# csiro-robotics/HOTFormerLoc

Hardware: AMD Instinct MI355X
Metric: point-clouds/sec (4096 pts, Wild-Places cfg) (higher is better)
Workload: dtype f32 storage and accumulation; Linear products as 3-term bf16 (hi, lo) split (16 significant bits per operand); window-attention QK^T / PV on fp16 (hi, lo) pairs (22 significant bits), softmax in f32; matched_precision leg = fp32-grade Linear products (3 bf16 planes per operand, 6 plane products) + f; 1 GPU; wild-places cfg, batch=32 clouds/GPU x 4096 pts, octree depth 7, forward-only, octree+neighbours resident, window plan + tap tables rebuilt inside every step (reference boundary); global_batch=32, parallelism=dp1, gemm=x3, collective=none

## Files before the change

### hotformerloc_amd/_native.py

```python

import ctypes
import os
from ctypes import c_char_p, c_double, c_float, c_int, c_int32, c_int64, c_uint32, c_uint64, c_void_p

_HERE = os.path.dirname(os.path.abspath(__file__))
LIB_PATH = os.path.join(_HERE, 'lib', 'libhotformerloc_hip.so')

HFL_OCTREE_MAX_POINTS = 1 << 20
HFL_OCTREE_MAX_DEPTH = 10


class NativeLibraryError(RuntimeError):
    pass


class WindowAttnDesc(ctypes.Structure):
    _fields_ = [('n_tokens', c_int64), ('rt_row0', c_int64), ('n_windows', c_int32),
                ('patch_size', c_int32), ('dilation', c_int32), ('n_relay', c_int32),
                ('n_heads', c_int32), ('pos_bnd', c_int32), ('batch_size', c_int32),
                ('scale', c_float), ('depth', c_int32), ('rpe_expanded', c_void_p)]


class BlockWeights(ctypes.Structure):
    _fields_ = [('channels', c_int64), ('eps', c_float), ('q_scale', c_float),
# ... 28 lines not shown
PHASE_REST = 2
PHASE_RELAY_QKV = 3
PHASE_TAIL = 4
FUSE_ATTN_NO_RELAY = 1
FUSE_ATTN_WS = 2


class BlockIO(ctypes.Structure):
    _fields_ = [('x_in', c_void_p), ('relay', c_void_p), ('out', c_void_p), ('arena', c_void_p),
                ('neigh', c_void_p), ('tok_meta', c_void_p), ('n_rows', c_int64), ('n_tokens', c_int64),
                ('phase', c_int32)]


class AdamChunk(ctypes.Structure):
    _fields_ = [('param', c_void_p), ('grad', c_void_p), ('exp_avg', c_void_p), ('exp_avg_sq', c_void_p), ('ema', c_void_p),
                ('count', c_int32), ('slot', c_int32)]


class AdamSlot(ctypes.Structure):
    _fields_ = [('step_size', c_float), ('bias_correction2_sqrt', c_float), ('one_minus_beta1', c_float), ('beta2', c_float),
                ('one_minus_beta2', c_float), ('eps', c_float), ('decay', c_float), ('decoupled', c_int32)]


class AugmentCloud(ctypes.Structure):
    _fields_ = [('remove_k', c_int32), ('block', c_int32), ('rot_cos', c_float), ('rot_sin', c_float), ('trans', c_float * 3),
                ('block_u', c_float * 4), ('reserved', c_float)]


class AugmentConfig(ctypes.Structure):
    _fields_ = [('normalize', c_int32), ('cylindrical_mask', c_int32), ('cylindrical_transform', c_int32),
                ('augment', c_int32), ('rotate', c_int32), ('set_rotate', c_int32), ('flip_axis', c_int32),
                ('set_cos', c_float), ('set_sin', c_float), ('jitter_sigma', c_float), ('jitter_clip', c_float)]


SIGNATURES = {
    'hfl_version': (c_int, []),
    'hfl_arch': (c_char_p, []),
    'hfl_dwconv_forward_backward': (c_int, [c_void_p, c_void_p, c_void_p, c_void_p, c_int, c_int64,
                                            c_int64, c_int, c_void_p]),
    'hfl_dwconv_weight_backward_workspace': (c_int64, [c_int64, c_int64, c_int]),
    'hfl_dwconv_weight_backward': (c_int, [c_void_p, c_void_p, c_void_p, c_void_p, c_int, c_int64,
                                           c_int64, c_int, c_void_p, c_void_p]),
    'hfl_inverse_neigh': (c_int, [c_void_p, c_void_p, c_int, c_int64, c_int, c_void_p]),
    'hfl_cpe_forward': (c_int, [c_void_p, c_void_p, c_void_p, c_void_p, c_void_p, c_void_p, c_int64,
                                c_int64, c_int, c_float, c_int, c_void_p]),
    'hfl_cpe_forward_save': (c_int, [c_void_p, c_void_p, c_void_p, c_void_p, c_void_p, c_void_p, c_void_p, c_int64,
                                c_int64, c_int, c_float, c_int, c_void_p]),
    'hfl_dwconv_add': (c_int, [c_void_p, c_void_p, c_void_p, c_void_p, c_void_p, c_int64, c_int64, c_int, c_void_p]),
    'hfl_octree_scratch_bytes': (c_int64, [c_int64, c_int, c_int, c_int]),
    'hfl_octree_build_clouds': (c_int, [c_void_p, c_void_p, c_int, c_int64, c_int, c_int, c_int,
                                        c_void_p, c_void_p, c_void_p, c_void_p]),
    'hfl_octree_merge': (c_int, [c_void_p, c_void_p, c_void_p, c_int, c_int, c_int, c_int64,
                                 c_void_p, c_void_p, c_void_p, c_void_p, c_void_p, c_void_p,
                                 c_void_p]),
    'hfl_octree_neigh': (c_int, [c_void_p, c_void_p, c_void_p, c_void_p, c_void_p, c_int64, c_int,
                                 c_int, c_void_p]),
    'hfl_token_meta': (c_int, [c_void_p, c_void_p, c_int64, c_int, c_void_p]),
    'hfl_octree_gather': (c_int, [c_void_p, c_void_p, c_void_p, c_int64, c_int, c_int64, c_void_p]),
    'hfl_prepare_clouds': (c_int, [c_void_p, c_void_p, c_void_p, c_void_p, c_int, c_int, c_int, c_int, c_void_p]),
    'hfl_augment_clouds': (c_int, [c_void_p, c_void_p, c_void_p, c_void_p, c_void_p, c_void_p, c_int, c_void_p, c_void_p,
                                   ctypes.POINTER(AugmentConfig), c_uint64, c_int64, c_void_p, c_void_p]),
    'hfl_voxel_keys': (c_int, [c_void_p, c_void_p, c_void_p, c_void_p, c_void_p, c_int, c_int64, c_double, c_void_p]),
    'hfl_voxel_reduce_workspace': (c_int64, [c_int64]),
    'hfl_voxel_reduce': (c_int, [c_void_p, c_void_p, c_void_p, c_void_p, c_void_p, c_void_p, c_void_p, c_int64, c_int, c_void_p,
                                 c_int64, c_void_p]),
    'hfl_submap_normalise': (c_int, [c_void_p, c_void_p, c_void_p, c_void_p, c_void_p, c_int, c_void_p]),
    'hfl_submap_normalise_rows': (c_int, [c_void_p] * 8 + [c_int, c_void_p]),
    'hfl_voxel_gather_rows': (c_int, [c_void_p, c_void_p, c_int64, c_void_p, c_int64, c_void_p]),
    'hfl_voxel_bounds': (c_int, [c_void_p, c_void_p, c_void_p, c_int, c_int64, c_void_p]),
    'hfl_voxel_occupancy_workspace': (c_int64, [c_int, c_int64]),
    'hfl_voxel_occupancy': (c_int, [c_void_p, c_void_p, c_int, c_int64, c_void_p, c_void_p, c_void_p, c_int, c_int64, c_int64,
                                    c_void_p, c_int64, c_void_p]),
    'hfl_cloth_raster': (c_int, [c_void_p, c_void_p, c_void_p, c_void_p, c_int, c_int64, c_void_p, c_void_p, c_int64, c_float,
                                 c_void_p]),
    'hfl_cloth_simulate': (c_int, [c_void_p, c_void_p, c_void_p, c_void_p, c_void_p, c_void_p, c_int, c_int64, c_float, c_float,
                                   c_float, c_float, c_int, c_int, c_void_p]),
    'hfl_cloth_classify': (c_int, [c_void_p, c_void_p, c_void_p, c_void_p, c_int, c_int64, c_void_p, c_void_p, c_int64, c_float,
                                   c_float, c_void_p]),
    'hfl_cloud_nonfinite': (c_int, [c_void_p, c_void_p, c_void_p, c_int, c_int64, c_void_p]),
    'hfl_knn_cell_keys': (c_int, [c_void_p, c_void_p, c_void_p, c_int, c_int64, c_void_p, c_void_p, c_int64, c_void_p]),
    'hfl_knn_mean_dist': (c_int, [c_void_p] * 9 + [c_int, c_int64, c_void_p, c_int64, c_int, c_void_p]),
    'hfl_outlier_threshold': (c_int, [c_void_p, c_void_p, c_void_p, c_int, c_int64, c_double, c_void_p]),
    'hfl_outlier_mask': (c_int, [c_void_p, c_void_p, c_void_p, c_void_p, c_int, c_int64, c_void_p]),
    'hfl_radius_mask': (c_int, [c_void_p, c_void_p, c_int64, c_double, c_void_p]),
    'hfl_tap_lists_workspace': (c_int64, [c_int64, c_int]),
    'hfl_tap_lists': (c_int, [c_void_p, c_void_p, c_void_p, c_void_p, c_int64, c_int, c_void_p, c_void_p]),
    'hfl_tap_lists_multi': (c_int, [c_int, c_void_p, c_void_p, c_void_p, c_void_p, c_void_p, c_void_p, c_void_p, c_void_p]),
    'hfl_tap_tiles': (c_int, [c_void_p, c_void_p, c_int, c_int, c_int, c_void_p]),
    'hfl_pad_index': (c_int, [c_void_p, c_void_p, c_int, c_int64, c_void_p]),
    'hfl_pad_rows': (c_int, [c_void_p, c_void_p, c_void_p, c_int, c_int64, c_int64, c_void_p]),
    'hfl_mixer_tail': (c_int, [c_void_p] * 6 + [c_int] * 5 + [c_void_p]),
    'hfl_attn_pool_ok': (c_int, [c_int]),
    'hfl_attn_pool_workspace': (c_int64, [c_int, c_int, c_int, c_int64]),
    'hfl_attn_pool': (c_int, [c_void_p, c_int64, c_void_p, c_void_p, c_void_p, c_int, c_int, c_int, c_int64, c_float, c_void_p,
                              c_int64, c_void_p]),
    'hfl_window_attention_fwd': (c_int, [c_void_p, c_void_p, c_void_p, c_void_p,
                                         ctypes.POINTER(WindowAttnDesc), c_void_p]),
    'hfl_window_attention_fwd_ex': (c_int, [c_void_p, c_void_p, c_void_p, c_void_p, c_void_p,
                                            ctypes.POINTER(WindowAttnDesc), c_int, c_void_p]),
    'hfl_window_attention_fwd_multi': (c_int, [c_int, c_void_p, c_void_p, c_void_p, c_void_p, c_void_p, c_int, c_void_p]),
    'hfl_layer_norm_split3': (c_int, [c_void_p, c_void_p, c_void_p, c_void_p, c_int64, c_int64,
                                      c_float, c_void_p]),
    'hfl_add_layer_norm_split3': (c_int, [c_void_p, c_void_p, c_void_p, c_void_p, c_void_p, c_void_p,
                                          c_void_p, c_int64, c_int64, c_float, c_void_p]),
    'hfl_add_bias': (c_int, [c_void_p, c_void_p, c_void_p, c_void_p, c_int64, c_int64, c_void_p]),
    'hfl_bias_gelu_split3': (c_int, [c_void_p, c_void_p, c_void_p, c_int64, c_int64, c_void_p]),
    'hfl_split3': (c_int, [c_void_p, c_void_p, c_int64, c_int64, c_void_p]),
    'hfl_window_attention_bwd': (c_int, [c_void_p, c_void_p, c_void_p, c_void_p, c_void_p, c_void_p,
                                         ctypes.POINTER(WindowAttnDesc), c_void_p]),
    'hfl_window_attention_bwd_workspace': (c_int64, [ctypes.POINTER(WindowAttnDesc)]),
    'hfl_window_attention_bwd_det': (c_int, [c_void_p, c_void_p, c_void_p, c_void_p, c_void_p, c_void_p,
                                             ctypes.POINTER(WindowAttnDesc), c_void_p, c_void_p]),
    'hfl_window_attention_bwd_split2': (c_int, [c_void_p, c_void_p, c_void_p, c_void_p, c_void_p, c_void_p,
                                                ctypes.POINTER(WindowAttnDesc), c_void_p, c_void_p]),
    'hfl_relay_attention_bwd': (c_int, [c_void_p, c_void_p, c_void_p, c_void_p, c_void_p, c_int, c_int,
                                        c_float, c_int, c_void_p]),
    'hfl_inverse_table': (c_int, [c_void_p, c_int64, c_void_p, c_int64, c_int, c_void_p]),
    'hfl_octree_gather_bwd': (c_int, [c_void_p, c_void_p, c_void_p, c_int64, c_int, c_int64, c_void_p]),
    'hfl_relay_token_init_bwd': (c_int, [c_void_p, c_void_p, c_void_p, c_int64, c_int32, c_int32,
                                         c_int64, c_void_p]),
    'hfl_linear_x3': (c_int, [c_void_p, c_void_p, c_void_p, c_void_p, c_void_p, c_int64, c_int, c_int, c_int, c_void_p]),
    'hfl_linear_x6_grouped_gather': (c_int, [c_void_p, c_void_p, c_void_p, c_void_p, c_int64, c_void_p, c_int64, c_int64, c_int, c_int,
                                     c_void_p]),
    'hfl_linear_x6_padded_k': (c_int64, [c_int64]),
    'hfl_linear_x6_pack': (c_int, [c_void_p, c_void_p, c_int64, c_int64, c_void_p]),
    'hfl_linear_x6': (c_int, [c_void_p, c_void_p, c_void_p, c_void_p, c_void_p, c_void_p, c_int64, c_int, c_int, c_int, c_void_p]),
    'hfl_linear_x6_gelu_fwd': (c_int, [c_void_p, c_void_p, c_void_p, c_void_p, c_void_p, c_int64, c_int, c_int, c_void_p]),
    'hfl_linear_x6_gelu_bwd': (c_int, [c_void_p, c_void_p, c_void_p, c_void_p, c_int64, c_int, c_int, c_void_p]),
    'hfl_layer_norm_split2': (c_int, [c_void_p, c_void_p, c_void_p, c_void_p, c_int64, c_int64,
                                      c_float, c_void_p]),
    'hfl_layer_norm_relu': (c_int, [c_void_p, c_void_p, c_void_p, c_void_p, c_void_p, c_int64, c_int64, c_float, c_void_p]),
    'hfl_linear_x3_qkv': (c_int, [c_void_p, c_void_p, c_void_p, c_void_p, c_int64, c_int, c_int, c_float, c_void_p]),
    'hfl_window_attention_f16_ok': (c_int, [ctypes.POINTER(WindowAttnDesc), c_int64]),
    'hfl_split2': (c_int, [c_void_p, c_void_p, c_int64, c_int64, c_void_p]),
    'hfl_block_forward_x3_arena': (c_int64, [c_int64, c_int64]),
    'hfl_block_forward_x3': (c_int, [c_void_p, c_void_p, c_void_p, c_void_p]),
    'hfl_block_attention_x3_multi': (c_int, [c_int, c_void_p, c_void_p, c_void_p, c_void_p]),
    'hfl_relay_block_forward_x3_arena': (c_int64, [c_int64, c_int64]),
    'hfl_relay_block_forward_x3': (c_int, [c_void_p, c_void_p, c_void_p]),
    'hfl_relay_block_fused_ok': (c_int, [c_void_p, c_void_p]),
    'hfl_relay_block_fused_x3': (c_int, [c_void_p, c_void_p, c_void_p]),
    'hfl_relay_block_pack_bytes': (c_int64, [c_int]),
    'hfl_relay_block_pack': (c_int, [c_void_p, c_void_p, c_void_p, c_void_p, c_void_p, c_int, c_void_p]),
    'hfl_linear_x3_grouped': (c_int, [c_void_p, c_void_p, c_void_p, c_void_p, c_int64, c_int64, c_int, c_int, c_void_p]),
    'hfl_linear_x3_grouped_gather': (c_int, [c_void_p, c_void_p, c_void_p, c_int64, c_void_p, c_void_p, c_int64, c_int64, c_int,
                                     c_int, c_void_p]),
    'hfl_split2_rows': (c_int, [c_void_p, c_void_p, c_void_p, c_int64, c_int64, c_void_p]),
    'hfl_linear_x3_rows': (c_int, [c_void_p, c_void_p, c_void_p, c_void_p, c_void_p, c_void_p, c_int64, c_int, c_int, c_void_p]),
    'hfl_linear_x3_gelu_fwd': (c_int, [c_void_p, c_void_p, c_void_p, c_void_p, c_void_p, c_int64, c_int, c_int, c_void_p]),
    'hfl_linear_x3_gelu_bwd': (c_int, [c_void_p, c_void_p, c_void_p, c_void_p, c_int64, c_int, c_int, c_void_p]),
    'hfl_tap_wgrad': (c_int, [c_void_p, c_void_p, c_void_p, c_void_p, c_int, c_void_p, c_int, c_int, c_int, c_void_p,
                             c_void_p]),
    'hfl_slot_sum': (c_int, [c_void_p, c_void_p, c_void_p, c_void_p, c_int64, c_int64, c_int, c_void_p]),
    'hfl_tap_wgrad_gather': (c_int, [c_void_p, c_void_p, c_void_p, c_void_p, c_void_p, c_void_p, c_int, c_void_p, c_int, c_int,
                                    c_int, c_void_p, c_void_p]),
    'hfl_wgrad_x3_workspace': (c_int64, [c_int64, c_int64, c_int64]),
    'hfl_wgrad_x3': (c_int, [c_void_p, c_void_p, c_void_p, c_void_p, c_int64, c_int64, c_int64, c_void_p, c_void_p]),
    'hfl_wgrad_f32_workspace': (c_int64, [c_int64, c_int64, c_int64]),
    'hfl_wgrad_f32': (c_int, [c_void_p, c_void_p, c_void_p, c_void_p, c_int64, c_int64, c_int64, c_void_p, c_void_p]),
    'hfl_layer_norm_bwd_blocks': (c_int, [c_int64, c_int64]),
    'hfl_layer_norm_bwd_add': (c_int, [c_void_p, c_void_p, c_void_p, c_void_p, c_void_p, c_void_p, c_void_p, c_int64, c_int64,
                                       c_float, c_void_p]),
    'hfl_layer_norm_bwd_finalize': (c_int, [c_void_p, c_void_p, c_void_p, c_void_p, c_int, c_int64, c_void_p]),
    'hfl_layer_norm_bwd': (c_int, [c_void_p, c_void_p, c_void_p, c_void_p, c_void_p, c_void_p, c_int64, c_int64,
                                   c_float, c_void_p]),
    'hfl_set_variant': (c_int, [c_char_p, c_int]),
    'hfl_smoothap_rows': (c_int, [c_void_p, c_void_p, c_void_p, c_void_p, c_void_p, c_void_p, c_int, c_int,
                                  c_float, c_void_p]),
    'hfl_pairwise_dist': (c_int, [c_void_p, c_void_p, c_int, c_int, c_void_p]),
    'hfl_pairwise_dist_bwd': (c_int, [c_void_p, c_void_p, c_void_p, c_void_p, c_int, c_int, c_void_p]),
    'hfl_batch_masks': (c_int, [c_void_p, c_void_p, c_void_p, c_void_p, c_int, c_void_p, c_void_p, c_void_p, c_void_p, c_int,
                                c_void_p]),
    'hfl_radius_lists': (c_int, [c_void_p, c_void_p, c_void_p, c_void_p, c_void_p, c_void_p, c_int64, c_void_p, c_int64, c_double,
                                 c_double, c_int, c_void_p]),
    'hfl_transform_points': (c_int, [c_void_p, c_void_p, c_void_p, c_void_p, c_int64, c_int64, c_void_p]),
    'hfl_nn_dist': (c_int, [c_void_p, c_void_p, c_void_p, c_void_p, c_int64, c_void_p, c_void_p, c_int64, c_void_p, c_int64,
                            c_int64, c_void_p]),
    'hfl_pair_stats': (c_int, [c_void_p, c_void_p, c_void_p, c_void_p, c_int64, c_int64, ctypes.POINTER(c_float), c_int,
                               c_void_p]),
    'hfl_ema_update': (c_int, [c_void_p, c_int, c_float, c_void_p]),
    'hfl_adam_step': (c_int, [c_void_p, c_int, c_void_p, c_int, c_float, c_void_p]),
    'hfl_kd_rows': (c_int, [c_void_p, c_void_p, c_void_p, c_void_p, c_int, c_int, c_float, c_void_p]),
    'hfl_gemm_bf16_tn': (c_int, [c_void_p, c_void_p, c_void_p, c_int64, c_int, c_int, c_void_p]),
    'hfl_gemm_bf16': (c_int, [c_void_p, c_void_p, c_void_p, c_void_p, c_void_p, c_int64, c_int, c_int, c_void_p]),
    'hfl_window_rpe_expand_size': (c_int64, [c_int, c_int, c_int, c_int]),
    'hfl_window_rpe_expand': (c_int, [c_void_p, c_void_p, c_int, c_int, c_int, c_int, c_void_p]),
    'hfl_relay_attention_fwd': (c_int, [c_void_p, c_void_p, c_void_p, c_void_p, c_int, c_int,
                                        c_float, c_int, c_void_p]),
    'hfl_relay_attention_f16_fwd': (c_int, [c_void_p, c_void_p, c_void_p, c_void_p, c_int, c_int, c_int, c_void_p, c_int, c_void_p]),
    'hfl_relay_token_init': (c_int, [c_void_p, c_void_p, c_void_p, c_int64, c_int32, c_int32,
                                     c_int64, c_void_p]),
    'hfl_window_stats': (c_int, [c_void_p, c_void_p, c_int64, c_int32, c_int32, c_int, c_void_p]),
    'hfl_layer_norm': (c_int, [c_void_p, c_void_p, c_void_p, c_void_p, c_int64, c_int64, c_float,
                               c_void_p]),
    'hfl_add_layer_norm': (c_int, [c_void_p, c_void_p, c_void_p, c_void_p, c_void_p, c_void_p,
                                   c_void_p, c_int64, c_int64, c_float, c_void_p]),
    'hfl_mlp_fused_pack_bytes': (c_int64, [c_int]),
    'hfl_mlp_fused_pack': (c_int, [c_void_p, c_void_p, c_void_p, c_int, c_void_p]),
    'hfl_ln_mlp_fused': (c_int, [c_void_p, c_void_p, c_void_p, c_void_p, c_float, c_void_p, c_void_p, c_void_p, c_int64, c_int,
                         c_void_p]),
    'hfl_ln_mlp_fused_workspace': (c_int64, [c_int64, c_int]),
    'hfl_mlp_fused_pack_bytes_h': (c_int64, [c_int, c_int]),
    'hfl_mlp_fused_pack_h': (c_int, [c_void_p, c_void_p, c_void_p, c_int, c_int, c_void_p]),
    'hfl_ln_mlp_fused_workspace_h': (c_int64, [c_int64, c_int, c_int]),
    'hfl_ln_mlp_fused_h': (c_int, [c_void_p, c_void_p, c_void_p, c_void_p, c_float, c_void_p, c_void_p, c_void_p, c_int64, c_int,
                                   c_int, c_void_p, c_int64, c_void_p]),
    'hfl_ln_mlp_fused_ws': (c_int, [c_void_p, c_void_p, c_void_p, c_void_p, c_float, c_void_p, c_void_p, c_void_p, c_int64, c_int,
                            c_void_p, c_int64, c_void_p]),
    'hfl_attn_fused_ok': (c_int, [c_void_p, c_int, c_int]),
    'hfl_attn_fused_fwd': (c_int, [c_void_p, c_void_p, c_void_p, c_void_p, c_float, c_void_p, c_void_p, c_float, c_void_p, c_void_p,
                           c_void_p, c_void_p]),
    'hfl_attn_ws_ok': (c_int, [c_void_p, c_int]),
    'hfl_attn_ws_fwd': (c_int, [c_void_p, c_void_p, c_void_p, c_void_p, c_float, c_void_p, c_void_p, c_float, c_void_p,
                        c_void_p, c_void_p, c_void_p, c_void_p]),
    'hfl_qkv_fused_pack_bytes': (c_int64, [c_int]),
    'hfl_qkv_fused_pack': (c_int, [c_void_p, c_void_p, c_int, c_void_p]),
    'hfl_ln_qkv_fused_seg': (c_int, [c_void_p, c_void_p, c_void_p, c_void_p, c_float, c_void_p, c_void_p, c_float, c_int64, c_int,
                                     c_void_p]),
    'hfl_linear_x3_seg': (c_int, [c_void_p, c_void_p, c_void_p, c_void_p, c_void_p, c_int64, c_int, c_int, c_void_p]),
    'hfl_ln_qkv_fused': (c_int, [c_void_p, c_void_p, c_void_p, c_void_p, c_float, c_void_p, c_void_p, c_float, c_int64, c_int,
                         c_void_p]),
    'hfl_segment_softmax': (c_int, [c_void_p, c_void_p, c_int, c_int, c_float, c_void_p]),
    'hfl_row_sq_norms': (c_int, [c_void_p, c_void_p, c_int64, c_int, c_void_p]),
    'hfl_flat_l2_topk_workspace': (c_int64, [c_int64, c_int64, c_int64, c_int]),
    'hfl_flat_l2_topk': (c_int, [c_void_p, c_void_p, c_void_p, c_void_p, c_void_p, c_int64, c_int64, c_int, c_int, c_void_p,
                                 c_int64, c_void_p]),
}

_lib = None


def load():
    global _lib
    if _lib is not None:
        return _lib
    if not os.path.exists(LIB_PATH):
        raise NativeLibraryError(
            'libhotformerloc_hip.so not found at %s -- the HIP extension is required '
            '(no CPU fallback); run `python -m hotformerloc_amd.build`' % LIB_PATH)
    lib = ctypes.CDLL(LIB_PATH)
    for name, (res, args) in SIGNATURES.items():
        try:
            fn = getattr(lib, name)
        except AttributeError as e:
            raise NativeLibraryError('symbol %s missing from %s' % (name, LIB_PATH)) from e
        fn.restype = res
        fn.argtypes = args
    _lib = lib
    return lib


def check(rc: int, what: str):
    if rc != 0:
        kind = {-1: 'HFL_EINVAL (unsupported shape/argument)',
                -2: 'HFL_ECAPACITY (input exceeds a kernel limit)'}.get(
                    rc, 'hipBLASLt status %d' % (-100 - rc) if rc <= -100 else 'hipError %d' % rc)
        raise NativeLibraryError('%s failed: %s' % (what, kind))


def ptr_array(ptrs):
    arr = (c_void_p * len(ptrs))()
    for i, p in enumerate(ptrs):
        arr[i] = p
    return arr
```

### hotformerloc_amd/build.py

```python

import os
import shutil
import subprocess
import sys
from concurrent.futures import ThreadPoolExecutor

HERE = os.path.dirname(os.path.abspath(__file__))
CSRC = os.path.join(HERE, 'csrc')
LIBDIR = os.path.join(HERE, 'lib')
LIBNAME = 'libhotformerloc_hip.so'
ARCH = 'gfx950'
SOURCES = ['capi.hip', 'dwconv.hip', 'octree.hip', 'preprocess.hip', 'augment.hip', 'voxel.hip', 'ground.hip', 'outliers.hip', 'window_misc.hip', 'attention.hip', 'gemm_x3.hip', 'gemm_x6.hip', 'mlp_fused.hip', 'qkv_fused.hip', 'attn_fused.hip', 'attn_ws.hip', 'relay_block.hip', 'attn_pool.hip', 'wgrad_x3.hip', 'wgrad_f32.hip', 'tapconv.hip', 'gemm_lt.hip', 'loss.hip', 'pairwise.hip', 'batch_masks.hip', 'radius.hip', 'overlap.hip', 'ema.hip', 'optim.hip', 'retrieval.hip']
FLAGS = ['--offload-arch=' + ARCH, '-O3', '-std=c++17', '-fPIC', '-fno-gpu-rdc',
         '-Wall', '-Wno-unused-function']
ROCM = os.environ.get('ROCM_PATH', '/opt/rocm')
LINK_FLAGS = ['-L' + os.path.join(ROCM, 'lib'), '-lhipblaslt', '-Wl,-rpath,' + os.path.join(ROCM, 'lib')]
EXTRA_FLAGS = {'attention.hip': ['-mllvm', '-amdgpu-mfma-vgpr-form=1'],
               'mlp_fused.hip': ['-fno-slp-vectorize'],
               'qkv_fused.hip': ['-fno-slp-vectorize'],
               'attn_fused.hip': ['-fno-slp-vectorize', '-mllvm', '-amdgpu-mfma-vgpr-form=1'],
               'attn_ws.hip': ['-fno-slp-vectorize', '-mllvm', '-amdgpu-mfma-vgpr-form=1'],
               'relay_block.hip': ['-fno-slp-vectorize', '-mllvm', '-amdgpu-mfma-vgpr-form=1'],
               'radius.hip': ['-ffp-contract=off'],
               'ground.hip': ['-ffp-contract=off'],
               'outliers.hip': ['-ffp-contract=off']}


def _hipcc() -> str:
    for cand in (os.environ.get('HIPCC'), shutil.which('hipcc'), '/opt/rocm/bin/hipcc'):
        if cand and os.path.exists(cand):
            return cand
    raise RuntimeError('hipcc not found (need ROCm >= 7.0 for gfx950)')


def _newer(target: str, deps) -> bool:
    if not os.path.exists(target):
        return False
    t = os.path.getmtime(target)
    return all(os.path.getmtime(d) <= t for d in deps)


def build_library(force: bool = False, verbose: bool = True) -> str:
    os.makedirs(LIBDIR, exist_ok=True)
    objdir = os.path.join(LIBDIR, 'obj')
    os.makedirs(objdir, exist_ok=True)
    hipcc = _hipcc()
    headers = [os.path.join(CSRC, 'hfl_common.h'), os.path.join(CSRC, 'x3_math.h'), os.path.join(CSRC, 'stage_stream.h'),
               os.path.join(CSRC, 'prep_common.h'),
               os.path.join(HERE, '..', 'include', 'hotformerloc_hip.h')]
    jobs = []
    for src in SOURCES:
        s = os.path.join(CSRC, src)
        o = os.path.join(objdir, src.replace('.hip', '.o'))
        if force or not _newer(o, [s] + headers):
            jobs.append((s, o))

    def compile_one(job):
        s, o = job
        cmd = [hipcc] + FLAGS + EXTRA_FLAGS.get(os.path.basename(s), []) + os.environ.get('HFL_EXTRA_HIPCC_FLAGS', '').split() + \
            ['-c', s, '-o', o]
        r = subprocess.run(cmd, capture_output=True, text=True)
        if r.returncode != 0:
            raise RuntimeError('hipcc failed for %s:\n%s' % (s, r.stderr))
        if verbose and r.stderr.strip():
            print(r.stderr, file=sys.stderr)
        return o

    if jobs:
        with ThreadPoolExecutor(max_workers=min(4, len(jobs))) as ex:
            list(ex.map(compile_one, jobs))
    objs = [os.path.join(objdir, s.replace('.hip', '.o')) for s in SOURCES]
    for stale in set(os.listdir(objdir)) - {os.path.basename(o) for o in objs}:
        os.remove(os.path.join(objdir, stale))
    lib = os.path.join(LIBDIR, LIBNAME)
    if force or jobs or not os.path.exists(lib):
        cmd = [hipcc, '--offload-arch=' + ARCH, '-shared', '-fPIC', '-o', lib] + objs + LINK_FLAGS
        r = subprocess.run(cmd, capture_output=True, text=True)
        if r.returncode != 0:
            raise RuntimeError('link failed:\n' + r.stderr)
    if verbose:
        print('built', lib)
    return lib


if __name__ == '__main__':
    build_library(force='--force' in sys.argv)
```

### hotformerloc_amd/csrc/dwconv.hip

```cpp
#include "hfl_common.h"

namespace {

constexpr int kMaxTaps = 27;
constexpr int kMaxRowsPerBlock = 16;

struct RowGeom {
  int tpr;
  int rpb;
};

static RowGeom row_geom(int64_t channels) {
  RowGeom g;
  g.tpr = (int)(channels / 4);
  g.rpb = 256 / g.tpr;
  if (g.rpb < 1) g.rpb = 1;
  if (g.rpb > kMaxRowsPerBlock) g.rpb = kMaxRowsPerBlock;
  return g;
}

static int persistent_per_cu(const void* kernel, int threads, size_t lds, int want, int* cache_nb, size_t* cache_lds) {
  if (*cache_lds != lds + 1) {
    int nb = 0;
    if (hipOccupancyMaxActiveBlocksPerMultiprocessor(&nb, kernel, threads, lds) != hipSuccess || nb < 1) nb = 0;
    *cache_nb = nb;
    *cache_lds = lds + 1;
  }
  const int nb = *cache_nb;
  if (nb < 1) return want;
  if (nb >= want) return want;
  return (want / nb) * nb >= nb ? ((want / nb) * nb) : nb;
}

template <typename IdxT, int KFIX>
__global__ void __launch_bounds__(256) dwconv_fwd_vec4(float* __restrict__ out, const float* __restrict__ data,
                                const float* __restrict__ weight, const IdxT* __restrict__ neigh,
                                int64_t n_out, int C, int kngh, int tpr, int rpb) {
  extern __shared__ __attribute__((aligned(16))) unsigned char smem[];
  const int K = KFIX > 0 ? KFIX : kngh;
  float4* s_w = reinterpret_cast<float4*>(smem);
  IdxT* s_idx = reinterpret_cast<IdxT*>(smem + (size_t)K * C * sizeof(float));
  const int tx = threadIdx.x % tpr, ty = threadIdx.x / tpr;
  const int c4n = C / 4;
  for (int i = threadIdx.x; i < K * c4n; i += blockDim.x)
    s_w[i] = reinterpret_cast<const float4*>(weight)[i];

  for (int64_t base = (int64_t)blockIdx.x * rpb; base < n_out; base += (int64_t)gridDim.x * rpb) {
    const int64_t h = base + ty;
    const bool live = h < n_out;
    __syncthreads();
    if (live)
      for (int k = tx; k < K; k += tpr) s_idx[ty * K + k] = neigh[h * K + k];
    __syncthreads();
    if (!live) continue;
    float4 acc = make_float4(0.f, 0.f, 0.f, 0.f);
    constexpr int B = 9;
#pragma unroll 1
    for (int k0 = 0; k0 < K; k0 += B) {
      float4 v[B];
      bool ok[B];
#pragma unroll
      for (int j = 0; j < B; ++j) {
        const int k = k0 + j;
        int64_t ni = (k < K) ? (int64_t)s_idx[ty * K + k] : -1;
        ok[j] = ni >= 0;
        if (!ok[j]) ni = 0;
        v[j] = reinterpret_cast<const float4*>(data + ni * C)[tx];
      }
#pragma unroll
      for (int j = 0; j < B; ++j) {
        const int k = k0 + j;
        if (k < K && ok[j]) acc = hfl_fma4(s_w[k * c4n + tx], v[j], acc);
      }
    }
    reinterpret_cast<float4*>(out + h * C)[tx] = acc;
  }
}

template <int B>
__global__ void __launch_bounds__(256) slot_sum_kernel(float* __restrict__ out, const float* __restrict__ part,
                                                        const int32_t* __restrict__ slot, const float* __restrict__ bias,
                                                        int64_t n_out, int C, int K, int tpr, int rpb) {
  extern __shared__ __attribute__((aligned(16))) unsigned char smem[];
  int32_t* s_idx = reinterpret_cast<int32_t*>(smem);
  const int tx = threadIdx.x % tpr, ty = threadIdx.x / tpr;
  const float4 bv = bias != nullptr ? reinterpret_cast<const float4*>(bias)[tx] : make_float4(0.f, 0.f, 0.f, 0.f);
  for (int64_t base = (int64_t)blockIdx.x * rpb; base < n_out; base += (int64_t)gridDim.x * rpb) {
    const int64_t h = base + ty;
    const bool live = h < n_out;
    __syncthreads();
    if (live)
      for (int k = tx; k < K; k += tpr) s_idx[ty * K + k] = slot[h * K + k];
    __syncthreads();
    if (!live) continue;
    float4 acc = make_float4(0.f, 0.f, 0.f, 0.f);
#pragma unroll 1
    for (int k0 = 0; k0 < K; k0 += B) {
      float4 v[B];
      bool ok[B];
#pragma unroll
      for (int j = 0; j < B; ++j) {
        const int k = k0 + j;
        int64_t ni = (k < K) ? (int64_t)s_idx[ty * K + k] : -1;
        ok[j] = ni >= 0;
        if (!ok[j]) ni = 0;
        v[j] = reinterpret_cast<const float4*>(part + ni * C)[tx];
      }
#pragma unroll
      for (int j = 0; j < B; ++j)
        if (ok[j]) { acc.x += v[j].x; acc.y += v[j].y; acc.z += v[j].z; acc.w += v[j].w; }
    }
    if (bias != nullptr) { acc.x += bv.x; acc.y += bv.y; acc.z += bv.z; acc.w += bv.w; }
    reinterpret_cast<float4*>(out + h * C)[tx] = acc;
  }
}

template <typename IdxT>
__global__ void dwconv_fwd_scalar(float* __restrict__ out, const float* __restrict__ data,
                                  const float* __restrict__ weight, const IdxT* __restrict__ neigh,
                                  int64_t n_out, int64_t C, int K) {
  const int64_t total = n_out * C;
  for (int64_t i = (int64_t)blockIdx.x * blockDim.x + threadIdx.x; i < total;
       i += (int64_t)gridDim.x * blockDim.x) {
    const int64_t h = i / C, c = i % C;
    float acc = 0.f;
    for (int k = 0; k < K; ++k) {
      const int64_t ni = (int64_t)neigh[h * K + k];
      if (ni >= 0) acc = fmaf(weight[k * C + c], data[ni * C + c], acc);
    }
    out[i] = acc;
  }
}

template <typename IdxT>
static int launch_fwd(float* out, const float* data, const float* weight, const IdxT* neigh,
                      int64_t n_out, int64_t C, int K, hipStream_t s) {
  if (n_out == 0) return HFL_OK;
  if (C % 4 == 0 && C <= 1024 && K <= kMaxTaps) {
    RowGeom g = row_geom(C);
    const size_t lds = (size_t)K * C * sizeof(float) + (size_t)g.rpb * K * sizeof(IdxT);
    const int64_t need = hfl_cdiv(n_out, g.rpb);
    static int nb27 = 0, nb0 = 0;
    static size_t l27 = 0, l0 = 0;
    const int per_cu = K == 27 ? persistent_per_cu(reinterpret_cast<const void*>(dwconv_fwd_vec4<IdxT, 27>), g.tpr * g.rpb, lds, 8,
                                                   &nb27, &l27)
                               : persistent_per_cu(reinterpret_cast<const void*>(dwconv_fwd_vec4<IdxT, 0>), g.tpr * g.rpb, lds, 8,
                                                   &nb0, &l0);
    const int64_t cap = (int64_t)hfl_stream_cus(s) * per_cu;
    const int blocks = (int)(need < cap ? need : cap);
    if (K == 27)
      dwconv_fwd_vec4<IdxT, 27><<<blocks, g.tpr * g.rpb, lds, s>>>(out, data, weight, neigh, n_out,
                                                                   (int)C, K, g.tpr, g.rpb);
    else
      dwconv_fwd_vec4<IdxT, 0><<<blocks, g.tpr * g.rpb, lds, s>>>(out, data, weight, neigh, n_out,
                                                                  (int)C, K, g.tpr, g.rpb);
  } else {
    const int64_t total = n_out * C;
    const int64_t need = hfl_cdiv(total, 256);
    const int blocks = (int)(need < 2048 ? need : 2048);
    dwconv_fwd_scalar<IdxT><<<blocks, 256, 0, s>>>(out, data, weight, neigh, n_out, C, K);
  }
  HFL_RETURN_LAST_ERROR();
}

template <typename IdxT, int B, int K0>
__device__ __forceinline__ void wgrad_taps(float4 (&acc)[kMaxTaps], const float4 g, const float* __restrict__ data,
                                           const IdxT* idx, int K, int C, int tx) {
  constexpr int NB = K0 + B <= kMaxTaps ? B : kMaxTaps - K0;
  float4 d[NB];
  bool ok[NB];
#pragma unroll
  for (int j = 0; j < NB; ++j) {
    const int64_t ni = K0 + j < K ? (int64_t)idx[K0 + j] : (int64_t)-1;
    ok[j] = ni >= 0;
    d[j] = reinterpret_cast<const float4*>(data + (ok[j] ? ni : (int64_t)0) * C)[tx];
  }
#pragma unroll
  for (int j = 0; j < NB; ++j) {
    const float4 a = hfl_fma4(d[j], g, acc[K0 + j]);
    acc[K0 + j].x = ok[j] ? a.x : acc[K0 + j].x;
    acc[K0 + j].y = ok[j] ? a.y : acc[K0 + j].y;
    acc[K0 + j].z = ok[j] ? a.z : acc[K0 + j].z;
    acc[K0 + j].w = ok[j] ? a.w : acc[K0 + j].w;
  }
}

template <typename IdxT, int B, int K0 = 0>
__device__ __forceinline__ void wgrad_row(float4 (&acc)[kMaxTaps], const float4 g, const float* __restrict__ data,
                                          const IdxT* idx, int K, int C, int tx) {
  if constexpr (K0 < kMaxTaps) {
    if (K0 < K) wgrad_taps<IdxT, B, K0>(acc, g, data, idx, K, C, tx);
    wgrad_row<IdxT, B, K0 + B>(acc, g, data, idx, K, C, tx);
  }
}

template <typename IdxT, int B>
__global__ void __launch_bounds__(256) dwconv_wgrad_partial(float* __restrict__ partial, const float* __restrict__ grad,
                                     const float* __restrict__ data, const IdxT* __restrict__ neigh,
                                     int64_t n_rows, int C, int K, int tpr, int rpb) {
  extern __shared__ __attribute__((aligned(16))) unsigned char smem[];
  IdxT* s_idx = reinterpret_cast<IdxT*>(smem);
  const int tx = threadIdx.x % tpr, ty = threadIdx.x / tpr;
  float4 acc[kMaxTaps];
#pragma unroll
  for (int k = 0; k < kMaxTaps; ++k) acc[k] = make_float4(0.f, 0.f, 0.f, 0.f);
  const int64_t groups = (n_rows + rpb - 1) / rpb;
  const int64_t per_xcd = (groups + 7) >> 3;
  const int xcd = blockIdx.x & 7;
  const int64_t xg0 = (int64_t)xcd * per_xcd;
  const int64_t xg1 = xg0 + per_xcd < groups ? xg0 + per_xcd : groups;
  const int nb = ((int)gridDim.x - xcd + 7) >> 3;
  for (int64_t grp = xg0 + (blockIdx.x >> 3); grp < xg1; grp += nb) {
    const int64_t h = grp * rpb + ty;
    const bool live = h < n_rows;
    __syncthreads();
    if (live)
      for (int k = tx; k < K; k += tpr) s_idx[ty * K + k] = neigh[h * K + k];
    __syncthreads();
    if (!live) continue;
    const float4 g = reinterpret_cast<const float4*>(grad + h * C)[tx];
    wgrad_row<IdxT, B>(acc, g, data, s_idx + ty * K, K, C, tx);
  }
  float4* s_red = reinterpret_cast<float4*>(smem + (((size_t)rpb * K * sizeof(IdxT) + 15) & ~(size_t)15));
#pragma unroll
  for (int k0 = 0; k0 < kMaxTaps; k0 += 9) {
    if (k0 < K && rpb > 1) {
      __syncthreads();
      if (ty > 0) {
#pragma unroll
        for (int j = 0; j < 9; ++j)
          if (k0 + j < K) s_red[((ty - 1) * 9 + j) * tpr + tx] = acc[k0 + j];
      }
      __syncthreads();
      if (ty == 0) {
        for (int t = 1; t < rpb; ++t) {
#pragma unroll
          for (int j = 0; j < 9; ++j)
            if (k0 + j < K) {
              const float4 v = s_red[((t - 1) * 9 + j) * tpr + tx];
              acc[k0 + j].x += v.x; acc[k0 + j].y += v.y; acc[k0 + j].z += v.z; acc[k0 + j].w += v.w;
            }
        }
      }
    }
  }
  if (ty == 0) {
    float4* dst = reinterpret_cast<float4*>(partial + (int64_t)blockIdx.x * K * C);
#pragma unroll
    for (int k = 0; k < kMaxTaps; ++k)
      if (k < K) dst[k * (C / 4) + tx] = acc[k];
  }
}

__global__ void __launch_bounds__(1024) dwconv_wgrad_reduce(float* __restrict__ out, const float* __restrict__ partial,
                                                            int n_partial, int64_t kc) {
  __shared__ float s[16][64];
  const int lane = threadIdx.x & 63, grp = threadIdx.x >> 6;
  const int64_t i = (int64_t)blockIdx.x * 64 + lane;
  float acc = 0.f;
  if (i < kc)
    for (int p = grp; p < n_partial; p += 16) acc += partial[(int64_t)p * kc + i];
  s[grp][lane] = acc;
  __syncthreads();
  if (grp == 0 && i < kc) {
    float v = 0.f;
#pragma unroll
// ... 29 lines not shown
template <typename IdxT>
static int launch_wgrad(float* out, const float* grad, const float* data, const IdxT* neigh,
                        int64_t n_rows, int64_t C, int K, void* workspace, hipStream_t s) {
  if (C % 4 == 0 && C <= 1024 && K <= kMaxTaps) {
    RowGeom g = row_geom(C);
    const int blocks = wgrad_blocks(n_rows, g.rpb);
    const size_t lds = (((size_t)g.rpb * K * sizeof(IdxT) + 15) & ~(size_t)15) +
                       (size_t)(g.rpb - 1) * 9 * C * sizeof(float);
    float* partial = static_cast<float*>(workspace);
    dwconv_wgrad_partial<IdxT, 9><<<blocks, g.tpr * g.rpb, lds, s>>>(partial, grad, data, neigh, n_rows, (int)C, K, g.tpr, g.rpb);
    const int64_t kc = (int64_t)K * C;
    dwconv_wgrad_reduce<<<(int)hfl_cdiv(kc, 64), 1024, 0, s>>>(out, partial, blocks, kc);
  } else {
    const int64_t kc = (int64_t)K * C;
    dwconv_wgrad_scalar<IdxT><<<(int)hfl_cdiv(kc, 256), 256, 0, s>>>(out, grad, data, neigh, n_rows, C, K);
  }
  HFL_RETURN_LAST_ERROR();
}

template <typename IdxT>
__global__ void inverse_neigh_kernel(IdxT* __restrict__ ineigh, const IdxT* __restrict__ neigh,
                                     int64_t n_rows, int K) {
  const int64_t total = n_rows * K;
  for (int64_t i = (int64_t)blockIdx.x * blockDim.x + threadIdx.x; i < total;
       i += (int64_t)gridDim.x * blockDim.x) {
    const int64_t h = i / K;
    const int k = (int)(i % K);
    const int64_t j = (int64_t)neigh[i];
    if (j >= 0) ineigh[j * K + k] = (IdxT)h;
  }
}

template <int TPR, bool NORM>
__global__ void __launch_bounds__(256) cpe_fwd_kernel(float* __restrict__ out, float* __restrict__ conv_out,
                               const float* __restrict__ x, const float* __restrict__ add,
                               const float* __restrict__ weight, const float* __restrict__ gamma,
                               const float* __restrict__ beta, const int32_t* __restrict__ neigh,
                               int64_t n_rows, int K, float eps, int residual) {
  constexpr int C = TPR * 4;
  constexpr int RPB = 256 / TPR;
  extern __shared__ __attribute__((aligned(16))) unsigned char smem[];
  float4* s_w = reinterpret_cast<float4*>(smem);
  int32_t* s_idx = reinterpret_cast<int32_t*>(smem + (size_t)K * C * sizeof(float));
  unsigned char* s_tap = reinterpret_cast<unsigned char*>(s_idx + (256 / TPR) * K);
  const int tx = threadIdx.x % TPR, ty = threadIdx.x / TPR;
  for (int i = threadIdx.x; i < K * TPR; i += blockDim.x)
    s_w[i] = reinterpret_cast<const float4*>(weight)[i];
  const float4 gm = NORM ? reinterpret_cast<const float4*>(gamma)[tx] : make_float4(1.f, 1.f, 1.f, 1.f);
  const float4 bt = NORM ? reinterpret_cast<const float4*>(beta)[tx] : make_float4(0.f, 0.f, 0.f, 0.f);

  const int64_t groups = (n_rows + RPB - 1) / RPB;
  const int64_t per_xcd = (groups + 7) >> 3;
  const int64_t xg0 = (int64_t)(blockIdx.x & 7) * per_xcd;
  const int64_t xg1 = xg0 + per_xcd < groups ? xg0 + per_xcd : groups;
  for (int64_t grp = xg0 + (blockIdx.x >> 3); grp < xg1; grp += gridDim.x >> 3) {
    const int64_t base = grp * RPB;
    const int64_t h = base + ty;
    const bool live = h < n_rows;
    __syncthreads();
    int n_live = 0;
    if (TPR >= kMaxTaps) {
      const int ni = (live && tx < K) ? neigh[h * K + tx] : -1;
      const unsigned long long bal = __ballot(ni >= 0);
      const int shift = (threadIdx.x & 63) - tx;
      const unsigned mask = (unsigned)((bal >> shift) & ((1ull << kMaxTaps) - 1ull));
      n_live = __popc(mask);
      if (ni >= 0) {
        const int rank = __popc(mask & ((1u << tx) - 1u));
        s_idx[ty * K + rank] = ni;
        s_tap[ty * K + rank] = (unsigned char)tx;
      }
    } else if (live) {
      for (int k = tx; k < K; k += TPR) s_idx[ty * K + k] = neigh[h * K + k];
    }
    __syncthreads();
    float4 acc = make_float4(0.f, 0.f, 0.f, 0.f);
    constexpr int B = 9;
    if (TPR >= kMaxTaps) {
#pragma unroll 1
      for (int k0 = 0; k0 < n_live; k0 += B) {
        float4 v[B];
        int e[B];
#pragma unroll
        for (int j = 0; j < B; ++j) {
          e[j] = ty * K + min(k0 + j, n_live - 1);
          v[j] = reinterpret_cast<const float4*>(x + (int64_t)s_idx[e[j]] * C)[tx];
        }
#pragma unroll
        for (int j = 0; j < B; ++j) {
          float4 w = s_w[(int)s_tap[e[j]] * TPR + tx];
          if (k0 + j >= n_live) w = make_float4(0.f, 0.f, 0.f, 0.f);
          acc = hfl_fma4(w, v[j], acc);
        }
      }
    } else {
#pragma unroll 1
      for (int k0 = 0; k0 < K; k0 += B) {
        float4 v[B];
        bool ok[B];
#pragma unroll
        for (int j = 0; j < B; ++j) {
          const int k = k0 + j;
          int64_t ni = (live && k < K) ? (int64_t)s_idx[ty * K + k] : -1;
          ok[j] = ni >= 0;
          if (!ok[j]) ni = 0;
          v[j] = reinterpret_cast<const float4*>(x + ni * C)[tx];
        }
#pragma unroll
        for (int j = 0; j < B; ++j) {
          const int k = k0 + j;
          if (k < K && ok[j]) acc = hfl_fma4(s_w[k * TPR + tx], v[j], acc);
        }
      }
    }
    float4 y = acc;
    if (NORM) {
      const float inv_c = 1.0f / (float)C;
      const float mean = hfl_group_sum<TPR>((acc.x + acc.y) + (acc.z + acc.w)) * inv_c;
      const float4 d = make_float4(acc.x - mean, acc.y - mean, acc.z - mean, acc.w - mean);
      const float var = hfl_group_sum<TPR>((d.x * d.x + d.y * d.y) + (d.z * d.z + d.w * d.w)) * inv_c;
      const float rstd = 1.0f / sqrtf(var + eps);
      y = make_float4(fmaf(d.x * rstd, gm.x, bt.x), fmaf(d.y * rstd, gm.y, bt.y),
                      fmaf(d.z * rstd, gm.z, bt.z), fmaf(d.w * rstd, gm.w, bt.w));
    }
    if (live) {
      if (NORM && conv_out != nullptr) reinterpret_cast<float4*>(conv_out + h * C)[tx] = acc;
      if (residual) {
        const float4 xv = reinterpret_cast<const float4*>(add + h * C)[tx];
        y.x += xv.x; y.y += xv.y; y.z += xv.z; y.w += xv.w;
      }
      reinterpret_cast<float4*>(out + h * C)[tx] = y;
    }
  }
}


template <int TPR, bool NORM>
static int launch_cpe(float* out, float* conv_out, const float* x, const float* add, const float* w, const float* gamma,
                      const float* beta, const int32_t* neigh, int64_t n, int K, float eps,
                      int residual, hipStream_t s) {
  constexpr int RPB = 256 / TPR;
  const size_t lds = (size_t)K * TPR * 16 + (size_t)RPB * K * (sizeof(int32_t) + 1) + 16;
  const int64_t need = hfl_cdiv(n, RPB);
  static int nb = 0;
  static size_t nb_lds = 0;
  const int per_cu = persistent_per_cu(reinterpret_cast<const void*>(cpe_fwd_kernel<TPR, NORM>), 256, lds, 8, &nb, &nb_lds);
  const int64_t cap = (int64_t)hfl_stream_cus(s) * per_cu;
  int blocks = (int)(need < cap ? need : cap);
  blocks = (blocks + 7) & ~7;
  cpe_fwd_kernel<TPR, NORM><<<blocks, 256, lds, s>>>(out, conv_out, x, add, w, gamma, beta, neigh, n, K, eps, residual);
  HFL_RETURN_LAST_ERROR();
}

}

extern "C" {

int hfl_dwconv_forward_backward(float* out, const float* data, const float* weight,
                                const void* neigh, int idx64, int64_t n_out, int64_t channels,
                                int kngh, hfl_stream_t stream) {
  if (n_out < 0 || channels <= 0 || kngh <= 0) return HFL_EINVAL;
  hipStream_t s = static_cast<hipStream_t>(stream);
  if (idx64)
    return launch_fwd<int64_t>(out, data, weight, static_cast<const int64_t*>(neigh), n_out,
                               channels, kngh, s);
  return launch_fwd<int32_t>(out, data, weight, static_cast<const int32_t*>(neigh), n_out,
                             channels, kngh, s);
}

int64_t hfl_dwconv_weight_backward_workspace(int64_t n_rows, int64_t channels, int kngh) {
  if (channels % 4 != 0 || channels > 1024 || kngh > kMaxTaps) return 16;
  RowGeom g = row_geom(channels);
  return (int64_t)wgrad_blocks(n_rows, g.rpb) * kngh * channels * (int64_t)sizeof(float);
}

int hfl_dwconv_weight_backward(float* out, const float* grad, const float* data,
                               const void* neigh, int idx64, int64_t n_rows, int64_t channels,
                               int kngh, void* workspace, hfl_stream_t stream) {
  if (n_rows < 0 || channels <= 0 || kngh <= 0) return HFL_EINVAL;
  hipStream_t s = static_cast<hipStream_t>(stream);
  if (idx64)
    return launch_wgrad<int64_t>(out, grad, data, static_cast<const int64_t*>(neigh), n_rows,
                                 channels, kngh, workspace, s);
  return launch_wgrad<int32_t>(out, grad, data, static_cast<const int32_t*>(neigh), n_rows,
                               channels, kngh, workspace, s);
}

int hfl_inverse_neigh(void* ineigh, const void* neigh, int idx64, int64_t n_rows, int kngh,
                      hfl_stream_t stream) {
  if (n_rows < 0 || kngh <= 0) return HFL_EINVAL;
  hipStream_t s = static_cast<hipStream_t>(stream);
  const size_t esz = idx64 ? 8 : 4;
  hipError_t e = hipMemsetAsync(ineigh, 0xFF, (size_t)n_rows * kngh * esz, s);
  if (e != hipSuccess) return (int)e;
  if (n_rows == 0) return HFL_OK;
  const int64_t need = hfl_cdiv(n_rows * kngh, 256);
  const int blocks = (int)(need < 4096 ? need : 4096);
  if (idx64)
    inverse_neigh_kernel<int64_t><<<blocks, 256, 0, s>>>(static_cast<int64_t*>(ineigh),
                                                         static_cast<const int64_t*>(neigh), n_rows, kngh);
  else
    inverse_neigh_kernel<int32_t><<<blocks, 256, 0, s>>>(static_cast<int32_t*>(ineigh),
                                                         static_cast<const int32_t*>(neigh), n_rows, kngh);
  HFL_RETURN_LAST_ERROR();
}

int hfl_cpe_forward_save(float* out, float* conv_out, const float* x, const float* weight, const float* gamma,
                         const float* beta, const int32_t* neigh, int64_t n_rows, int64_t channels,
                         int kngh, float eps, int residual, hfl_stream_t stream) {
  if (n_rows < 0 || kngh <= 0 || kngh > kMaxTaps) return HFL_EINVAL;
  if (n_rows == 0) return HFL_OK;
  hipStream_t s = static_cast<hipStream_t>(stream);
  switch (channels) {
    case 256: return launch_cpe<64, true>(out, conv_out, x, x, weight, gamma, beta, neigh, n_rows, kngh, eps, residual, s);
    case 128: return launch_cpe<32, true>(out, conv_out, x, x, weight, gamma, beta, neigh, n_rows, kngh, eps, residual, s);
    case 64:  return launch_cpe<16, true>(out, conv_out, x, x, weight, gamma, beta, neigh, n_rows, kngh, eps, residual, s);
    case 32:  return launch_cpe<8, true>(out, conv_out, x, x, weight, gamma, beta, neigh, n_rows, kngh, eps, residual, s);
    default:  return HFL_EINVAL;
  }
}

int hfl_dwconv_add(float* out, const float* data, const float* weight, const int32_t* neigh, const float* add,
                   int64_t n_out, int64_t channels, int kngh, hfl_stream_t stream) {
  if (n_out < 0 || kngh <= 0 || kngh > kMaxTaps || out == data || out == nullptr) return HFL_EINVAL;
  if (n_out == 0) return HFL_OK;
  hipStream_t s = static_cast<hipStream_t>(stream);
  const int res = add != nullptr ? 1 : 0;
  switch (channels) {
    case 256: return launch_cpe<64, false>(out, nullptr, data, add, weight, nullptr, nullptr, neigh, n_out, kngh, 0.f, res, s);
    case 128: return launch_cpe<32, false>(out, nullptr, data, add, weight, nullptr, nullptr, neigh, n_out, kngh, 0.f, res, s);
    case 64:  return launch_cpe<16, false>(out, nullptr, data, add, weight, nullptr, nullptr, neigh, n_out, kngh, 0.f, res, s);
    case 32:  return launch_cpe<8, false>(out, nullptr, data, add, weight, nullptr, nullptr, neigh, n_out, kngh, 0.f, res, s);
    default:  return HFL_EINVAL;
  }
}

int hfl_cpe_forward(float* out, const float* x, const float* weight, const float* gamma,
                    const float* beta, const int32_t* neigh, int64_t n_rows, int64_t channels,
                    int kngh, float eps, int residual, hfl_stream_t stream) {
  return hfl_cpe_forward_save(out, nullptr, x, weight, gamma, beta, neigh, n_rows, channels, kngh, eps, residual, stream);
}

int hfl_inverse_table(int32_t* inverse, int64_t n_src_rows, const int32_t* table, int64_t n_dst_rows,
                      int kngh, hfl_stream_t stream) {
  if (n_src_rows < 0 || n_dst_rows < 0 || kngh <= 0) return HFL_EINVAL;
  hipStream_t s = static_cast<hipStream_t>(stream);
  hipError_t e = hipMemsetAsync(inverse, 0xFF, (size_t)n_src_rows * kngh * sizeof(int32_t), s);
  if (e != hipSuccess) return (int)e;
  if (n_dst_rows == 0) return HFL_OK;
  const int64_t need = hfl_cdiv(n_dst_rows * kngh, 256);
  const int blocks = (int)(need < 4096 ? need : 4096);
  inverse_neigh_kernel<int32_t><<<blocks, 256, 0, s>>>(inverse, table, n_dst_rows, kngh);
  HFL_RETURN_LAST_ERROR();
}

int hfl_slot_sum(float* out, const float* part, const int32_t* slot, const float* bias, int64_t n_out, int64_t channels, int kngh,
                 hfl_stream_t stream) {
  if (n_out < 0 || channels <= 0 || channels % 4 != 0 || channels > 1024 || kngh <= 0 || kngh > kMaxTaps) return HFL_EINVAL;
  if (n_out == 0) return HFL_OK;
  if (out == nullptr || part == nullptr || slot == nullptr) return HFL_EINVAL;
  hipStream_t s = static_cast<hipStream_t>(stream);
  const RowGeom g = row_geom(channels);
  const size_t lds = (size_t)g.rpb * kngh * sizeof(int32_t);
  static int nb = 0;
  static size_t nb_lds = 0;
  const int per_cu = persistent_per_cu(reinterpret_cast<const void*>(slot_sum_kernel<9>), g.tpr * g.rpb, lds, 8, &nb, &nb_lds);
  const int64_t need = hfl_cdiv(n_out, g.rpb), cap = (int64_t)hfl_stream_cus(s) * per_cu;
  slot_sum_kernel<9><<<(int)(need < cap ? need : cap), g.tpr * g.rpb, lds, s>>>(out, part, slot, bias, n_out, (int)channels, kngh,
                                                                               g.tpr, g.rpb);
  HFL_RETURN_LAST_ERROR();
}
}
```

### hotformerloc_amd/csrc/octree.hip

```cpp
#include "hfl_common.h"

namespace {

constexpr int kBuildThreads = 1024;
constexpr int kLdsChunk = 16384;
constexpr int kMaxDepthSlots = HFL_OCTREE_MAX_DEPTH + 1;

__device__ __forceinline__ uint32_t shuffle_key(uint32_t x, uint32_t y, uint32_t z, int depth) {
  uint32_t key = 0;
  for (int i = 0; i < depth; ++i)
    key |= (((x >> i) & 1u) << (3 * i + 2)) | (((y >> i) & 1u) << (3 * i + 1)) |
           (((z >> i) & 1u) << (3 * i));
  return key;
}

__device__ __forceinline__ void unshuffle_key(uint32_t key, int depth, int& x, int& y, int& z) {
  x = y = z = 0;
  for (int i = 0; i < depth; ++i) {
    x |= ((key >> (3 * i + 2)) & 1u) << i;
    y |= ((key >> (3 * i + 1)) & 1u) << i;
    z |= ((key >> (3 * i)) & 1u) << i;
  }
}

// ... 170 lines not shown
      o[2] = sz / c;
      ++rank;
    }
  }
  int cur = total;
  if (tid == 0) counts[depth * batch + b] = cur;
  __syncthreads();

  for (int d = depth; d > full_depth; --d) {
    const uint32_t* kd = sv.key_at(d) + base;
    uint32_t* kp = sv.key_at(d - 1) + base;
    uint32_t* sl = sv.slot_at(d) + base;
    const int perd = (cur + kBuildThreads - 1) / kBuildThreads;
    const int a0 = min(tid * perd, cur), a1 = min(a0 + perd, cur);
    int h = 0;
    for (int i = a0; i < a1; ++i) h += (i == 0 || (kd[i - 1] >> 3) != (kd[i] >> 3)) ? 1 : 0;
    int tot = 0;
    int r = block_excl_scan(h, s_wave, &tot);
    for (int i = a0; i < a1; ++i) {
      const uint32_t ki = kd[i];
      if (i == 0 || (kd[i - 1] >> 3) != (ki >> 3)) {
        kp[r] = ki >> 3;
        ++r;
      }
      sl[i] = (uint32_t)(r - 1) * 8u + (ki & 7u);
    }
    cur = tot;
    if (tid == 0) counts[(d - 1) * batch + b] = cur;
    __syncthreads();
  }
  if (tid < full_depth) counts[tid * batch + b] = 1 << (3 * tid);
}

struct MergeArgs {
  int64_t* keys[kMaxDepthSlots];
  int32_t* children[kMaxDepthSlots];
  int64_t* nkeys[kMaxDepthSlots];
  int32_t* nidx[kMaxDepthSlots];
};

__device__ __forceinline__ int find_cloud(const int64_t* __restrict__ off, int batch, int64_t t) {
  int lo = 0, hi = batch;
  while (hi - lo > 1) {
    const int mid = (lo + hi) >> 1;
    if (off[mid] <= t) lo = mid; else hi = mid;
  }
  return lo;
}

__global__ void merge_sparse_kernel(ScratchView sv, const int64_t* __restrict__ cloud_off,
                                    const int32_t* __restrict__ cum_nne, int batch, int depth,
                                    int full_depth, MergeArgs a,
                                    const float* __restrict__ leaf_points,
                                    float* __restrict__ points_out) {
  const int d = full_depth + blockIdx.y;
  const int64_t t = (int64_t)blockIdx.x * blockDim.x + threadIdx.x;
  if (t >= sv.P) return;
  const int b = find_cloud(cloud_off, batch, t);
  const int64_t i = t - cloud_off[b];
  const int32_t* cum_d = cum_nne + (int64_t)d * (batch + 1);
  const int64_t cnt = cum_d[b + 1] - cum_d[b];
  if (i >= cnt) return;
  const int64_t g = cum_d[b] + i;
  const uint32_t key = sv.key_at(d)[t];
  const int64_t bbits = (int64_t)b << 48;
  a.nkeys[d][g] = bbits | (int64_t)key;
  int64_t pos;
  if (d == full_depth) {
    pos = ((int64_t)b << (3 * d)) + key;
  } else {
    const int32_t* cum_p = cum_nne + (int64_t)(d - 1) * (batch + 1);
    pos = 8 * (int64_t)cum_p[b] + sv.slot_at(d)[t];
  }
  a.nidx[d][g] = (int32_t)pos;
  a.children[d][pos] = (int32_t)g;
  if (d < depth && a.keys[d + 1] != nullptr) {
    int64_t* kc = a.keys[d + 1] + 8 * g;
#pragma unroll
    for (int j = 0; j < 8; ++j) kc[j] = bbits | (int64_t)(key * 8u + j);
  }
  if (d == depth) {
    const float* src = leaf_points + t * 3;
    float* dst = points_out + g * 3;
    dst[0] = src[0];
    dst[1] = src[1];
    dst[2] = src[2];
  }
}

__global__ void merge_full_kernel(int batch, int full_depth, MergeArgs a) {
  const int d = blockIdx.y;
  const int64_t per = (int64_t)1 << (3 * d);
  const int64_t t = (int64_t)blockIdx.x * blockDim.x + threadIdx.x;
  if (t >= per * batch) return;
  const int64_t b = t / per, m = t % per;
  if (a.keys[d] != nullptr) a.keys[d][t] = (b << 48) | m;
  if (d < full_depth) {
    a.children[d][t] = (int32_t)t;
    a.nkeys[d][t] = (b << 48) | m;
    a.nidx[d][t] = (int32_t)t;
  }
}

__global__ void neigh_full_kernel(int32_t* __restrict__ out, const int32_t* __restrict__ children,
                                  const int64_t* __restrict__ nkeys, int64_t nne, int depth) {
  const int64_t t = (int64_t)blockIdx.x * blockDim.x + threadIdx.x;
  if (t >= nne * 27) return;
  const int64_t g = t / 27;
  const int o = (int)(t % 27);
  const int64_t key = nkeys[g];
  const int64_t b = key >> 48;
  int x, y, z;
  unshuffle_key((uint32_t)(key & 0xFFFFFFFFll), depth, x, y, z);
  x += o / 9 - 1;
  y += (o / 3) % 3 - 1;
  z += o % 3 - 1;
  const int bound = 1 << depth;
  int32_t res = -1;
  if (x >= 0 && y >= 0 && z >= 0 && x < bound && y < bound && z < bound)
    res = children[(b << (3 * depth)) + shuffle_key((uint32_t)x, (uint32_t)y, (uint32_t)z, depth)];
  out[t] = res;
}

__global__ void neigh_walk_kernel(int32_t* __restrict__ out, const int32_t* __restrict__ neigh_parent,
                                  const int32_t* __restrict__ nidx,
                                  const int32_t* __restrict__ children, int64_t nne) {
  const int64_t t = (int64_t)blockIdx.x * blockDim.x + threadIdx.x;
  if (t >= nne * 27) return;
  const int64_t g = t / 27;
  const int o = (int)(t % 27);
  const int32_t pos = nidx[g];
  const int64_t parent = pos >> 3;
  const int oct = pos & 7;
  const int tx = ((oct >> 2) & 1) + o / 9 - 1;
  const int ty = ((oct >> 1) & 1) + (o / 3) % 3 - 1;
  const int tz = (oct & 1) + o % 3 - 1;
  const int po = ((tx >> 1) + 1) * 9 + ((ty >> 1) + 1) * 3 + ((tz >> 1) + 1);
  const int co = ((tx & 1) << 2) | ((ty & 1) << 1) | (tz & 1);
  const int32_t q = neigh_parent[parent * 27 + po];
  out[t] = q < 0 ? -1 : children[(int64_t)q * 8 + co];
}

__global__ void token_meta_kernel(uint32_t* __restrict__ meta, const int64_t* __restrict__ nkeys,
                                  int64_t n, int depth) {
  const int64_t t = (int64_t)blockIdx.x * blockDim.x + threadIdx.x;
  if (t >= n) return;
  const int64_t key = nkeys[t];
  int x, y, z;
  unshuffle_key((uint32_t)(key & 0xFFFFFFFFll), depth, x, y, z);
  meta[2 * t] = (uint32_t)x | ((uint32_t)y << 10) | ((uint32_t)z << 20);
  meta[2 * t + 1] = (uint32_t)(key >> 48);
}

constexpr int kTapRows = 1024;
constexpr int kTapMax = 32;
constexpr int kTapTables = 16;

struct TapTable {
  const int32_t* table;
  int32_t* src;
  int32_t* slot;
  int32_t* edges;
  int32_t* block_counts;
  int64_t rows;
  int taps;
  int first_block;
};
struct TapMulti {
  TapTable t[kTapTables];
  int n;
  int total_blocks;
};

__device__ __forceinline__ const TapTable& tap_find(const TapMulti& m, int block, int& local) {
  int i = 0;
  while (i + 1 < m.n && block >= m.t[i + 1].first_block) ++i;
  local = block - m.t[i].first_block;
  return m.t[i];
}

template <int TAPS>
__device__ __forceinline__ void tap_load_rows(const int32_t* __restrict__ table, int64_t rows, int64_t row0, int32_t* lds_wave,
                                              int lane, int32_t (&v)[kTapMax], int taps_rt) {
  if constexpr (TAPS == 8) {
    const int64_t r = row0 + lane;
    int4 a = make_int4(-1, -1, -1, -1), b = a;
    if (r < rows) {
      a = reinterpret_cast<const int4*>(table)[r * 2];
      b = reinterpret_cast<const int4*>(table)[r * 2 + 1];
    }
    v[0] = a.x; v[1] = a.y; v[2] = a.z; v[3] = a.w; v[4] = b.x; v[5] = b.y; v[6] = b.z; v[7] = b.w;
  } else if constexpr (TAPS > 0) {
    const int64_t w0 = row0 * TAPS, wend = rows * TAPS;
#pragma unroll
    for (int j = 0; j < TAPS; ++j) {
      const int64_t w = w0 + j * 64 + lane;
      lds_wave[j * 64 + lane] = w < wend ? table[w] : -1;
    }
    __builtin_amdgcn_fence(__ATOMIC_RELEASE, "wavefront");
    __builtin_amdgcn_wave_barrier();
#pragma unroll
    for (int k = 0; k < TAPS; ++k) v[k] = lds_wave[lane * TAPS + k];
    __builtin_amdgcn_wave_barrier();
  } else {
    const int64_t r = row0 + lane;
#pragma unroll
    for (int k = 0; k < kTapMax; ++k)
      if (k < taps_rt) v[k] = r < rows ? table[r * taps_rt + k] : -1;
  }
}

template <int TAPS>
__device__ __forceinline__ void tap_count_body(const TapTable& t, int block, int32_t* lds) {
  __shared__ int32_t wave_cnt[4][kTapMax];
  const int lane = threadIdx.x & 63, wave = threadIdx.x >> 6;
  const int taps = TAPS > 0 ? TAPS : t.taps;
  int32_t acc[kTapMax];
#pragma unroll
  for (int k = 0; k < kTapMax; ++k) acc[k] = 0;
  const int64_t row0 = (int64_t)block * kTapRows;
  int32_t* lds_wave = lds + wave * (64 * (TAPS > 0 ? TAPS : 1));
  for (int it = 0; it < kTapRows / 256; ++it) {
    int32_t v[kTapMax];
    tap_load_rows<TAPS>(t.table, t.rows, row0 + it * 256 + wave * 64, lds_wave, lane, v, taps);
#pragma unroll
    for (int k = 0; k < kTapMax; ++k)
      if (k < taps) acc[k] += __popcll(__ballot(v[k] >= 0));
  }
  if (lane == 0)
    for (int k = 0; k < taps; ++k) wave_cnt[wave][k] = acc[k];
  __syncthreads();
  if ((int)threadIdx.x < taps)
    t.block_counts[(int64_t)block * taps + threadIdx.x] =
        wave_cnt[0][threadIdx.x] + wave_cnt[1][threadIdx.x] + wave_cnt[2][threadIdx.x] + wave_cnt[3][threadIdx.x];
}

__global__ void __launch_bounds__(256)
tap_count_kernel(const TapMulti m) {
  __shared__ int32_t lds[4 * 64 * 27];
  int block;
  const TapTable& t = tap_find(m, blockIdx.x, block);
  if (t.taps == 27) tap_count_body<27>(t, block, lds);
  else if (t.taps == 8) tap_count_body<8>(t, block, lds);
  else tap_count_body<0>(t, block, lds);
}

__global__ void __launch_bounds__(1024)
tap_scan_kernel(const TapMulti m) {
  __shared__ int32_t total[kTapMax];
  const TapTable& t = m.t[blockIdx.x];
  const int taps = t.taps;
  const int nblocks = (blockIdx.x + 1 < (unsigned)m.n ? m.t[blockIdx.x + 1].first_block : m.total_blocks) - t.first_block;
  int32_t* block_counts = t.block_counts;
  const int lane = threadIdx.x & 63;
  for (int k = threadIdx.x >> 6; k < taps; k += 16) {
    int32_t run = 0;
    for (int b0 = 0; b0 < nblocks; b0 += 64) {
      const int b = b0 + lane;
      const int32_t v = b < nblocks ? block_counts[(int64_t)b * taps + k] : 0;
      int32_t inc = v;
#pragma unroll
      for (int o = 1; o < 64; o <<= 1) {
        const int32_t u = __shfl_up(inc, o, 64);
        if (lane >= o) inc += u;
      }
      if (b < nblocks) block_counts[(int64_t)b * taps + k] = run + inc - v;
      run += __shfl(inc, 63, 64);
    }
    if (lane == 0) total[k] = run;
  }
  __syncthreads();
  if (threadIdx.x == 0) {
    int32_t e = 0;
    for (int k = 0; k < taps; ++k) {
      t.edges[k] = e;
      e += total[k];
    }
    t.edges[taps] = e;
  }
}

template <int TAPS>
__device__ __forceinline__ void tap_fill_body(const TapTable& t, int block, int32_t* lds) {
  __shared__ int32_t wave_cnt[4][kTapMax];
  __shared__ int32_t base[kTapMax];
  const int lane = threadIdx.x & 63, wave = threadIdx.x >> 6;
  const int taps = TAPS > 0 ? TAPS : t.taps;
  if ((int)threadIdx.x < taps) base[threadIdx.x] = t.edges[threadIdx.x] + t.block_counts[(int64_t)block * taps + threadIdx.x];
  const int64_t row0 = (int64_t)block * kTapRows;
  const unsigned long long lt = lane == 0 ? 0ull : (~0ull >> (64 - lane));
  int32_t* lds_wave = lds + wave * (64 * (TAPS > 0 ? TAPS : 1));
  for (int it = 0; it < kTapRows / 256; ++it) {
    const int64_t rw = row0 + it * 256 + wave * 64;
    const int64_t r = rw + lane;
    const bool in = r < t.rows;
    int32_t v[kTapMax];
    unsigned long long mk[kTapMax];
    tap_load_rows<TAPS>(t.table, t.rows, rw, lds_wave, lane, v, taps);
#pragma unroll
    for (int k = 0; k < kTapMax; ++k)
      if (k < taps) mk[k] = __ballot(v[k] >= 0);
    __syncthreads();
    if (lane == 0)
      for (int k = 0; k < taps; ++k) wave_cnt[wave][k] = __popcll(mk[k]);
    __syncthreads();
    int32_t pos[kTapMax];
#pragma unroll
    for (int k = 0; k < kTapMax; ++k) {
      if (k < taps) {
        int32_t off = base[k];
        for (int w = 0; w < wave; ++w) off += wave_cnt[w][k];
        pos[k] = v[k] >= 0 ? off + __popcll(mk[k] & lt) : -1;
        if (in && v[k] >= 0) t.src[pos[k]] = v[k];
      }
    }
    if constexpr (TAPS == 8) {
      if (in) {
        reinterpret_cast<int4*>(t.slot)[r * 2] = make_int4(pos[0], pos[1], pos[2], pos[3]);
        reinterpret_cast<int4*>(t.slot)[r * 2 + 1] = make_int4(pos[4], pos[5], pos[6], pos[7]);
      }
    } else if constexpr (TAPS > 0) {
#pragma unroll
      for (int k = 0; k < TAPS; ++k) lds_wave[lane * TAPS + k] = pos[k];
      __builtin_amdgcn_fence(__ATOMIC_RELEASE, "wavefront");
      __builtin_amdgcn_wave_barrier();
      const int64_t w0 = rw * TAPS, wend = t.rows * TAPS;
#pragma unroll
      for (int j = 0; j < TAPS; ++j) {
        const int64_t w = w0 + j * 64 + lane;
        if (w < wend) t.slot[w] = lds_wave[j * 64 + lane];
      }
      __builtin_amdgcn_wave_barrier();
    } else {
#pragma unroll
      for (int k = 0; k < kTapMax; ++k)
        if (k < taps && in) t.slot[r * taps + k] = pos[k];
    }
    __syncthreads();
    if ((int)threadIdx.x < taps)
      base[threadIdx.x] += wave_cnt[0][threadIdx.x] + wave_cnt[1][threadIdx.x] + wave_cnt[2][threadIdx.x] +
                           wave_cnt[3][threadIdx.x];
  }
}

__global__ void __launch_bounds__(256)
tap_fill_kernel(const TapMulti m) {
  __shared__ int32_t lds[4 * 64 * 27];
  int block;
  const TapTable& t = tap_find(m, blockIdx.x, block);
  if (t.taps == 27) tap_fill_body<27>(t, block, lds);
  else if (t.taps == 8) tap_fill_body<8>(t, block, lds);
  else tap_fill_body<0>(t, block, lds);
}

}

extern "C" {

int64_t hfl_octree_scratch_bytes(int64_t total_points, int batch, int max_points, int depth) {
  return level_words(total_points, depth) * (int64_t)sizeof(uint32_t) +
         (int64_t)batch * next_pow2(max_points) * (int64_t)sizeof(unsigned long long) + 64;
}

int hfl_octree_build_clouds(const float* points, const int64_t* cloud_offsets, int batch,
                              int64_t total_points, int max_points, int depth, int full_depth,
                              void* scratch, float* leaf_points, int32_t* counts,
                              hfl_stream_t stream) {
  if (batch <= 0 || depth < 1 || depth > HFL_OCTREE_MAX_DEPTH || full_depth < 0 || full_depth > depth)
    return HFL_EINVAL;
  if (max_points > HFL_OCTREE_MAX_POINTS) return HFL_ECAPACITY;
  if (max_points < 1) return HFL_EINVAL;
  int ch_cap = next_pow2(max_points);
  if (ch_cap > kLdsChunk) ch_cap = kLdsChunk;
  hipStream_t s = static_cast<hipStream_t>(stream);
  ScratchView sv = make_view(scratch, total_points, max_points, depth, full_depth);
  const size_t lds = (size_t)ch_cap * 8 + 32 * sizeof(int);
  hipError_t e = hipFuncSetAttribute(reinterpret_cast<const void*>(build_cloud_kernel),
                                     hipFuncAttributeMaxDynamicSharedMemorySize, (int)lds);
  if (e != hipSuccess) return (int)e;
  build_cloud_kernel<<<batch, kBuildThreads, lds, s>>>(points, cloud_offsets, batch, depth, full_depth,
                                                       sv, leaf_points, counts, ch_cap);
  HFL_RETURN_LAST_ERROR();
}

int hfl_octree_merge(const void* scratch, const int64_t* cloud_offsets, const int32_t* cum_nne,
                     int batch, int depth, int full_depth, int64_t total_points,
                     int64_t* const* keys, int32_t* const* children, int64_t* const* nkeys,
                     int32_t* const* nidx, const float* leaf_points, float* points_out,
                     hfl_stream_t stream) {
  if (batch <= 0 || depth < 1 || depth > HFL_OCTREE_MAX_DEPTH || full_depth < 0 || full_depth > depth)
    return HFL_EINVAL;
  hipStream_t s = static_cast<hipStream_t>(stream);
  MergeArgs a;
  for (int d = 0; d < kMaxDepthSlots; ++d) {
    const bool in = d <= depth;
    a.keys[d] = (in && keys != nullptr) ? keys[d] : nullptr;
    a.children[d] = in ? children[d] : nullptr;
    a.nkeys[d] = in ? nkeys[d] : nullptr;
    a.nidx[d] = in ? nidx[d] : nullptr;
  }
  ScratchView sv = make_view(const_cast<void*>(scratch), total_points, 2, depth, full_depth);
  {
    const int64_t per = ((int64_t)1 << (3 * full_depth)) * batch;
    dim3 grid((unsigned)hfl_cdiv(per, 256), (unsigned)(full_depth + 1));
    merge_full_kernel<<<grid, 256, 0, s>>>(batch, full_depth, a);
  }
  if (total_points > 0) {
    dim3 grid((unsigned)hfl_cdiv(total_points, 256), (unsigned)(depth - full_depth + 1));
    merge_sparse_kernel<<<grid, 256, 0, s>>>(sv, cloud_offsets, cum_nne, batch, depth, full_depth, a,
                                             leaf_points, points_out);
  }
  HFL_RETURN_LAST_ERROR();
}

int hfl_octree_neigh(int32_t* neigh_out, const int32_t* neigh_parent, const int32_t* nidx,
                     const int32_t* children, const int64_t* nkeys, int64_t nne, int depth,
                     int full_depth, hfl_stream_t stream) {
  if (nne < 0 || depth < 0) return HFL_EINVAL;
  if (nne == 0) return HFL_OK;
  hipStream_t s = static_cast<hipStream_t>(stream);
  const unsigned blocks = (unsigned)hfl_cdiv(nne * 27, 256);
  if (depth <= full_depth)
    neigh_full_kernel<<<blocks, 256, 0, s>>>(neigh_out, children, nkeys, nne, depth);
  else
    neigh_walk_kernel<<<blocks, 256, 0, s>>>(neigh_out, neigh_parent, nidx, children, nne);
  HFL_RETURN_LAST_ERROR();
}

int hfl_token_meta(uint32_t* tok_meta, const int64_t* nkeys, int64_t n, int depth,
                   hfl_stream_t stream) {
  if (n < 0 || depth < 0 || depth > HFL_OCTREE_MAX_DEPTH) return HFL_EINVAL;
  if (n == 0) return HFL_OK;
  token_meta_kernel<<<(unsigned)hfl_cdiv(n, 256), 256, 0, static_cast<hipStream_t>(stream)>>>(
      tok_meta, nkeys, n, depth);
  HFL_RETURN_LAST_ERROR();
}

int64_t hfl_tap_lists_workspace(int64_t rows, int taps) {
  return hfl_cdiv(rows > 0 ? rows : 1, kTapRows) * (int64_t)taps * (int64_t)sizeof(int32_t);
}

int hfl_tap_lists_multi(int n, int32_t* const* src, int32_t* const* slot, int32_t* const* edges, const int32_t* const* table,
                        const int64_t* rows, const int32_t* taps, void* const* workspace, hfl_stream_t stream) {
  if (n < 1 || n > kTapTables || src == nullptr || slot == nullptr || edges == nullptr || table == nullptr || rows == nullptr ||
      taps == nullptr || workspace == nullptr)
    return HFL_EINVAL;
  TapMulti m;
  m.n = n;
  int first = 0;
  for (int i = 0; i < n; ++i) {
    if (rows[i] < 0 || taps[i] < 1 || taps[i] > kTapMax) return HFL_EINVAL;
    if (rows[i] * taps[i] > 0x7fffffffLL) return HFL_ECAPACITY;
    m.t[i].table = table[i]; m.t[i].src = src[i]; m.t[i].slot = slot[i]; m.t[i].edges = edges[i];
    m.t[i].block_counts = static_cast<int32_t*>(workspace[i]);
    m.t[i].rows = rows[i]; m.t[i].taps = taps[i]; m.t[i].first_block = first;
    first += (int)hfl_cdiv(rows[i] > 0 ? rows[i] : 1, kTapRows);
  }
  for (int i = n; i < kTapTables; ++i) m.t[i] = m.t[0];
  m.total_blocks = first;
  hipStream_t s = static_cast<hipStream_t>(stream);
  tap_count_kernel<<<first, 256, 0, s>>>(m);
  tap_scan_kernel<<<n, 1024, 0, s>>>(m);
  tap_fill_kernel<<<first, 256, 0, s>>>(m);
  HFL_RETURN_LAST_ERROR();
}

int hfl_tap_lists(int32_t* src, int32_t* slot, int32_t* edges, const int32_t* table, int64_t rows, int taps,
                  void* workspace, hfl_stream_t stream) {
  const int32_t t = taps;
  return hfl_tap_lists_multi(1, &src, &slot, &edges, &table, &rows, &t, &workspace, stream);
}

__global__ void __launch_bounds__(64) tap_tiles_kernel(int32_t* __restrict__ tiles, const int32_t* __restrict__ edges, int taps,
                                                       int tile_rows, int w_rows) {
  __shared__ int first[kTapMax + 1];
  if (threadIdx.x == 0) {
    int acc = 0;
    for (int k = 0; k < taps; ++k) {
      first[k] = acc;
      acc += (edges[k + 1] - edges[k] + tile_rows - 1) / tile_rows;
    }
    first[taps] = acc;
  }
  __syncthreads();
  for (int k = 0; k < taps; ++k) {
    const int a = edges[k], b = edges[k + 1];
    for (int t = threadIdx.x; t < first[k + 1] - first[k]; t += blockDim.x) {
      const int r0 = a + t * tile_rows;
      int32_t* o = tiles + 3 * (int64_t)(first[k] + t);
      o[0] = r0;
      o[1] = b - r0 < tile_rows ? b - r0 : tile_rows;
      o[2] = k * w_rows;
    }
  }
// ... 57 lines not shown
```

### hotformerloc_amd/csrc/window_misc.hip

```cpp
#include "hfl_common.h"

namespace {

template <int VEC>
__global__ void gather_kernel(float* __restrict__ out, const float* __restrict__ data,
                              const int32_t* __restrict__ neigh, int64_t n_out, int K, int C) {
  const int cv = C / VEC;
  const int64_t total = n_out * K * cv;
  for (int64_t i = (int64_t)blockIdx.x * blockDim.x + threadIdx.x; i < total;
       i += (int64_t)gridDim.x * blockDim.x) {
    const int64_t mk = i / cv;
    const int c = (int)(i % cv);
    const int32_t ni = neigh[mk];
    if (VEC == 4) {
      float4 v = make_float4(0.f, 0.f, 0.f, 0.f);
      if (ni >= 0) v = reinterpret_cast<const float4*>(data + (int64_t)ni * C)[c];
      reinterpret_cast<float4*>(out + mk * C)[c] = v;
    } else {
      out[mk * C + c] = ni >= 0 ? data[(int64_t)ni * C + c] : 0.f;
    }
  }
}


__global__ void gather_bwd_kernel(float* __restrict__ ddata, const float* __restrict__ dcol,
                                  const int32_t* __restrict__ ineigh, int64_t n_rows, int K, int C) {
  const int cv = C / 4;
  const int64_t total = n_rows * cv;
  for (int64_t i = (int64_t)blockIdx.x * blockDim.x + threadIdx.x; i < total;
       i += (int64_t)gridDim.x * blockDim.x) {
    const int64_t n = i / cv;
    const int c = (int)(i % cv);
    float4 acc = make_float4(0.f, 0.f, 0.f, 0.f);
    for (int k = 0; k < K; ++k) {
      const int32_t m = ineigh[n * K + k];
      if (m >= 0) {
        const float4 v = reinterpret_cast<const float4*>(dcol + ((int64_t)m * K + k) * C)[c];
        acc.x += v.x; acc.y += v.y; acc.z += v.z; acc.w += v.w;
      }
    }
    reinterpret_cast<float4*>(ddata + n * C)[c] = acc;
  }
}

__global__ void gather_bwd_scalar_kernel(float* __restrict__ ddata, const float* __restrict__ dcol,
                                         const int32_t* __restrict__ ineigh, int64_t n_rows, int K, int C) {
  const int64_t total = n_rows * C;
  for (int64_t i = (int64_t)blockIdx.x * blockDim.x + threadIdx.x; i < total;
       i += (int64_t)gridDim.x * blockDim.x) {
    const int64_t n = i / C;
    const int c = (int)(i % C);
    float acc = 0.f;
    for (int k = 0; k < K; ++k) {
      const int32_t m = ineigh[n * K + k];
      if (m >= 0) acc += dcol[((int64_t)m * K + k) * C + c];
    }
    ddata[i] = acc;
  }
}

__global__ void relay_init_bwd_kernel(float* __restrict__ dx, const float* __restrict__ drt,
                                      const uint32_t* __restrict__ meta, int64_t n_tokens,
                                      int32_t n_windows, int K, int C) {
  const int cv = C / 4;
  const int c = threadIdx.x;
  for (int w = blockIdx.x; w < n_windows; w += gridDim.x) {
    const int64_t t0 = (int64_t)w * K;
    if (t0 >= n_tokens) continue;
    const uint32_t owner = meta[2 * t0 + 1];
    int cnt = 0;
    for (int k = 0; k < K; ++k) {
      const int64_t t = t0 + k;
      if (t >= n_tokens || meta[2 * t + 1] != owner) break;
      ++cnt;
    }
    float4 gsc = make_float4(0.f, 0.f, 0.f, 0.f);
    if (c < cv) {
      const float4 gr = reinterpret_cast<const float4*>(drt + (int64_t)w * C)[c];
      const float n = (float)cnt;
      gsc = make_float4(gr.x / n, gr.y / n, gr.z / n, gr.w / n);
    }
    for (int k = 0; k < K; ++k) {
      const int64_t t = t0 + k;
      if (t >= n_tokens) break;
      if (c < cv)
        reinterpret_cast<float4*>(dx + t * C)[c] = k < cnt ? gsc : make_float4(0.f, 0.f, 0.f, 0.f);
    }
  }
}

__global__ void relay_init_kernel(float* __restrict__ rt, const float* __restrict__ x,
                                  const uint32_t* __restrict__ meta, int64_t n_tokens,
                                  int32_t n_windows, int K, int C) {
  const int cv = C / 4;
  const int c = threadIdx.x;
  const int lane = threadIdx.x & 63;
  for (int w = blockIdx.x; w < n_windows; w += gridDim.x) {
    const int64_t t0 = (int64_t)w * K;
    float4 acc = make_float4(0.f, 0.f, 0.f, 0.f);
    int cnt = 0;
    if (t0 < n_tokens) {
      const uint32_t owner = meta[2 * t0 + 1];
      for (int k0 = 0; k0 < K; k0 += 64) {
        const int k = k0 + lane;
        const int64_t t = t0 + k;
        const bool mine = k < K && t < n_tokens && meta[2 * (t < n_tokens ? t : t0) + 1] == owner;
        const unsigned long long lead = ~__ballot(mine);
        const int run = lead == 0ull ? 64 : __builtin_ctzll(lead);
        cnt += run;
        if (run < 64) break;
      }
      if (c < cv) {
        for (int k0 = 0; k0 < cnt; k0 += 8) {
          float4 v[8];
#pragma unroll
          for (int j = 0; j < 8; ++j) v[j] = reinterpret_cast<const float4*>(x + (t0 + (k0 + j < cnt ? k0 + j : 0)) * C)[c];
#pragma unroll
          for (int j = 0; j < 8; ++j)
            if (k0 + j < cnt) { acc.x += v[j].x; acc.y += v[j].y; acc.z += v[j].z; acc.w += v[j].w; }
        }
      }
    }
    if (c < cv) {
      float4 o = make_float4(0.f, 0.f, 0.f, 0.f);
      if (cnt > 0) {
        const float n = (float)cnt;
        o = make_float4(acc.x / n, acc.y / n, acc.z / n, acc.w / n);
      }
      reinterpret_cast<float4*>(rt + (int64_t)w * C)[c] = o;
    }
  }
}

__global__ void window_stats_kernel(float* __restrict__ stats, const uint32_t* __restrict__ meta,
                                    int64_t n_tokens, int32_t n_windows, int K, float scale) {
  const int w = blockIdx.x * blockDim.x + threadIdx.x;
  if (w >= n_windows) return;
  float* o = stats + (int64_t)w * 9;
  const int64_t t0 = (int64_t)w * K;
  float out[9] = {0.f, 0.f, 0.f, 0.f, 0.f, 0.f, 0.f, 0.f, 0.f};
  if (t0 < n_tokens) {
    const uint32_t owner = meta[2 * t0 + 1];
    int cnt = 0;
    float sx = 0.f, sy = 0.f, sz = 0.f;
    for (int k = 0; k < K; ++k) {
      const int64_t t = t0 + k;
      if (t >= n_tokens || meta[2 * t + 1] != owner) break;
      const uint32_t p = meta[2 * t];
      sx += (float)(p & 1023u) * scale - 1.0f;
      sy += (float)((p >> 10) & 1023u) * scale - 1.0f;
      sz += (float)((p >> 20) & 1023u) * scale - 1.0f;
      ++cnt;
    }
    const float c = (float)cnt;
    const float cs = c < 1.f ? 1.f : c;
    const float mx = sx / cs, my = sy / cs, mz = sz / cs;
    out[0] = mx; out[1] = my; out[2] = mz;
    if (cnt >= 2) {
      float cxx = 0.f, cxy = 0.f, cxz = 0.f, cyy = 0.f, cyz = 0.f, czz = 0.f;
      for (int k = 0; k < cnt; ++k) {
        const uint32_t p = meta[2 * (t0 + k)];
        const float dx = ((float)(p & 1023u) * scale - 1.0f) - mx;
        const float dy = ((float)((p >> 10) & 1023u) * scale - 1.0f) - my;
        const float dz = ((float)((p >> 20) & 1023u) * scale - 1.0f) - mz;
        cxx += dx * dx; cxy += dx * dy; cxz += dx * dz;
        cyy += dy * dy; cyz += dy * dz; czz += dz * dz;
      }
      const float den = c - 1.0f;
      out[3] = cxx / den; out[4] = cxy / den; out[5] = cxz / den;
      out[6] = cyy / den; out[7] = cyz / den; out[8] = czz / den;
    }
  }
#pragma unroll
  for (int i = 0; i < 9; ++i) o[i] = out[i];
}

__global__ void __launch_bounds__(1024)
segment_softmax_kernel(float* __restrict__ scores, const int64_t* __restrict__ row_off,
                       int n_queries, float scale) {
  __shared__ float s_m[16][64];
  __shared__ float s_l[16][64];
  const int b = blockIdx.x;
  const int q = blockIdx.y * 64 + (threadIdx.x & 63);
  const int grp = threadIdx.x >> 6;
  const int64_t r0 = row_off[b], r1 = row_off[b + 1];
  const bool live = q < n_queries;
  float m = -INFINITY, l = 0.f;
  if (live) {
    for (int64_t r = r0 + grp; r < r1; r += 16) {
      const float s = scores[r * n_queries + q] * scale;
      const float mn = fmaxf(m, s);
      l = l * __expf(m - mn) + __expf(s - mn);
      m = mn;
    }
  }
  s_m[grp][threadIdx.x & 63] = m;
  s_l[grp][threadIdx.x & 63] = l;
  __syncthreads();
  float M = -INFINITY;
#pragma unroll
  for (int g = 0; g < 16; ++g) M = fmaxf(M, s_m[g][threadIdx.x & 63]);
  float L = 0.f;
#pragma unroll
  for (int g = 0; g < 16; ++g) {
    const float mg = s_m[g][threadIdx.x & 63];
    if (mg > -INFINITY) L += s_l[g][threadIdx.x & 63] * __expf(mg - M);
  }
  if (live && L > 0.f) {
    const float inv = 1.0f / L;
    for (int64_t r = r0 + grp; r < r1; r += 16) {
      const int64_t idx = r * n_queries + q;
      scores[idx] = __expf(scores[idx] * scale - M) * inv;
    }
  }
}


__device__ __forceinline__ uint16_t hfl_bf16_rne(float v) {
  uint32_t u = __float_as_uint(v);
  u += 0x7FFFu + ((u >> 16) & 1u);
  return (uint16_t)(u >> 16);
}
__device__ __forceinline__ void hfl_split4(const float4 v, uint2& hi, uint2& lo) {
  const uint16_t h0 = hfl_bf16_rne(v.x), h1 = hfl_bf16_rne(v.y), h2 = hfl_bf16_rne(v.z), h3 = hfl_bf16_rne(v.w);
  const uint16_t l0 = hfl_bf16_rne(v.x - __uint_as_float((uint32_t)h0 << 16));
  const uint16_t l1 = hfl_bf16_rne(v.y - __uint_as_float((uint32_t)h1 << 16));
  const uint16_t l2 = hfl_bf16_rne(v.z - __uint_as_float((uint32_t)h2 << 16));
  const uint16_t l3 = hfl_bf16_rne(v.w - __uint_as_float((uint32_t)h3 << 16));
  hi = make_uint2((uint32_t)h0 | ((uint32_t)h1 << 16), (uint32_t)h2 | ((uint32_t)h3 << 16));
  lo = make_uint2((uint32_t)l0 | ((uint32_t)l1 << 16), (uint32_t)l2 | ((uint32_t)l3 << 16));
}
__device__ __forceinline__ void hfl_store_split3(uint16_t* row, int C, int c4, const float4 v) {
  uint2 hi, lo;
  hfl_split4(v, hi, lo);
  reinterpret_cast<uint2*>(row)[c4] = hi;
  reinterpret_cast<uint2*>(row + C)[c4] = hi;
  reinterpret_cast<uint2*>(row + 2 * C)[c4] = lo;
}

__device__ __forceinline__ void hfl_store_split2(uint16_t* row, int c4, const float4 v) {
  uint2 hi, lo;
  hfl_split4(v, hi, lo);
  uint16_t* o = row + (c4 >> 3) * 64 + (c4 & 7) * 4;
  *reinterpret_cast<uint2*>(o) = hi;
  *reinterpret_cast<uint2*>(o + 32) = lo;
}

template <int TPR, int VPL, bool ADD, int SPLIT>
__global__ void __launch_bounds__(256)
layer_norm_kernel(float* __restrict__ h_out, float* x_out, const float* x, const float* __restrict__ y,
                  const float* __restrict__ bias, const float* __restrict__ gamma,
                  const float* __restrict__ beta, int64_t n_rows, float eps, int relu) {
  constexpr int C = TPR * VPL * 4;
  constexpr int RPB = 256 / TPR;
  const int tx = threadIdx.x % TPR, ty = threadIdx.x / TPR;
  float4 gm[VPL], bt[VPL], bs[VPL];
#pragma unroll
  for (int v = 0; v < VPL; ++v) {
    gm[v] = reinterpret_cast<const float4*>(gamma)[v * TPR + tx];
    bt[v] = reinterpret_cast<const float4*>(beta)[v * TPR + tx];
    bs[v] = make_float4(0.f, 0.f, 0.f, 0.f);
    if (ADD && bias != nullptr) bs[v] = reinterpret_cast<const float4*>(bias)[v * TPR + tx];
  }
  const float inv_c = 1.0f / (float)C;
  for (int64_t base = (int64_t)blockIdx.x * RPB; base < n_rows; base += (int64_t)gridDim.x * RPB) {
    const int64_t r = base + ty;
    const bool live = r < n_rows;
    float4 a[VPL];
    float sum = 0.f;
#pragma unroll
    for (int v = 0; v < VPL; ++v) {
      a[v] = make_float4(0.f, 0.f, 0.f, 0.f);
      if (live) {
        a[v] = reinterpret_cast<const float4*>(x + r * C)[v * TPR + tx];
        if (ADD) {
          const float4 b = reinterpret_cast<const float4*>(y + r * C)[v * TPR + tx];
          a[v].x += b.x + bs[v].x; a[v].y += b.y + bs[v].y;
          a[v].z += b.z + bs[v].z; a[v].w += b.w + bs[v].w;
          reinterpret_cast<float4*>(x_out + r * C)[v * TPR + tx] = a[v];
        }
      }
      sum += (a[v].x + a[v].y) + (a[v].z + a[v].w);
    }
    const float mean = hfl_group_sum<TPR>(sum) * inv_c;
    float sq = 0.f;
#pragma unroll
    for (int v = 0; v < VPL; ++v) {
      a[v].x -= mean; a[v].y -= mean; a[v].z -= mean; a[v].w -= mean;
      sq += (a[v].x * a[v].x + a[v].y * a[v].y) + (a[v].z * a[v].z + a[v].w * a[v].w);
    }
    const float rstd = 1.0f / sqrtf(hfl_group_sum<TPR>(sq) * inv_c + eps);
    if (live) {
#pragma unroll
      for (int v = 0; v < VPL; ++v) {
        float4 o;
        o.x = fmaf(a[v].x * rstd, gm[v].x, bt[v].x);
        o.y = fmaf(a[v].y * rstd, gm[v].y, bt[v].y);
        o.z = fmaf(a[v].z * rstd, gm[v].z, bt[v].z);
        o.w = fmaf(a[v].w * rstd, gm[v].w, bt[v].w);
        if (relu) {
          o.x = fmaxf(o.x, 0.f); o.y = fmaxf(o.y, 0.f); o.z = fmaxf(o.z, 0.f); o.w = fmaxf(o.w, 0.f);
        }
        if (SPLIT == 1)
          hfl_store_split3(reinterpret_cast<uint16_t*>(h_out) + r * 3 * C, C, v * TPR + tx, o);
        else if (SPLIT == 2)
          hfl_store_split2(reinterpret_cast<uint16_t*>(h_out) + r * 2 * C, v * TPR + tx, o);
        else
          reinterpret_cast<float4*>(h_out + r * C)[v * TPR + tx] = o;
      }
    }
  }
}

template <int TPR, int VPL>
static int launch_ln(float* h_out, float* x_out, const float* x, const float* y, const float* bias,
                     const float* gamma, const float* beta, int64_t n, float eps, int split_flags,
                     hipStream_t s) {
  const int split = split_flags & 0xF, relu = (split_flags >> 4) & 1;
  constexpr int RPB = 256 / TPR;
  const int64_t need = hfl_cdiv(n, RPB);
  const int64_t cap = (int64_t)hfl_stream_cus(s) * 16;
  const int blocks = (int)(need < cap ? need : cap);
  if (y != nullptr) {
    if (split == 2)
      layer_norm_kernel<TPR, VPL, true, 2><<<blocks, 256, 0, s>>>(h_out, x_out, x, y, bias, gamma, beta, n, eps, relu);
    else if (split)
      layer_norm_kernel<TPR, VPL, true, 1><<<blocks, 256, 0, s>>>(h_out, x_out, x, y, bias, gamma, beta, n, eps, relu);
    else
      layer_norm_kernel<TPR, VPL, true, 0><<<blocks, 256, 0, s>>>(h_out, x_out, x, y, bias, gamma, beta, n, eps, relu);
  } else {
    if (split == 2)
      layer_norm_kernel<TPR, VPL, false, 2><<<blocks, 256, 0, s>>>(h_out, x_out, x, y, bias, gamma, beta, n, eps, relu);
    else if (split)
      layer_norm_kernel<TPR, VPL, false, 1><<<blocks, 256, 0, s>>>(h_out, x_out, x, y, bias, gamma, beta, n, eps, relu);
    else
      layer_norm_kernel<TPR, VPL, false, 0><<<blocks, 256, 0, s>>>(h_out, x_out, x, y, bias, gamma, beta, n, eps, relu);
  }
  HFL_RETURN_LAST_ERROR();
}

static int dispatch_ln(float* h_out, float* x_out, const float* x, const float* y, const float* bias,
                       const float* gamma, const float* beta, int64_t n, int64_t C, float eps,
                       int split, hipStream_t s) {
  if (n == 0) return HFL_OK;
  switch (C) {
    case 16:   return launch_ln<4, 1>(h_out, x_out, x, y, bias, gamma, beta, n, eps, split, s);
    case 32:   return launch_ln<8, 1>(h_out, x_out, x, y, bias, gamma, beta, n, eps, split, s);
    case 64:   return launch_ln<16, 1>(h_out, x_out, x, y, bias, gamma, beta, n, eps, split, s);
    case 128:  return launch_ln<32, 1>(h_out, x_out, x, y, bias, gamma, beta, n, eps, split, s);
    case 256:  return launch_ln<64, 1>(h_out, x_out, x, y, bias, gamma, beta, n, eps, split, s);
    case 512:  return launch_ln<64, 2>(h_out, x_out, x, y, bias, gamma, beta, n, eps, split, s);
    case 1024: return launch_ln<64, 4>(h_out, x_out, x, y, bias, gamma, beta, n, eps, split, s);
    default:   return HFL_EINVAL;
  }
}

template <int TPR, int VPL>
__global__ void __launch_bounds__(256)
layer_norm_bwd_kernel(float* __restrict__ dx, float* __restrict__ dg_part, float* __restrict__ db_part,
                      const float* __restrict__ dy, const float* __restrict__ x, const float* __restrict__ gamma,
                      const float* dres, int64_t n_rows, float eps) {
  constexpr int C = TPR * VPL * 4;
  constexpr int RPB = 256 / TPR;
  __shared__ float4 s_red[256];
  const int tx = threadIdx.x % TPR, ty = threadIdx.x / TPR;
  float4 gm[VPL], ag[VPL], ab[VPL];
#pragma unroll
  for (int v = 0; v < VPL; ++v) {
    gm[v] = reinterpret_cast<const float4*>(gamma)[v * TPR + tx];
    ag[v] = make_float4(0.f, 0.f, 0.f, 0.f);
    ab[v] = ag[v];
  }
  const float inv_c = 1.0f / (float)C;
  for (int64_t base = (int64_t)blockIdx.x * RPB; base < n_rows; base += (int64_t)gridDim.x * RPB) {
    const int64_t r = base + ty;
    const bool live = r < n_rows;
    float4 a[VPL], d[VPL];
    float sum = 0.f;
#pragma unroll
    for (int v = 0; v < VPL; ++v) {
      a[v] = make_float4(0.f, 0.f, 0.f, 0.f);
      d[v] = a[v];
      if (live) {
        a[v] = reinterpret_cast<const float4*>(x + r * C)[v * TPR + tx];
        d[v] = reinterpret_cast<const float4*>(dy + r * C)[v * TPR + tx];
      }
      sum += (a[v].x + a[v].y) + (a[v].z + a[v].w);
    }
    const float mean = hfl_group_sum<TPR>(sum) * inv_c;
    float sq = 0.f;
#pragma unroll
    for (int v = 0; v < VPL; ++v) {
      a[v].x -= mean; a[v].y -= mean; a[v].z -= mean; a[v].w -= mean;
      sq += (a[v].x * a[v].x + a[v].y * a[v].y) + (a[v].z * a[v].z + a[v].w * a[v].w);
    }
    const float rstd = 1.0f / sqrtf(hfl_group_sum<TPR>(sq) * inv_c + eps);
    float s1 = 0.f, s2 = 0.f;
#pragma unroll
    for (int v = 0; v < VPL; ++v) {
      a[v].x *= rstd; a[v].y *= rstd; a[v].z *= rstd; a[v].w *= rstd;
      ab[v].x += d[v].x; ab[v].y += d[v].y; ab[v].z += d[v].z; ab[v].w += d[v].w;
      ag[v].x = fmaf(d[v].x, a[v].x, ag[v].x); ag[v].y = fmaf(d[v].y, a[v].y, ag[v].y);
      ag[v].z = fmaf(d[v].z, a[v].z, ag[v].z); ag[v].w = fmaf(d[v].w, a[v].w, ag[v].w);
      d[v].x *= gm[v].x; d[v].y *= gm[v].y; d[v].z *= gm[v].z; d[v].w *= gm[v].w;
      s1 += (d[v].x + d[v].y) + (d[v].z + d[v].w);
      s2 += (d[v].x * a[v].x + d[v].y * a[v].y) + (d[v].z * a[v].z + d[v].w * a[v].w);
    }
    s1 = hfl_group_sum<TPR>(s1) * inv_c;
    s2 = hfl_group_sum<TPR>(s2) * inv_c;
    if (live) {
#pragma unroll
      for (int v = 0; v < VPL; ++v) {
        float4 o;
        o.x = rstd * (d[v].x - s1 - a[v].x * s2);
        o.y = rstd * (d[v].y - s1 - a[v].y * s2);
        o.z = rstd * (d[v].z - s1 - a[v].z * s2);
        o.w = rstd * (d[v].w - s1 - a[v].w * s2);
        if (dres != nullptr) {
          const float4 rs = reinterpret_cast<const float4*>(dres + r * C)[v * TPR + tx];
          o.x += rs.x; o.y += rs.y; o.z += rs.z; o.w += rs.w;
        }
        reinterpret_cast<float4*>(dx + r * C)[v * TPR + tx] = o;
      }
    }
  }
#pragma unroll
  for (int v = 0; v < VPL; ++v) {
#pragma unroll
    for (int which = 0; which < 2; ++which) {
      __syncthreads();
      s_red[threadIdx.x] = which == 0 ? ag[v] : ab[v];
      __syncthreads();
      if (ty == 0) {
        float4 t = s_red[tx];
        for (int j = 1; j < RPB; ++j) {
          const float4 u = s_red[j * TPR + tx];
          t.x += u.x; t.y += u.y; t.z += u.z; t.w += u.w;
        }
        float* dst = (which == 0 ? dg_part : db_part) + (int64_t)blockIdx.x * C;
        reinterpret_cast<float4*>(dst)[v * TPR + tx] = t;
      }
    }
  }
}

static int ln_bwd_blocks(int64_t n, int rpb) {
  const int64_t need = hfl_cdiv(n, rpb);
  const int64_t cap = (int64_t)hfl_num_cus() * 8;
  return (int)(need < cap ? (need < 1 ? 1 : need) : cap);
}

template <int TPR, int VPL>
static int launch_ln_bwd(float* dx, float* dgp, float* dbp, const float* dy, const float* x, const float* gamma,
                         const float* dres, int64_t n, float eps, hipStream_t s) {
  layer_norm_bwd_kernel<TPR, VPL><<<ln_bwd_blocks(n, 256 / TPR), 256, 0, s>>>(dx, dgp, dbp, dy, x, gamma, dres, n, eps);
  HFL_RETURN_LAST_ERROR();
}

template <int MODE>
__global__ void __launch_bounds__(256)
eltwise_kernel(void* __restrict__ out, const float* a, const float* b,
               const float* __restrict__ bias, int64_t n_rows, int C) {
  const int cv = C / 4;
// ... 259 lines not shown
```

### hotformerloc_amd/model.py

```python

import contextlib
import functools
import os
from typing import Dict, List, Optional

import torch
import torch.nn as nn
import torch.nn.functional as F
from torch.utils.checkpoint import checkpoint

from . import autograd as ag
from . import dwconv as hdw
from . import ops
from ._native import (BlockWeights, RelayBlockWeights, WindowAttnDesc, FUSE_ATTN_NO_RELAY, FUSE_ATTN_WS, PHASE_WHOLE,
                      PHASE_TOKENS, PHASE_REST, PHASE_RELAY_QKV, PHASE_TAIL)
from .plan import WindowPlan
from .weight_cache import _STORE as _W3_CACHE, derived


_FORCE_TRAIN_PATH = False


def _grad_path(x=None) -> bool:
    return torch.is_grad_enabled() or _FORCE_TRAIN_PATH


@contextlib.contextmanager
def training_numerics():
    global _FORCE_TRAIN_PATH
    old, _FORCE_TRAIN_PATH = _FORCE_TRAIN_PATH, True
    try:
        yield
    finally:
        _FORCE_TRAIN_PATH = old


def _ln(x, m: nn.LayerNorm):
    if x.is_cuda and not _grad_path(x) and x.shape[-1] in ops._LN_CHANNELS:
        return ops.layer_norm(x, m.weight, m.bias, m.eps)
    if x.is_cuda and x.numel() > 0 and x.shape[-1] in ops._LN_CHANNELS and x.dtype == torch.float32:
        return ag.layer_norm(x, m.weight, m.bias, m.eps)
    return F.layer_norm(x, m.normalized_shape, m.weight, m.bias, m.eps)


def _add_ln(x, y, m: nn.LayerNorm):
    if x.is_cuda and not _grad_path(x) and x.shape[-1] in ops._LN_CHANNELS:
        return ops.add_layer_norm(x, y, m.weight, m.bias, m.eps)
    x = x + y
    return x, _ln(x, m)


_GEMM_MODE = os.environ.get('HFL_GEMM', 'x3')
_SIDE_STREAM_MAX_ROWS = 32768

_PYRAMID_STREAMS = True
_SERIAL_STREAMS = False
_TRAIN_SPLIT = False
_TRAIN_X3 = True
_TRAIN_X6 = True
_TRAIN_MLP = True
_SPARSE_CONV = True
_EARLY_PHASE = True
_ATTN_WS = True
_ATTN_WS_MIN_ROWS = 40000
_ATTN_WS_EARLY = False
_MERGED_ATTN = True
_NATIVE_BLOCK = True
_RELAY_FUSED = True
_Q_PRESCALE = 16 ** -0.5 * 1.4426950408889634


def set_train_split(enabled: bool):
    global _TRAIN_SPLIT
    _TRAIN_SPLIT = bool(enabled)


def set_train_x3(enabled: bool):
    global _TRAIN_X3
    _TRAIN_X3 = bool(enabled)


def set_train_x6(enabled: bool):
    global _TRAIN_X6
    _TRAIN_X6 = bool(enabled)


def set_pyramid_streams(enabled):
    global _PYRAMID_STREAMS, _SERIAL_STREAMS
    _SERIAL_STREAMS = enabled == 'serial'
    _PYRAMID_STREAMS = bool(enabled)


def set_gemm_mode(mode: str):
    global _GEMM_MODE
    assert mode in ('fp32', 'bf16x3', 'x3', 'x6')
    _GEMM_MODE = mode


def get_gemm_mode() -> str:
    return _GEMM_MODE


def _split_path(x) -> bool:
    return _GEMM_MODE in ('bf16x3', 'x3') and x.is_cuda and not _grad_path() and x.shape[-1] % 128 == 0


def _w2(lin: nn.Linear):
    return ag._weight_image('x3', ops.split2_weight, lin.weight, False)


def _w6(lin: nn.Linear):
    return ag._w6_cached(lin.weight, False)


def _x6_lin_ok(lin: nn.Linear) -> bool:
    return ops.linear_x6_ok(lin.in_features, lin.out_features)


def _x6_path(x, *linears) -> bool:
    return (_GEMM_MODE == 'x6' and x.is_cuda and not _grad_path() and x.dtype == torch.float32 and x.numel() > 0
            and all(_x6_lin_ok(l) for l in linears))


def _x3_train(x, *linears) -> bool:
    return (_GEMM_MODE == 'x3' and _TRAIN_X3 and x.is_cuda and x.dtype == torch.float32 and x.numel() > 0
            and all(ag.linear_x3_ok(l.in_features, l.out_features) for l in linears))


def _x6_train(x, *linears) -> bool:
    return (_GEMM_MODE == 'x6' and _TRAIN_X6 and x.is_cuda and _grad_path() and x.dtype == torch.float32 and x.numel() > 0
            and all(ag.linear_x6_ok(l.in_features, l.out_features) for l in linears))


def _block_tail_x6(x, attn_out, proj: nn.Linear, norm2: nn.LayerNorm, mlp: 'MLP'):
    x = ops.linear_x6(attn_out, _w6(proj), bias=proj.bias, residual=x)
    h = ops.layer_norm(x, norm2.weight, norm2.bias, norm2.eps)
    g = ops.linear_x6(h, _w6(mlp.fc1), bias=mlp.fc1.bias, gelu=True)
    return ops.linear_x6(g, _w6(mlp.fc2), bias=mlp.fc2.bias, residual=x)


_MLP_FUSED_MIN_ROWS = 1000


def _mlp_pack(mlp: 'MLP', rows: int):
    f1, f2 = mlp.fc1, mlp.fc2
    c = f1.in_features
    if not (rows >= _MLP_FUSED_MIN_ROWS and c in (128, 256) and f1.out_features == 4 * c
            and f2.in_features == 4 * c and f2.out_features == c and f1.bias is not None and f2.bias is not None):
        return None
    w1, w2 = f1.weight, f2.weight
    return derived('mlp', (w1, w2), lambda: ops.mlp_fused_pack(w1, w2))


_QKV_FUSED_MIN_ROWS = 1000


def _qkv_pack(att: 'OctreeAttention', rows: int):
    lin = att.qkv
    c = lin.in_features
    if not (rows >= _QKV_FUSED_MIN_ROWS and c in (128, 256) and lin.out_features == 3 * c and lin.bias is not None):
        return None
    w = lin.weight
    return derived('qkvpack', (w,), lambda: ops.qkv_fused_pack(w))


def _relay_pack(att: 'RTAttention', mlp: 'MLP'):
    lins = (att.qkv, att.proj, mlp.fc1, mlp.fc2)
    c = att.dim
    if not (c == 256 and att.num_heads == 16 and mlp.fc1.out_features == 4 * c and all(l.bias is not None for l in lins)):
        return None
    ws = tuple(l.weight for l in lins)
    return derived('relaypack', ws, lambda: ops.relay_block_pack(*ws))


def _block_tail_x3(x, attn_out2, attn: 'OctreeAttention', norm2: nn.LayerNorm, mlp: 'MLP', fused_any_rows: bool = False):
    x = ops.linear_x3(attn_out2, _w2(attn.proj), bias=attn.proj.bias, residual=x)
    pack = _mlp_pack(mlp, _MLP_FUSED_MIN_ROWS if fused_any_rows else x.shape[0])
    if pack is not None:
        return ops.ln_mlp_fused(x, norm2.weight, norm2.bias, norm2.eps, pack, mlp.fc1.bias, mlp.fc2.bias)
    h2 = ops.layer_norm_split2(x, norm2.weight, norm2.bias, norm2.eps)
    g2 = ops.linear_x3(h2, _w2(mlp.fc1), bias=mlp.fc1.bias, gelu_split_out=True)
    return ops.linear_x3(g2, _w2(mlp.fc2), bias=mlp.fc2.bias, residual=x)


def _w3(lin: nn.Linear):
    return ag._w3_cached(lin.weight, False)


class SplitLinear(nn.Linear):

    def forward(self, x):
        if _grad_path() and _x3_train(x, self):
            return ag.linear_x3(x, self.weight, self.bias)
        if (_GEMM_MODE == 'bf16x3' and _TRAIN_SPLIT and x.is_cuda and _grad_path()
                and self.in_features % 8 == 0 and self.out_features % 8 == 0 and x.numel() > 0):
            return ag.linear_split(x, self.weight, self.bias)
        if _x6_train(x, self):
            return ag.linear_x6(x, self.weight, self.bias)
        if _x6_path(x, self):
            y = ops.linear_x6(x.reshape(-1, self.in_features), _w6(self), bias=self.bias)
            return y.view(*x.shape[:-1], self.out_features)
        return F.linear(x, self.weight, self.bias)


def _block_tail_split(x, attn_out3, attn: 'OctreeAttention', norm2: nn.LayerNorm, mlp: 'MLP'):
    if _GEMM_MODE == 'x3':
        return _block_tail_x3(x, attn_out3, attn, norm2, mlp)
    x = ops.gemm_bf16(attn_out3, _w3(attn.proj), bias=attn.proj.bias, residual=x)
    h3 = ops.layer_norm_split3(x, norm2.weight, norm2.bias, norm2.eps)
    g3 = ops.bias_gelu_split3(ops.split_mm(h3, _w3(mlp.fc1)), mlp.fc1.bias)
    return ops.gemm_bf16(g3, _w3(mlp.fc2), bias=mlp.fc2.bias, residual=x)


_CHECKPOINT_POLICY = os.environ.get('HFL_CHECKPOINT', 'auto')
_CHECKPOINT_FREE_FRACTION = float(os.environ.get('HFL_CHECKPOINT_FREE_FRACTION', '0.5'))
_BLOCK_BYTES_PER_ROW_CHANNEL = 80


def set_checkpoint_policy(policy: str):
    global _CHECKPOINT_POLICY
    assert policy in ('always', 'never', 'auto')
    prev, _CHECKPOINT_POLICY = _CHECKPOINT_POLICY, policy
    return prev


def _free_memory(device) -> int:
    free, _ = torch.cuda.mem_get_info(device)
    return free + torch.cuda.memory_reserved(device) - torch.cuda.memory_allocated(device)


def _use_checkpoint(stage, row_channels: int = 0, n_blocks: int = 1, device=None) -> bool:
    if not (bool(stage.grad_checkpoint) and stage.training and torch.is_grad_enabled()):
        return False
    if _CHECKPOINT_POLICY == 'always':
        return True
    if _CHECKPOINT_POLICY == 'never':
        return False
    if device is None or device.type != 'cuda' or row_channels <= 0:
        return True
    need = row_channels * n_blocks * _BLOCK_BYTES_PER_ROW_CHANNEL
    return need > _CHECKPOINT_FREE_FRACTION * _free_memory(device)


def _checkpoint_block(blk, *args):
    mods = blk.__dict__.get('_drop_path_mods')
    if mods is None:
        mods = blk.__dict__['_drop_path_mods'] = [m for m in blk.modules() if isinstance(m, OctreeDropPath)]
    snap = [(m, m._factors) for m in mods]

    def run(*a):
        prev = [(m, m._factors, m._calls) for m, _ in snap]
        for m, f in snap:
            m._factors, m._calls = f, 0
        try:
            return blk(*a)
        finally:
            for m, f, c in prev:
                m._factors, m._calls = f, c
    return checkpoint(run, *args, use_reentrant=False)


def disarm_drop_paths(model: nn.Module):
    cache = model.__dict__.get('_drop_path_cache')
    if cache is not None:
        for m in cache['mods']:
            m._factors = None


def _require_layernorm(conv_norm: str):
    if conv_norm.lower() != 'layernorm':
        raise NotImplementedError("conv_norm=%r: every shipped config uses 'layernorm'" % conv_norm)


def arm_drop_paths(model: nn.Module, batch_size: int, device, dtype=torch.float32):
    cache = model.__dict__.get('_drop_path_cache')
    if cache is None:
        cache = model.__dict__['_drop_path_cache'] = {'mods': [m for m in model.modules() if isinstance(m, OctreeDropPath)]}
    mods = [m for m in cache['mods'] if m.drop_prob > 0.0]
    sig = (tuple((m.drop_prob, m.scale_by_keep) for m in mods), str(device), dtype)
    if cache.get('sig') != sig:
        keep = [1.0 - m.drop_prob for m in mods for _ in range(2)]
        div = [(1.0 - m.drop_prob) if (m.scale_by_keep and m.drop_prob < 1.0) else 1.0 for m in mods for _ in range(2)]
        cache['sig'] = sig
        cache['keep'] = torch.tensor(keep, dtype=dtype).reshape(-1, 1).to(device)
        cache['div'] = torch.tensor(div, dtype=dtype).reshape(-1, 1).to(device)
    if not mods:
        return
    f = torch.floor(torch.rand(2 * len(mods), batch_size, dtype=dtype, device=device) + cache['keep']) / cache['div']
    for i, m in enumerate(mods):
        m._factors = f[2 * i:2 * i + 2]
        m._calls = 0


class OctreeDropPath(nn.Module):

    def __init__(self, drop_prob: float = 0.0, scale_by_keep: bool = True):
        super().__init__()
        self.drop_prob = float(drop_prob)
        self.scale_by_keep = scale_by_keep

    _factors = None
    _calls = 0

    def _draw(self, batch_size: int, dtype, device):
        f = self._factors
        if f is not None:
            if f.dim() != 2 or f.shape[1] != batch_size or f.device != device or f.dtype != dtype:
                raise RuntimeError('OctreeDropPath: armed factors %s %s on %s do not match a call with batch %d, %s on %s'
                                   % (tuple(f.shape), f.dtype, f.device, batch_size, dtype, device))
            r = f[self._calls % f.shape[0]]
            self._calls += 1
            return r
        keep = 1.0 - self.drop_prob
        rnd = torch.floor(torch.rand(batch_size, dtype=dtype, device=device) + keep)
        if keep > 0.0 and self.scale_by_keep:
            rnd = rnd / keep
        return rnd

    def forward(self, data, bid, batch_size: int):
        if self.drop_prob <= 0.0 or not self.training:
            return data
        return data * self._draw(batch_size, data.dtype, data.device)[bid].unsqueeze(1)

    def row_scale(self, bid, batch_size: int, like):
        if self.drop_prob <= 0.0 or not self.training:
            return None
        return self._draw(batch_size, like.dtype, like.device)[bid].reshape(-1).contiguous()

    def extra_repr(self):
        return 'drop_prob={:.4f}'.format(self.drop_prob)


class OctreeConv(nn.Module):

    def __init__(self, in_channels: int, out_channels: int, kernel_size: List[int] = [3],
                 stride: int = 1, nempty: bool = True, use_bias: bool = False):
        super().__init__()
        if not nempty:
            raise NotImplementedError('nempty=False octree conv is off the HOTFormerLoc path')
        ks = list(kernel_size) * 3 if len(kernel_size) == 1 else list(kernel_size)
        self.kernel = ''.join(str(k) for k in ks)
        self.kdim = ks[0] * ks[1] * ks[2]
        self.in_channels, self.out_channels, self.stride = in_channels, out_channels, stride
        self.weights = nn.Parameter(torch.empty(self.kdim, in_channels, out_channels))
        self.bias = nn.Parameter(torch.zeros(out_channels)) if use_bias else None
        nn.init.xavier_uniform_(self.weights)

    def takes_split2(self) -> bool:
        return (_SPARSE_CONV and (self.kernel, self.stride) in (('333', 1), ('222', 2)) and self.in_channels >= 32
                and _GEMM_MODE == 'x3' and self.in_channels % 32 == 0
                and (self.out_channels % 128 == 0 or self.out_channels == 64) and not _grad_path())

    def forward(self, data: torch.Tensor, octree, depth: int):
        if data.dtype == torch.bfloat16:
            assert self.takes_split2() and data.shape[1] == 2 * self.in_channels
            return self._forward_live_taps(data, octree, depth)
        if (_SPARSE_CONV and (self.kernel, self.stride) in (('333', 1), ('222', 2)) and self.in_channels >= 32
                and data.is_cuda):
            if not _grad_path(data):
                return self._forward_live_taps(data, octree, depth)
            if self.in_channels % 64 == 0 and self.out_channels % 64 == 0:
                out = ag.live_tap_conv(data, self.weights, octree, depth, self.kernel, self.stride)
                return out if self.bias is None else out + self.bias
        neigh = octree.get_neigh(depth, self.kernel, self.stride, nempty=True)
        col = ag.octree_gather(data, neigh) if _grad_path(data) else ops.octree_gather(data, neigh)
        w = self.weights.reshape(self.kdim * self.in_channels, self.out_channels)
        if torch.is_grad_enabled() and (col.requires_grad or self.weights.requires_grad):
            return ag.tall_mm(col, w, self.bias)
        if self.bias is not None:
            return torch.addmm(self.bias, col, w)
        return torch.mm(col, w)


    def _forward_live_taps(self, data, octree, depth):
        src, slot, edges = octree.sparse_taps(depth, self.kernel, self.stride)
        if (_GEMM_MODE == 'x3' and self.in_channels % 32 == 0
                and (self.out_channels % 128 == 0 or self.out_channels == 64) and edges[-1] > 0):
            npad = max(self.out_channels, 128)
            d2 = data if data.dtype == torch.bfloat16 else ops.split2(data)
            if d2.shape[0] * self.in_channels * 4 < (1 << 32):
                part = ops.linear_x3_grouped_gather(d2, src, ag._tap_blocks(self.weights, True, npad, ops.split2, 'taps2'),
                                                    octree.tap_tiles(depth, self.kernel, self.stride, npad), self.out_channels)
            else:
                gs = ops.octree_gather(d2.view(torch.float32), src).view(torch.bfloat16)
                part = ops.linear_x3_grouped(gs, ag._tap_blocks(self.weights, True, npad, ops.split2, 'taps2'),
                                             octree.tap_tiles(depth, self.kernel, self.stride, npad), self.out_channels)
            return self._slot_sum(part, slot)
        if (_GEMM_MODE == 'x6' and not _grad_path() and data.dtype == torch.float32 and edges[-1] > 0
                and self.in_channels % 32 == 0 and (self.out_channels % 128 == 0 or self.out_channels == 64)):
            npad = max(self.out_channels, 128)
            part = ops.linear_x6_grouped_gather(data, src, ag._tap_blocks(self.weights, True, npad),
                                                octree.tap_tiles(depth, self.kernel, self.stride, npad), self.out_channels)
            return self._slot_sum(part, slot)
        g = ops.octree_gather(data, src)
        part = torch.empty((g.shape[0], self.out_channels), dtype=torch.float32, device=data.device)
        w = self.weights
        for k in range(self.kdim):
            if edges[k + 1] > edges[k]:
                torch.mm(g[edges[k]:edges[k + 1]], w[k], out=part[edges[k]:edges[k + 1]])
        return self._slot_sum(part, slot)

    def _slot_sum(self, part, slot):
        if part.shape[1] % 4 == 0 and part.shape[1] <= 1024 and slot.shape[1] <= 27 and slot.dtype == torch.int32:
            return ops.slot_sum(part, slot, self.bias)
        out = ops.dwconv_forward_backward(part, self._unit(part.device), slot)
        return out if self.bias is None else out + self.bias

    def _unit(self, device):
        ones = self.__dict__.get('_unit_taps')
        if ones is None or ones.device != device:
            ones = torch.ones((self.kdim, 1, self.out_channels), dtype=torch.float32, device=device)
            self.__dict__['_unit_taps'] = ones
        return ones


class OctreeDWConvParams(nn.Module):

    def __init__(self, channels: int):
        super().__init__()
        self.weights = nn.Parameter(torch.empty(27, 1, channels))
        nn.init.xavier_uniform_(self.weights)


class OctreeConvNormRelu(nn.Module):

    def __init__(self, in_channels, out_channels, kernel_size=[3], stride=1, conv_norm='layernorm'):
        super().__init__()
        _require_layernorm(conv_norm)
        self.conv = OctreeConv(in_channels, out_channels, kernel_size, stride, nempty=True)
        self.norm = nn.LayerNorm(out_channels)

    def forward(self, data, octree, depth, split2_out: bool = False):
        y = self.conv(data, octree, depth)
        if y.is_cuda and not _grad_path(y) and y.shape[-1] in ops._LN_CHANNELS:
            return ops.layer_norm_relu(y, self.norm.weight, self.norm.bias, self.norm.eps, split2=split2_out)
        y = F.relu_(_ln(y, self.norm))
        return ops.split2(y) if split2_out else y


class PatchEmbed(nn.Module):

    def __init__(self, in_channels=3, dim=96, num_down=2, conv_norm='layernorm', downsample_input_embeddings=True):
        super().__init__()
        self.num_stages = num_down
        self.downsample_input_embeddings = downsample_input_embeddings
        if not downsample_input_embeddings:
            self.convs = nn.ModuleList([OctreeConvNormRelu(in_channels if i == 0 else dim, dim, [3], 1, conv_norm)
                                        for i in range(num_down)])
            return
        ch = [int(dim * 2 ** i) for i in range(-num_down, 1)]
        self.convs = nn.ModuleList([OctreeConvNormRelu(in_channels if i == 0 else ch[i], ch[i], [3], 1,
                                                       conv_norm) for i in range(num_down)])
        self.downsamples = nn.ModuleList([OctreeConvNormRelu(ch[i], ch[i + 1], [2], 2, conv_norm)
                                          for i in range(num_down)])
        self.proj = OctreeConvNormRelu(ch[-1], dim, [3], 1, conv_norm)

    def forward(self, data, octree, depth):
        if not self.downsample_input_embeddings:
            for i in range(self.num_stages):
                data = self.convs[i](data, octree, depth)
            return data
        seq = []
        for i in range(self.num_stages):
            seq += [(self.convs[i], depth - i), (self.downsamples[i], depth - i)]
        seq.append((self.proj, depth - self.num_stages))
        fast = data.is_cuda and not _grad_path(data)
        for n, (m, d) in enumerate(seq):
            nxt = seq[n + 1][0].conv if n + 1 < len(seq) else None
            data = m(data, octree, d, split2_out=bool(fast and nxt is not None and nxt.takes_split2()))
        return data


class Downsample(nn.Module):

    def __init__(self, in_channels, out_channels, conv_norm='layernorm'):
        super().__init__()
        _require_layernorm(conv_norm)
        self.conv = OctreeConv(in_channels, out_channels, [2], stride=2, nempty=True, use_bias=True)
        self.norm = nn.LayerNorm(out_channels)

    def forward(self, data, octree, depth):
        return _ln(self.conv(data, octree, depth), self.norm)


class MLP(nn.Module):

    def __init__(self, in_features, hidden_features=None, out_features=None):
        super().__init__()
        self.fc1 = SplitLinear(in_features, hidden_features or in_features)
        self.fc2 = SplitLinear(hidden_features or in_features, out_features or in_features)

    def forward(self, x):
        f1, f2 = self.fc1, self.fc2
        if f1.bias is not None and f2.bias is not None:
            fused = (ag.mlp_x3 if _TRAIN_MLP and _grad_path() and _x3_train(x, f1, f2)
                     else ag.mlp_x6 if _x6_train(x, f1, f2) else None)
            if fused is not None:
                return fused(x, f1.weight, f1.bias, f2.weight, f2.bias)
        if _x6_path(x, f1, f2) and x.dim() == 2:
            return ops.linear_x6(ops.linear_x6(x, _w6(f1), bias=f1.bias, gelu=True), _w6(f2), bias=f2.bias)
        return self.fc2(F.gelu(self.fc1(x)))


def _mlp_branch(x, norm: nn.LayerNorm, mlp: 'MLP', row_scale=None):
    f1, f2 = mlp.fc1, mlp.fc2
    if x.shape[-1] in ops._LN_CHANNELS and f1.bias is not None and f2.bias is not None:
        fused = (ag.ln_mlp_residual_x3 if _TRAIN_MLP and _x3_train(x, f1, f2)
                 else ag.ln_mlp_residual_x6 if x.dim() == 2 and _x6_train(x, f1, f2) else None)
        if fused is not None:
            return fused(x, norm.weight, norm.bias, norm.eps, f1.weight, f1.bias, f2.weight, f2.bias, row_scale)
    y = mlp(_ln(x, norm))
    return x + (y if row_scale is None else y * row_scale.unsqueeze(1))


class CPE(nn.Module):

    def __init__(self, dim, conv_norm='layernorm', xcpe=False):
        super().__init__()
        _require_layernorm(conv_norm)
        self.xcpe = xcpe
        if xcpe:
            self.conv = OctreeConv(dim, dim, [3], 1, nempty=True, use_bias=True)
            self.linear = nn.Linear(dim, dim)
        else:
            self.conv = OctreeDWConvParams(dim)
            self.linear = nn.Identity()
        self.norm = nn.LayerNorm(dim)

    def forward(self, data, plan: WindowPlan, depth: int, residual: bool, out=None):
        if self.xcpe:
            y = _ln(self.linear(self.conv(data, plan.octree, depth)), self.norm)
            y = data + y if residual else y
            if out is not None:
                out.copy_(y)
                return out
            return y
        if (_grad_path(data) and data.shape[1] in (32, 64, 128, 256) and data.is_cuda
                and data.dtype == torch.float32 and out is None):
            return ag.cpe(data, self.conv.weights, self.norm.weight, self.norm.bias, plan.neigh(depth), residual,
                          self.norm.eps)
        if _grad_path(data) or data.shape[1] not in (32, 64, 128, 256):
            y = _ln(hdw.octree_dwconv(data, self.conv.weights, plan.neigh(depth)), self.norm)
            y = data + y if residual else y
            if out is not None:
                out.copy_(y)
                return out
            return y
        return ops.cpe_forward(data, self.conv.weights, self.norm.weight, self.norm.bias,
                               plan.neigh(depth), residual, self.norm.eps, out=out)


class RPE(nn.Module):

    def __init__(self, patch_size, num_heads, dilation=1):
        super().__init__()
        self.pos_bnd = int(0.8 * patch_size * dilation ** 0.5)
        self.rpe_num = 2 * self.pos_bnd + 1
        self.rpe_table = nn.Parameter(torch.zeros(3 * self.rpe_num, num_heads))
        nn.init.trunc_normal_(self.rpe_table, std=0.02)


class OctreeAttention(nn.Module):

    def __init__(self, dim, patch_size, num_heads, dilation=1, rt_per_window=0, use_rpe=True):
        super().__init__()
        if dim // num_heads != 16:
            raise NotImplementedError('head dim must be 16 (all shipped configs)')
        self.dim, self.patch_size, self.num_heads = dim, patch_size, num_heads
        self.dilation, self.rt_per_window = dilation, rt_per_window
        self.qkv = SplitLinear(dim, dim * 3)
        self.proj = SplitLinear(dim, dim)
        self.rpe = RPE(patch_size, num_heads, dilation) if use_rpe else None

    def _cfg(self, plan: WindowPlan, depth: int) -> dict:
        nt = plan.n_tokens[depth]
        return dict(n_tokens=nt, n_windows=plan.n_windows[depth], patch_size=self.patch_size,
                    dilation=self.dilation, n_relay=self.rt_per_window, n_heads=self.num_heads,
                    batch_size=plan.B, rt_row0=nt, depth=depth)

    def core(self, qkv, plan: WindowPlan, depth: int, qkv_bias=None, out_split=False, qkv_f16=False):
        cfg = self._cfg(plan, depth)
        table = None if self.rpe is None else self.rpe.rpe_table
        if _grad_path(qkv):
            return ag.window_attention(qkv, table, plan.meta[depth], **cfg)
        return ops.window_attention(qkv, plan.meta[depth], table, qkv_bias=qkv_bias,
                                    out_split=out_split, qkv_f16=qkv_f16, **cfg)

    def forward(self, x, plan: WindowPlan, depth: int):
        return self.proj(self.core(self.qkv(x), plan, depth))

    def residual_branch(self, x, norm1: nn.LayerNorm, plan: WindowPlan, depth: int, row_scale=None):
        C = self.dim
        if _TRAIN_MLP and _x3_train(x, self.qkv, self.proj) and C in ops._LN_CHANNELS and self.proj.bias is not None:
            table = None if self.rpe is None else self.rpe.rpe_table
            return ag.ln_attn_residual_x3(x, norm1.weight, norm1.bias, norm1.eps, self.qkv.weight, self.qkv.bias, table,
                                          plan.meta[depth], self._cfg(plan, depth), self.proj.weight, self.proj.bias, row_scale)
        y = self.forward(_ln(x, norm1), plan, depth)
        return x + (y if row_scale is None else y * row_scale.unsqueeze(1))

    def forward_split(self, x, norm1: nn.LayerNorm, plan: WindowPlan, depth: int):
        if _GEMM_MODE == 'x3':
            f16 = _attn_f16_ok(x.shape[0], self, depth)
            nt = plan.n_tokens[depth]
            qpack = _qkv_pack(self, nt) if (f16 and x.dtype == torch.float32 and x.is_contiguous()) else None
            if qpack is not None:
                qkv = torch.empty((x.shape[0], 3 * x.shape[1]), dtype=torch.float32, device=x.device)
                ops.ln_qkv_fused(x[:nt], norm1.weight, norm1.bias, norm1.eps, qpack, self.qkv.bias, _Q_PRESCALE, out=qkv[:nt])
                if x.shape[0] > nt:
                    ops.ln_qkv_fused(x[nt:], norm1.weight, norm1.bias, norm1.eps, qpack, self.qkv.bias, _Q_PRESCALE, out=qkv[nt:])
                return self.core(qkv, plan, depth, out_split=2, qkv_f16=True)
            a2 = ops.layer_norm_split2(x, norm1.weight, norm1.bias, norm1.eps)
            if f16:
                qkv = ops.linear_x3_qkv(a2, _w2(self.qkv), self.qkv.bias, _Q_PRESCALE)
                return self.core(qkv, plan, depth, out_split=2, qkv_f16=True)
            qkv = ops.linear_x3(a2, _w2(self.qkv), bias=self.qkv.bias)
            return self.core(qkv, plan, depth, out_split=2)
        a3 = ops.layer_norm_split3(x, norm1.weight, norm1.bias, norm1.eps)
        return self.core(ops.split_mm(a3, _w3(self.qkv)), plan, depth, qkv_bias=self.qkv.bias,
                         out_split=True)


def _drops(block) -> bool:
    return block.training and block.drop_path.drop_prob > 0.0


def _fused_inference(block, x) -> bool:
    return _split_path(x) and not block.use_layer_scale and not _drops(block)


def _native_rows(block, x) -> bool:
    return (_fused_inference(block, x) and _GEMM_MODE == 'x3' and ops.KernelTimer.active is None
            and x.dtype == torch.float32 and x.is_contiguous())


def _init_layer_scale(block, dim, layer_scale):
# ... 977 lines not shown
```

### hotformerloc_amd/ops.py

```python

import ctypes
import weakref

import torch

from . import _native
from ._native import WindowAttnDesc, check


_RAW_STREAM = getattr(torch._C, '_cuda_getCurrentRawStream', None)
_RAW_DEVICE = getattr(torch._C, '_cuda_getDevice', None)


def _current_device() -> int:
    return _RAW_DEVICE() if _RAW_DEVICE is not None else torch.cuda.current_device()


def _stream():
    if _RAW_STREAM is not None and _RAW_DEVICE is not None:
        return ctypes.c_void_p(_RAW_STREAM(_RAW_DEVICE()))
    return ctypes.c_void_p(torch.cuda.current_stream().cuda_stream)


class KernelTimer:
    active = None

    def __init__(self, only=None):
        self.records = []
        self.only = None if only is None else frozenset(only)

    def __enter__(self):
        KernelTimer.active = self
        return self

    def __exit__(self, *exc):
        KernelTimer.active = None

    def summary(self):
        torch.cuda.synchronize()
        out = {}
        for name, e0, e1, nbytes, flops, moved in self.records:
            n, ms, b, f, mv = out.get(name, (0, 0.0, 0, 0, 0))
            out[name] = (n + 1, ms + e0.elapsed_time(e1), b + nbytes, f + flops, mv + moved)
        return out

    def by_size(self, name):
        torch.cuda.synchronize()
        groups = {}
        for n, e0, e1, nbytes, flops, moved in self.records:
            if n == name:
                c, ms = groups.get(nbytes, (0, 0.0))
                groups[nbytes] = (c + 1, ms + e0.elapsed_time(e1))
        return [(b, c, ms) for b, (c, ms) in sorted(groups.items(), reverse=True)]


class _timed:
    def __init__(self, name, nbytes, flops=0, moved=None):
        self.t = KernelTimer.active
        if self.t is not None and self.t.only is not None and name not in self.t.only:
            self.t = None
        if self.t is not None:
            self.name, self.nbytes, self.flops = name, int(nbytes), int(flops)
            self.moved = int(nbytes if moved is None else moved)

    def __enter__(self):
        if self.t is not None:
            self.e0 = torch.cuda.Event(enable_timing=True)
            self.e1 = torch.cuda.Event(enable_timing=True)
            self.e0.record()
        return self

    def __exit__(self, *exc):
        if self.t is not None:
            self.e1.record()
            self.t.records.append((self.name, self.e0, self.e1, self.nbytes, self.flops, self.moved))


def _dev(*tensors):
    cur = None
    for t in tensors:
        if t is None:
            continue
        if not t.is_cuda:
            raise _native.NativeLibraryError(
                'hotformerloc_amd ops need GPU tensors (got %s); there is no CPU fallback' % t.device)
        if cur is None:
            cur = _current_device()
        if t.device.index != cur:
            raise _native.NativeLibraryError(
                'tensor on %s but the current device is cuda:%d; wrap the call in torch.cuda.device(...)'
                % (t.device, cur))


def _f32c(t):
    if t.dtype != torch.float32:
        raise TypeError('float32 expected, got %s' % t.dtype)
    return t.contiguous()


def _idx(neigh):
    if neigh.dtype == torch.int64:
        return neigh.contiguous(), 1
    if neigh.dtype == torch.int32:
        return neigh.contiguous(), 0
    raise TypeError('neighbour table must be int32 or int64, got %s' % neigh.dtype)


def dwconv_forward_backward(data: torch.Tensor, weight: torch.Tensor, neigh: torch.Tensor):
    _dev(data, weight, neigh)
    data, weight = _f32c(data), _f32c(weight)
    neigh, i64 = _idx(neigh)
    m, k = neigh.shape
    c = data.shape[1]
    out = torch.empty((m, c), dtype=torch.float32, device=data.device)
    check(_native.load().hfl_dwconv_forward_backward(
        out.data_ptr(), data.data_ptr(), weight.data_ptr(), neigh.data_ptr(), i64, m, c, k,
        _stream()), 'hfl_dwconv_forward_backward')
    return out


def dwconv_add(data: torch.Tensor, weight: torch.Tensor, neigh: torch.Tensor, add=None, out=None):
    _dev(data, weight, neigh, add, out)
    data, weight = _f32c(data), _f32c(weight)
    assert neigh.dtype == torch.int32 and neigh.is_contiguous()
    m, k = neigh.shape
    c = data.shape[1]
    if out is None:
        out = torch.empty((m, c), dtype=torch.float32, device=data.device)
    else:
        assert tuple(out.shape) == (m, c) and out.is_contiguous() and out.dtype == torch.float32
        assert out.data_ptr() != data.data_ptr()
    if add is not None:
        add = _f32c(add)
        assert tuple(add.shape) == (m, c)
    check(_native.load().hfl_dwconv_add(out.data_ptr(), data.data_ptr(), weight.data_ptr(), neigh.data_ptr(),
                                        None if add is None else add.data_ptr(), m, c, k, _stream()), 'hfl_dwconv_add')
    return out


def slot_sum(part: torch.Tensor, slot: torch.Tensor, bias=None):
    _dev(part, slot, bias)
    part = _f32c(part)
    assert slot.dtype == torch.int32 and slot.is_contiguous() and slot.dim() == 2
    n, k = slot.shape
    c = part.shape[1]
    out = torch.empty((n, c), dtype=torch.float32, device=part.device)
    check(_native.load().hfl_slot_sum(out.data_ptr(), part.data_ptr(), slot.data_ptr(),
                                      None if bias is None else _f32c(bias).data_ptr(), n, c, k, _stream()), 'hfl_slot_sum')
    return out


def dwconv_weight_backward(grad: torch.Tensor, data: torch.Tensor, neigh: torch.Tensor):
    _dev(grad, data, neigh)
    grad, data = _f32c(grad), _f32c(data)
    neigh, i64 = _idx(neigh)
    n, k = neigh.shape
    c = data.shape[1]
    lib = _native.load()
    ws = torch.empty(int(lib.hfl_dwconv_weight_backward_workspace(n, c, k)), dtype=torch.uint8,
                     device=data.device)
    out = torch.empty((k, 1, c), dtype=torch.float32, device=data.device)
    check(lib.hfl_dwconv_weight_backward(out.data_ptr(), grad.data_ptr(), data.data_ptr(),
                                         neigh.data_ptr(), i64, n, c, k, ws.data_ptr(), _stream()),
          'hfl_dwconv_weight_backward')
    return out


def inverse_neigh(neigh: torch.Tensor):
    _dev(neigh)
    neigh, i64 = _idx(neigh)
    out = torch.empty_like(neigh)
    check(_native.load().hfl_inverse_neigh(out.data_ptr(), neigh.data_ptr(), i64, neigh.shape[0],
                                           neigh.shape[1], _stream()), 'hfl_inverse_neigh')
    return out


def cpe_forward(x, weight, gamma, beta, neigh, residual: bool, eps: float = 1e-5, out=None, conv_out=None):
    _dev(x, weight, gamma, beta, neigh, conv_out)
    x = _f32c(x)
    assert neigh.dtype == torch.int32 and neigh.is_contiguous()
    if out is None:
        out = torch.empty_like(x)
    else:
        assert out.shape == x.shape and out.is_contiguous() and out.dtype == torch.float32
        assert out.data_ptr() != x.data_ptr(), 'CPE gathers neighbours: cannot run in place'
    n, c = x.shape
    with _timed('hfl_cpe_forward', n * c * 8 + n * neigh.shape[1] * 4, 2 * neigh.shape[1] * n * c):
        if conv_out is not None:
            assert conv_out.shape == x.shape and conv_out.is_contiguous() and conv_out.dtype == torch.float32
            check(_native.load().hfl_cpe_forward_save(
                out.data_ptr(), conv_out.data_ptr(), x.data_ptr(), _f32c(weight).data_ptr(), _f32c(gamma).data_ptr(),
                _f32c(beta).data_ptr(), neigh.data_ptr(), n, c, neigh.shape[1],
                float(eps), int(bool(residual)), _stream()), 'hfl_cpe_forward_save')
            return out
        check(_native.load().hfl_cpe_forward(
            out.data_ptr(), x.data_ptr(), _f32c(weight).data_ptr(), _f32c(gamma).data_ptr(),
            _f32c(beta).data_ptr(), neigh.data_ptr(), n, c, neigh.shape[1],
            float(eps), int(bool(residual)), _stream()), 'hfl_cpe_forward')
    return out


_LN_CHANNELS = (16, 32, 64, 128, 256, 512, 1024)


def layer_norm(x, weight, bias, eps: float = 1e-5):
    _dev(x, weight, bias)
    c = x.shape[-1]
    xc = _f32c(x)
    out = torch.empty_like(xc)
    with _timed('hfl_layer_norm', xc.numel() * 8):
        check(_native.load().hfl_layer_norm(out.data_ptr(), xc.data_ptr(), weight.data_ptr(),
                                            bias.data_ptr(), xc.numel() // c, c, float(eps), _stream()),
              'hfl_layer_norm')
    return out


def layer_norm_bwd(dy, x, weight, eps: float = 1e-5, dres=None):
    _dev(dy, x, weight, dres)
    c = x.shape[-1]
    x2, dy2 = _f32c(x).view(-1, c), _f32c(dy).view(-1, c)
    lib = _native.load()
    nb = int(lib.hfl_layer_norm_bwd_blocks(x2.shape[0], c))
    if nb <= 0:
        raise _native.NativeLibraryError('hfl_layer_norm_bwd: unsupported channel count %d' % c)
    dx = torch.empty(x.shape, dtype=torch.float32, device=x.device)
    part = torch.empty((2, nb, c), dtype=torch.float32, device=x.device)
    check(lib.hfl_layer_norm_bwd_add(dx.data_ptr(), part[0].data_ptr(), part[1].data_ptr(), dy2.data_ptr(), x2.data_ptr(),
                                     _f32c(weight).data_ptr(), None if dres is None else _f32c(dres).data_ptr(),
                                     x2.shape[0], c, float(eps), _stream()), 'hfl_layer_norm_bwd')
    dgb = torch.empty((2, c), dtype=torch.float32, device=x.device)
    check(lib.hfl_layer_norm_bwd_finalize(dgb[0].data_ptr(), dgb[1].data_ptr(), part[0].data_ptr(), part[1].data_ptr(),
                                          nb, c, _stream()), 'hfl_layer_norm_bwd_finalize')
    return dx, dgb[0], dgb[1]


def add_layer_norm(x, y, weight, bias, eps: float = 1e-5, add_bias=None, inplace: bool = False):
    _dev(x, y, weight, bias, add_bias)
    c = x.shape[-1]
    x2, y2 = _f32c(x).view(-1, c), _f32c(y).view(-1, c)
    xo = x2 if inplace else torch.empty_like(x2)
    h = torch.empty_like(x2)
    with _timed('hfl_add_layer_norm', x2.numel() * 16):
        check(_native.load().hfl_add_layer_norm(
            xo.data_ptr(), h.data_ptr(), x2.data_ptr(), y2.data_ptr(),
            None if add_bias is None else add_bias.data_ptr(), weight.data_ptr(), bias.data_ptr(),
            x2.shape[0], c, float(eps), _stream()), 'hfl_add_layer_norm')
    return xo.view(x.shape), h.view(x.shape)


def _a3(rows, c, device):
    return torch.empty((rows, 3 * c), dtype=torch.bfloat16, device=device)


def layer_norm_split3(x, weight, bias, eps: float = 1e-5):
    _dev(x, weight, bias)
    c = x.shape[-1]
    x2 = _f32c(x).view(-1, c)
    out = _a3(x2.shape[0], c, x.device)
    with _timed('hfl_layer_norm_split3', x2.numel() * 10):
        check(_native.load().hfl_layer_norm_split3(out.data_ptr(), x2.data_ptr(), weight.data_ptr(),
                                                   bias.data_ptr(), x2.shape[0], c, float(eps),
                                                   _stream()), 'hfl_layer_norm_split3')
    return out


def add_layer_norm_split3(x, y, weight, bias, eps: float = 1e-5, add_bias=None):
    _dev(x, y, weight, bias, add_bias)
    c = x.shape[-1]
    x2, y2 = _f32c(x).view(-1, c), _f32c(y).view(-1, c)
    xo = torch.empty_like(x2)
    h = _a3(x2.shape[0], c, x.device)
    with _timed('hfl_add_layer_norm_split3', x2.numel() * 18):
        check(_native.load().hfl_add_layer_norm_split3(
            xo.data_ptr(), h.data_ptr(), x2.data_ptr(), y2.data_ptr(),
            None if add_bias is None else add_bias.data_ptr(), weight.data_ptr(), bias.data_ptr(),
            x2.shape[0], c, float(eps), _stream()), 'hfl_add_layer_norm_split3')
    return xo.view(x.shape), h


def add_bias(x, y, bias=None):
    _dev(x, y, bias)
    c = x.shape[-1]
    x2, y2 = _f32c(x).view(-1, c), _f32c(y).view(-1, c)
    out = torch.empty_like(x2)
    with _timed('hfl_add_bias', x2.numel() * 12):
        check(_native.load().hfl_add_bias(out.data_ptr(), x2.data_ptr(), y2.data_ptr(),
                                          None if bias is None else bias.data_ptr(), x2.shape[0], c,
                                          _stream()), 'hfl_add_bias')
    return out.view(x.shape)


def bias_gelu_split3(x, bias=None):
    _dev(x, bias)
    c = x.shape[-1]
    x2 = _f32c(x).view(-1, c)
    out = _a3(x2.shape[0], c, x.device)
    with _timed('hfl_bias_gelu_split3', x2.numel() * 10):
        check(_native.load().hfl_bias_gelu_split3(out.data_ptr(), x2.data_ptr(),
                                                  None if bias is None else bias.data_ptr(),
                                                  x2.shape[0], c, _stream()), 'hfl_bias_gelu_split3')
    return out
# ... 1679 lines not shown
```

### include/hotformerloc_hip.h

```cpp
#ifndef HOTFORMERLOC_HIP_H
#define HOTFORMERLOC_HIP_H

#include <stdint.h>

#ifdef __cplusplus
extern "C" {
#endif

typedef void* hfl_stream_t;

#define HFL_OK 0
#define HFL_EINVAL (-1)
#define HFL_ECAPACITY (-2)
#define HFL_EBACKEND (-100)

int hfl_version(void);
const char* hfl_arch(void);


int hfl_dwconv_forward_backward(float* out, const float* data, const float* weight,
                                const void* neigh, int idx64, int64_t n_out,
                                int64_t channels, int kngh, hfl_stream_t stream);

int hfl_slot_sum(float* out, const float* part, const int32_t* slot, const float* bias, int64_t n_out, int64_t channels, int kngh,
                 hfl_stream_t stream);

int64_t hfl_dwconv_weight_backward_workspace(int64_t n_rows, int64_t channels, int kngh);
int hfl_dwconv_weight_backward(float* out, const float* grad, const float* data,
                               const void* neigh, int idx64, int64_t n_rows,
                               int64_t channels, int kngh, void* workspace,
                               hfl_stream_t stream);

int hfl_inverse_neigh(void* ineigh, const void* neigh, int idx64, int64_t n_rows,
                      int kngh, hfl_stream_t stream);

int hfl_cpe_forward(float* out, const float* x, const float* weight, const float* gamma,
                    const float* beta, const int32_t* neigh, int64_t n_rows,
                    int64_t channels, int kngh, float eps, int residual,
                    hfl_stream_t stream);
int hfl_cpe_forward_save(float* out, float* conv_out, const float* x, const float* weight, const float* gamma,
                         const float* beta, const int32_t* neigh, int64_t n_rows,
                         int64_t channels, int kngh, float eps, int residual,
                         hfl_stream_t stream);
int hfl_dwconv_add(float* out, const float* data, const float* weight, const int32_t* neigh, const float* add,
                   int64_t n_out, int64_t channels, int kngh, hfl_stream_t stream);


#define HFL_OCTREE_MAX_POINTS (1 << 20)
#define HFL_OCTREE_MAX_DEPTH 10

int64_t hfl_octree_scratch_bytes(int64_t total_points, int batch, int max_points, int depth);

int hfl_octree_build_clouds(const float* points, const int64_t* cloud_offsets, int batch,
                            int64_t total_points, int max_points, int depth, int full_depth,
                            void* scratch, float* leaf_points, int32_t* counts,
                            hfl_stream_t stream);

int hfl_octree_merge(const void* scratch, const int64_t* cloud_offsets, const int32_t* cum_nne,
                     int batch, int depth, int full_depth, int64_t total_points,
                     int64_t* const* keys, int32_t* const* children,
                     int64_t* const* nkeys, int32_t* const* nidx,
                     const float* leaf_points, float* points_out, hfl_stream_t stream);

int hfl_octree_neigh(int32_t* neigh_out, const int32_t* neigh_parent, const int32_t* nidx,
                     const int32_t* children, const int64_t* nkeys, int64_t nne, int depth,
                     int full_depth, hfl_stream_t stream);

int hfl_token_meta(uint32_t* tok_meta, const int64_t* nkeys, int64_t n, int depth,
                   hfl_stream_t stream);

int hfl_prepare_clouds(float* out_points, int32_t* out_counts, const float* points,
                       const int64_t* cloud_offsets, int batch, int normalize, int cylindrical_mask,
                       int cylindrical_transform, hfl_stream_t stream);

typedef struct hfl_augment_cloud {
  int32_t remove_k;
  int32_t block;
  float rot_cos, rot_sin;
  float trans[3];
  float block_u[4];
  float reserved;
} hfl_augment_cloud;

typedef struct hfl_augment_config {
  int32_t normalize;
  int32_t cylindrical_mask;
  int32_t cylindrical_transform;
  int32_t augment;
  int32_t rotate;
  int32_t set_rotate;
  int32_t flip_axis;
  float set_cos, set_sin;
  float jitter_sigma, jitter_clip;
} hfl_augment_config;

int hfl_augment_clouds(float* out_points, int32_t* out_counts, int32_t* out_index, const float* points,
                       const int64_t* cloud_offsets, const int64_t* host_cloud_offsets, int batch,
                       const hfl_augment_cloud* table, const hfl_augment_cloud* host_table,
                       const hfl_augment_config* config, uint64_t seed, int64_t cloud_base,
                       const uint32_t* selection_keys, hfl_stream_t stream);

#define HFL_VOXEL_MAX_CLOUDS 32767
#define HFL_VOXEL_MAX_CELLS 65535
#define HFL_VOXEL_MAX_POINTS 2147483646LL
int hfl_voxel_keys(int64_t* keys, int32_t* flags, uint32_t* bounds, const float* points, const int64_t* cloud_offsets,
                   int batch, int64_t n_points, double voxel_size, hfl_stream_t stream);
int64_t hfl_voxel_reduce_workspace(int64_t n_points);
int hfl_voxel_reduce(float* out_points, int64_t* out_offsets, int32_t* out_cell_counts, int64_t* out_keys,
                     const int64_t* sorted_keys, const int64_t* perm, const float* points, int64_t n_points, int batch,
                     void* workspace, int64_t workspace_bytes, hfl_stream_t stream);
int hfl_submap_normalise(float* out_points, int32_t* out_counts, int32_t* flags, const float* points,
                         const int64_t* cloud_offsets, int batch, hfl_stream_t stream);
int hfl_submap_normalise_rows(float* out_rows, int32_t* keep, const float* points, const int64_t* cloud_offsets,
                              const float* raw_points, const int64_t* raw_offsets, const int64_t* row_index,
                              const int64_t* row_offsets, int batch, hfl_stream_t stream);
int hfl_voxel_gather_rows(float* out_points, const float* points, int64_t n_points, const int64_t* index, int64_t n_rows,
                          hfl_stream_t stream);
int hfl_voxel_bounds(uint32_t* bounds, const float* points, const int64_t* cloud_offsets, int batch, int64_t n_points,
                     hfl_stream_t stream);
typedef struct {
  int32_t cloud;
  int32_t nx, ny, nz;
  double voxel;
  int64_t word_offset;
} hfl_voxel_candidate;
#define HFL_VOXEL_OCC_MAX_CANDIDATES 65535
#define HFL_VOXEL_OCC_MAX_WORDS 67108863LL
int64_t hfl_voxel_occupancy_workspace(int n_candidates, int64_t bitmap_words);
int hfl_voxel_occupancy(int32_t* counts, const hfl_voxel_candidate* candidates, int n_candidates, int64_t bitmap_words,
                        const uint32_t* bounds, const float* points, const int64_t* cloud_offsets, int batch,
                        int64_t n_points, int64_t max_cloud_points, void* workspace, int64_t workspace_bytes,
                        hfl_stream_t stream);

#define HFL_CLOTH_MAX_PARTICLES 10240
typedef struct {
  float ox, oy, u0;
  int32_t width, height;
  int32_t reserved;
  int64_t cell_offset;
} hfl_cloth_desc;
int hfl_cloth_raster(float* terrain, uint64_t* keys, const hfl_cloth_desc* descs_host, const hfl_cloth_desc* descs, int batch,
                     int64_t n_cells, const float* points, const int64_t* cloud_offsets, int64_t n_points, float resolution,
                     hfl_stream_t stream);
int hfl_cloth_simulate(float* heights, uint8_t* movable, int32_t* steps_run, const float* terrain,
                       const hfl_cloth_desc* descs_host, const hfl_cloth_desc* descs, int batch, int64_t n_cells, float f_one,
                       float f_two, float gravity_step, float velocity_keep, int iterations, int slope_smooth,
                       hfl_stream_t stream);
int hfl_cloth_classify(uint8_t* keep, const float* heights, const hfl_cloth_desc* descs_host, const hfl_cloth_desc* descs,
                       int batch, int64_t n_cells, const float* points, const int64_t* cloud_offsets, int64_t n_points,
                       float resolution, float threshold, hfl_stream_t stream);

#define HFL_KNN_MAX_NEIGHBOURS 32
#define HFL_KNN_MAX_CELLS 268435455LL
#define HFL_KNN_PHASE_STARTS 1
#define HFL_KNN_PHASE_QUERY 2
#define HFL_KNN_PHASE_FALLBACK 4
#define HFL_KNN_PHASE_ALL 7
typedef struct {
  float ox, oy, oz, cell;
  float mx, my, mz;
  int32_t k;
  int32_t nx, ny, nz;
  int32_t reserved;
  int64_t cell_base;
} hfl_knn_grid;
int hfl_cloud_nonfinite(int32_t* flags, const float* points, const int64_t* cloud_offsets, int batch, int64_t n_points,
                        hfl_stream_t stream);
int hfl_knn_cell_keys(int64_t* keys, const hfl_knn_grid* grids_host, const hfl_knn_grid* grids, int batch, int64_t n_cells,
                      const float* points, const int64_t* cloud_offsets, int64_t n_points, hfl_stream_t stream);
int hfl_knn_mean_dist(float* avg, int32_t* pending, int32_t* counter, int32_t* cell_starts, const float* sorted_points,
                      const int64_t* sorted_keys, const int64_t* perm, const hfl_knn_grid* grids_host,
                      const hfl_knn_grid* grids, int batch, int64_t n_cells, const int64_t* cloud_offsets, int64_t n_points,
                      int phases, hfl_stream_t stream);
int hfl_outlier_threshold(double* stats, const float* avg, const int64_t* cloud_offsets, int batch, int64_t n_points,
                          double std_ratio, hfl_stream_t stream);
int hfl_outlier_mask(uint8_t* keep, const float* avg, const double* stats, const int64_t* cloud_offsets, int batch,
                     int64_t n_points, hfl_stream_t stream);
int hfl_radius_mask(uint8_t* keep, const float* points, int64_t n_points, double radius_max, hfl_stream_t stream);
// ... 351 lines not shown
```

Baseline: 3218 clouds/s.

## Fuse LayerNorm and ReLU into sparse-conv slot-sum kernel and shrink tap-table blocks

Adds a slot_sum_norm kernel that sums the per-tap partial products and then applies LayerNorm (optionally ReLU and a bf16 split2 store) inside the same wave. This removes the separate normalization pass and its round trip of the conv output through memory. The slot-sum kernel also gets compile-time channel widths, replaces block barriers with wave barriers, and uses a ballot-built bitmask to skip missing taps. Separately, the tap-table builder now processes 256 rows per block instead of 1024, which launches more blocks and drops a barrier; the LN row helper is moved into a shared header.

New measurement: 3268 clouds/s (median of 6 runs). +1.5%, better.

```diff
diff --git a/hotformerloc_amd/_native.py b/hotformerloc_amd/_native.py
--- a/hotformerloc_amd/_native.py
+++ b/hotformerloc_amd/_native.py
@@ -204,6 +204,8 @@
     'hfl_tap_wgrad': (c_int, [c_void_p, c_void_p, c_void_p, c_void_p, c_int, c_void_p, c_int, c_int, c_int, c_void_p,
                              c_void_p]),
     'hfl_slot_sum': (c_int, [c_void_p, c_void_p, c_void_p, c_void_p, c_int64, c_int64, c_int, c_void_p]),
+    'hfl_slot_sum_norm': (c_int, [c_void_p, c_void_p, c_void_p, c_void_p, c_void_p, c_void_p, c_void_p, c_int64, c_int64, c_int,
+                                  c_float, c_int, c_void_p]),
     'hfl_tap_wgrad_gather': (c_int, [c_void_p, c_void_p, c_void_p, c_void_p, c_void_p, c_void_p, c_int, c_void_p, c_int, c_int,
                                     c_int, c_void_p, c_void_p]),
     'hfl_wgrad_x3_workspace': (c_int64, [c_int64, c_int64, c_int64]),
diff --git a/hotformerloc_amd/build.py b/hotformerloc_amd/build.py
--- a/hotformerloc_amd/build.py
+++ b/hotformerloc_amd/build.py
@@ -46,7 +46,7 @@
     os.makedirs(objdir, exist_ok=True)
     hipcc = _hipcc()
     headers = [os.path.join(CSRC, 'hfl_common.h'), os.path.join(CSRC, 'x3_math.h'), os.path.join(CSRC, 'stage_stream.h'),
-               os.path.join(CSRC, 'prep_common.h'),
+               os.path.join(CSRC, 'prep_common.h'), os.path.join(CSRC, 'ln_row.h'),
                os.path.join(HERE, '..', 'include', 'hotformerloc_hip.h')]
     jobs = []
     for src in SOURCES:
diff --git a/hotformerloc_amd/csrc/dwconv.hip b/hotformerloc_amd/csrc/dwconv.hip
--- a/hotformerloc_amd/csrc/dwconv.hip
+++ b/hotformerloc_amd/csrc/dwconv.hip
@@ -1,4 +1,5 @@
 #include "hfl_common.h"
+#include "ln_row.h"
 
 namespace {
 
@@ -77,41 +78,81 @@
   }
 }
 
-template <int B>
+constexpr int kSlotMax = 32;
+
+template <int TPR, int NORM, int B>
 __global__ void __launch_bounds__(256) slot_sum_kernel(float* __restrict__ out, const float* __restrict__ part,
                                                         const int32_t* __restrict__ slot, const float* __restrict__ bias,
-                                                        int64_t n_out, int C, int K, int tpr, int rpb) {
+                                                        const float* __restrict__ gamma, const float* __restrict__ beta,
+                                                        int64_t n_out, int C_rt, int K, int tpr_rt, int rpb, float eps, int relu) {
+  static_assert(NORM == 0 || TPR > 0, "the fused norm needs the row inside one wave");
   extern __shared__ __attribute__((aligned(16))) unsigned char smem[];
   int32_t* s_idx = reinterpret_cast<int32_t*>(smem);
+  const int tpr = TPR > 0 ? TPR : tpr_rt;
+  const int C = TPR > 0 ? TPR * 4 : C_rt;
   const int tx = threadIdx.x % tpr, ty = threadIdx.x / tpr;
   const float4 bv = bias != nullptr ? reinterpret_cast<const float4*>(bias)[tx] : make_float4(0.f, 0.f, 0.f, 0.f);
+  float4 gm[1], bt[1];
+  if (NORM) {
+    gm[0] = reinterpret_cast<const float4*>(gamma)[tx];
+    bt[0] = reinterpret_cast<const float4*>(beta)[tx];
+  }
+  int32_t* row_idx = s_idx + ty * K;
   for (int64_t base = (int64_t)blockIdx.x * rpb; base < n_out; base += (int64_t)gridDim.x * rpb) {
     const int64_t h = base + ty;
     const bool live = h < n_out;
-    __syncthreads();
-    if (live)
-      for (int k = tx; k < K; k += tpr) s_idx[ty * K + k] = slot[h * K + k];
-    __syncthreads();
-    if (!live) continue;
+    unsigned mask = 0;
+    if (TPR > 0) {
+      __builtin_amdgcn_fence(__ATOMIC_RELEASE, "wavefront");
+      __builtin_amdgcn_wave_barrier();
+      const int shift = (threadIdx.x & 63) - tx;
+      constexpr unsigned long long row_lanes = TPR >= 64 ? ~0ull : ((1ull << (TPR & 63)) - 1ull);
+#pragma unroll
+      for (int p = 0; p * TPR < kSlotMax; ++p) {
+        const int k = p * TPR + tx;
+        const bool in = live && k < K;
+        const int32_t ni = in ? slot[h * K + k] : -1;
+        if (in) row_idx[k] = ni;
+        const unsigned long long bal = __ballot(ni >= 0);
+        mask |= (unsigned)((bal >> shift) & row_lanes & 0xffffffffull) << (p * TPR);
+      }
+      __builtin_amdgcn_fence(__ATOMIC_RELEASE, "wavefront");
+      __builtin_amdgcn_wave_barrier();
+    } else {
+      __syncthreads();
+      if (live)
+        for (int k = tx; k < K; k += tpr) row_idx[k] = slot[h * K + k];
+      __syncthreads();
+      if (live)
+        for (int k = 0; k < K; ++k) mask |= (unsigned)(row_idx[k] >= 0) << k;
+    }
     float4 acc = make_float4(0.f, 0.f, 0.f, 0.f);
 #pragma unroll 1
-    for (int k0 = 0; k0 < K; k0 += B) {
+    while (mask != 0) {
+      int32_t ni[B];
       float4 v[B];
       bool ok[B];
 #pragma unroll
       for (int j = 0; j < B; ++j) {
-        const int k = k0 + j;
-        int64_t ni = (k < K) ? (int64_t)s_idx[ty * K + k] : -1;
-        ok[j] = ni >= 0;
-        if (!ok[j]) ni = 0;
-        v[j] = reinterpret_cast<const float4*>(part + ni * C)[tx];
-      }
+        ok[j] = mask != 0;
+        const int k = ok[j] ? __ffs(mask) - 1 : 0;
+        mask &= mask - 1;
+        ni[j] = row_idx[k];
+      }
+#pragma unroll
+      for (int j = 0; j < B; ++j)
+        if (ok[j]) v[j] = reinterpret_cast<const float4*>(part + (int64_t)ni[j] * C)[tx];
 #pragma unroll
       for (int j = 0; j < B; ++j)
         if (ok[j]) { acc.x += v[j].x; acc.y += v[j].y; acc.z += v[j].z; acc.w += v[j].w; }
     }
     if (bias != nullptr) { acc.x += bv.x; acc.y += bv.y; acc.z += bv.z; acc.w += bv.w; }
-    reinterpret_cast<float4*>(out + h * C)[tx] = acc;
+    if constexpr (NORM > 0) {
+      float4 a[1] = {live ? acc : make_float4(0.f, 0.f, 0.f, 0.f)};
+      hfl_ln_row<TPR, 1, NORM == 2 ? 2 : 0>(out, a, gm, bt, h, live, tx, eps, relu);
+    } else {
+      if (live) reinterpret_cast<float4*>(out + h * C)[tx] = acc;
+    }
   }
 }
 
@@ -447,6 +488,22 @@
   HFL_RETURN_LAST_ERROR();
 }
 
+
+template <int TPR, int NORM>
+static int launch_slot_sum(float* out, const float* part, const int32_t* slot, const float* bias, const float* gamma,
+                           const float* beta, int64_t n_out, int64_t channels, int K, float eps, int relu, hipStream_t s) {
+  const RowGeom g = row_geom(channels);
+  const size_t lds = (size_t)g.rpb * K * sizeof(int32_t);
+  static int nb = 0;
+  static size_t nb_lds = 0;
+  const int per_cu = persistent_per_cu(reinterpret_cast<const void*>(slot_sum_kernel<TPR, NORM, 8>), g.tpr * g.rpb, lds, 8, &nb,
+                                       &nb_lds);
+  const int64_t need = hfl_cdiv(n_out, g.rpb), cap = (int64_t)hfl_stream_cus(s) * per_cu;
+  slot_sum_kernel<TPR, NORM, 8><<<(int)(need < cap ? need : cap), g.tpr * g.rpb, lds, s>>>(
+      out, part, slot, bias, gamma, beta, n_out, (int)channels, K, g.tpr, g.rpb, eps, relu);
+  HFL_RETURN_LAST_ERROR();
+}
+
 }
 
 extern "C" {
@@ -551,18 +608,39 @@
 
 int hfl_slot_sum(float* out, const float* part, const int32_t* slot, const float* bias, int64_t n_out, int64_t channels, int kngh,
                  hfl_stream_t stream) {
-  if (n_out < 0 || channels <= 0 || channels % 4 != 0 || channels > 1024 || kngh <= 0 || kngh > kMaxTaps) return HFL_EINVAL;
+  if (n_out < 0 || channels <= 0 || channels % 4 != 0 || channels > 1024 || kngh <= 0 || kngh > kSlotMax) return HFL_EINVAL;
   if (n_out == 0) return HFL_OK;
   if (out == nullptr || part == nullptr || slot == nullptr) return HFL_EINVAL;
   hipStream_t s = static_cast<hipStream_t>(stream);
-  const RowGeom g = row_geom(channels);
-  const size_t lds = (size_t)g.rpb * kngh * sizeof(int32_t);
-  static int nb = 0;
-  static size_t nb_lds = 0;
-  const int per_cu = persistent_per_cu(reinterpret_cast<const void*>(slot_sum_kernel<9>), g.tpr * g.rpb, lds, 8, &nb, &nb_lds);
-  const int64_t need = hfl_cdiv(n_out, g.rpb), cap = (int64_t)hfl_stream_cus(s) * per_cu;
-  slot_sum_kernel<9><<<(int)(need < cap ? need : cap), g.tpr * g.rpb, lds, s>>>(out, part, slot, bias, n_out, (int)channels, kngh,
-                                                                               g.tpr, g.rpb);
-  HFL_RETURN_LAST_ERROR();
-}
-}
+  switch (channels) {
+    case 256: return launch_slot_sum<64, 0>(out, part, slot, bias, nullptr, nullptr, n_out, channels, kngh, 0.f, 0, s);
+    case 128: return launch_slot_sum<32, 0>(out, part, slot, bias, nullptr, nullptr, n_out, channels, kngh, 0.f, 0, s);
+    case 64:  return launch_slot_sum<16, 0>(out, part, slot, bias, nullptr, nullptr, n_out, channels, kngh, 0.f, 0, s);
+    case 32:  return launch_slot_sum<8, 0>(out, part, slot, bias, nullptr, nullptr, n_out, channels, kngh, 0.f, 0, s);
+    default:  return launch_slot_sum<0, 0>(out, part, slot, bias, nullptr, nullptr, n_out, channels, kngh, 0.f, 0, s);
+  }
+}
+
+int hfl_slot_sum_norm(float* out_f32, uint16_t* out_split2, const float* part, const int32_t* slot, const float* bias,
+                      const float* gamma, const float* beta, int64_t n_out, int64_t channels, int kngh, float eps, int relu,
+                      hfl_stream_t stream) {
+  if (n_out < 0 || kngh <= 0 || kngh > kSlotMax || (out_f32 == nullptr) == (out_split2 == nullptr)) return HFL_EINVAL;
+  if (channels != 32 && channels != 64 && channels != 128 && channels != 256) return HFL_EINVAL;
+  if (out_split2 != nullptr && channels % 32 != 0) return HFL_EINVAL;
+  if (n_out == 0) return HFL_OK;
+  if (part == nullptr || slot == nullptr || gamma == nullptr || beta == nullptr) return HFL_EINVAL;
+  hipStream_t s = static_cast<hipStream_t>(stream);
+  float* out = out_f32 != nullptr ? out_f32 : reinterpret_cast<float*>(out_split2);
+  const int r = relu ? 1 : 0;
+#define HFL_SLOT_NORM(TPR)                                                                                                    \
+  return out_split2 != nullptr ? launch_slot_sum<TPR, 2>(out, part, slot, bias, gamma, beta, n_out, channels, kngh, eps, r, s) \
+                               : launch_slot_sum<TPR, 1>(out, part, slot, bias, gamma, beta, n_out, channels, kngh, eps, r, s)
+  switch (channels) {
+    case 256: HFL_SLOT_NORM(64);
+    case 128: HFL_SLOT_NORM(32);
+    case 64:  HFL_SLOT_NORM(16);
+    default:  HFL_SLOT_NORM(8);
+  }
+#undef HFL_SLOT_NORM
+}
+}
diff --git a/hotformerloc_amd/csrc/ln_row.h b/hotformerloc_amd/csrc/ln_row.h
--- /dev/null
+++ b/hotformerloc_amd/csrc/ln_row.h
@@ -0,0 +1,69 @@
+#pragma once
+#include "hfl_common.h"
+
+__device__ __forceinline__ uint16_t hfl_bf16_rne(float v) {
+  uint32_t u = __float_as_uint(v);
+  u += 0x7FFFu + ((u >> 16) & 1u);
+  return (uint16_t)(u >> 16);
+}
+__device__ __forceinline__ void hfl_split4(const float4 v, uint2& hi, uint2& lo) {
+  const uint16_t h0 = hfl_bf16_rne(v.x), h1 = hfl_bf16_rne(v.y), h2 = hfl_bf16_rne(v.z), h3 = hfl_bf16_rne(v.w);
+  const uint16_t l0 = hfl_bf16_rne(v.x - __uint_as_float((uint32_t)h0 << 16));
+  const uint16_t l1 = hfl_bf16_rne(v.y - __uint_as_float((uint32_t)h1 << 16));
+  const uint16_t l2 = hfl_bf16_rne(v.z - __uint_as_float((uint32_t)h2 << 16));
+  const uint16_t l3 = hfl_bf16_rne(v.w - __uint_as_float((uint32_t)h3 << 16));
+  hi = make_uint2((uint32_t)h0 | ((uint32_t)h1 << 16), (uint32_t)h2 | ((uint32_t)h3 << 16));
+  lo = make_uint2((uint32_t)l0 | ((uint32_t)l1 << 16), (uint32_t)l2 | ((uint32_t)l3 << 16));
+}
+__device__ __forceinline__ void hfl_store_split3(uint16_t* row, int C, int c4, const float4 v) {
+  uint2 hi, lo;
+  hfl_split4(v, hi, lo);
+  reinterpret_cast<uint2*>(row)[c4] = hi;
+  reinterpret_cast<uint2*>(row + C)[c4] = hi;
+  reinterpret_cast<uint2*>(row + 2 * C)[c4] = lo;
+}
+
+__device__ __forceinline__ void hfl_store_split2(uint16_t* row, int c4, const float4 v) {
+  uint2 hi, lo;
+  hfl_split4(v, hi, lo);
+  uint16_t* o = row + (c4 >> 3) * 64 + (c4 & 7) * 4;
+  *reinterpret_cast<uint2*>(o) = hi;
+  *reinterpret_cast<uint2*>(o + 32) = lo;
+}
+
+template <int TPR, int VPL, int SPLIT>
+__device__ __forceinline__ void hfl_ln_row(float* __restrict__ h_out, float4 (&a)[VPL], const float4 (&gm)[VPL],
+                                           const float4 (&bt)[VPL], int64_t r, bool live, int tx, float eps, int relu) {
+  constexpr int C = TPR * VPL * 4;
+  const float inv_c = 1.0f / (float)C;
+  float sum = 0.f;
+#pragma unroll
+  for (int v = 0; v < VPL; ++v) sum += (a[v].x + a[v].y) + (a[v].z + a[v].w);
+  const float mean = hfl_group_sum<TPR>(sum) * inv_c;
+  float sq = 0.f;
+#pragma unroll
+  for (int v = 0; v < VPL; ++v) {
+    a[v].x -= mean; a[v].y -= mean; a[v].z -= mean; a[v].w -= mean;
+    sq += (a[v].x * a[v].x + a[v].y * a[v].y) + (a[v].z * a[v].z + a[v].w * a[v].w);
+  }
+  const float rstd = 1.0f / sqrtf(hfl_group_sum<TPR>(sq) * inv_c + eps);
+  if (live) {
+#pragma unroll
+    for (int v = 0; v < VPL; ++v) {
+      float4 o;
+      o.x = fmaf(a[v].x * rstd, gm[v].x, bt[v].x);
+      o.y = fmaf(a[v].y * rstd, gm[v].y, bt[v].y);
+      o.z = fmaf(a[v].z * rstd, gm[v].z, bt[v].z);
+      o.w = fmaf(a[v].w * rstd, gm[v].w, bt[v].w);
+      if (relu) {
+        o.x = fmaxf(o.x, 0.f); o.y = fmaxf(o.y, 0.f); o.z = fmaxf(o.z, 0.f); o.w = fmaxf(o.w, 0.f);
+      }
+      if (SPLIT == 1)
+        hfl_store_split3(reinterpret_cast<uint16_t*>(h_out) + r * 3 * C, C, v * TPR + tx, o);
+      else if (SPLIT == 2)
+        hfl_store_split2(reinterpret_cast<uint16_t*>(h_out) + r * 2 * C, v * TPR + tx, o);
+      else
+        reinterpret_cast<float4*>(h_out + r * C)[v * TPR + tx] = o;
+    }
+  }
+}
diff --git a/hotformerloc_amd/csrc/octree.hip b/hotformerloc_amd/csrc/octree.hip
--- a/hotformerloc_amd/csrc/octree.hip
+++ b/hotformerloc_amd/csrc/octree.hip
@@ -346,7 +346,7 @@
   meta[2 * t + 1] = (uint32_t)(key >> 48);
 }
 
-constexpr int kTapRows = 1024;
+constexpr int kTapRows = 256;
 constexpr int kTapMax = 32;
 constexpr int kTapTables = 16;
 
@@ -409,20 +409,17 @@
   __shared__ int32_t wave_cnt[4][kTapMax];
   const int lane = threadIdx.x & 63, wave = threadIdx.x >> 6;
   const int taps = TAPS > 0 ? TAPS : t.taps;
-  int32_t acc[kTapMax];
-#pragma unroll
-  for (int k = 0; k < kTapMax; ++k) acc[k] = 0;
+  static_assert(kTapRows == 256, "one row per thread");
   const int64_t row0 = (int64_t)block * kTapRows;
   int32_t* lds_wave = lds + wave * (64 * (TAPS > 0 ? TAPS : 1));
-  for (int it = 0; it < kTapRows / 256; ++it) {
-    int32_t v[kTapMax];
-    tap_load_rows<TAPS>(t.table, t.rows, row0 + it * 256 + wave * 64, lds_wave, lane, v, taps);
-#pragma unroll
-    for (int k = 0; k < kTapMax; ++k)
-      if (k < taps) acc[k] += __popcll(__ballot(v[k] >= 0));
-  }
-  if (lane == 0)
-    for (int k = 0; k < taps; ++k) wave_cnt[wave][k] = acc[k];
+  int32_t v[kTapMax];
+  tap_load_rows<TAPS>(t.table, t.rows, row0 + wave * 64, lds_wave, lane, v, taps);
+#pragma unroll
+  for (int k = 0; k < kTapMax; ++k)
+    if (k < taps) {
+      const int32_t c = __popcll(__ballot(v[k] >= 0));
+      if (lane == 0) wave_cnt[wave][k] = c;
+    }
   __syncthreads();
   if ((int)threadIdx.x < taps)
     t.block_counts[(int64_t)block * taps + threadIdx.x] =
@@ -484,56 +481,49 @@
   const int64_t row0 = (int64_t)block * kTapRows;
   const unsigned long long lt = lane == 0 ? 0ull : (~0ull >> (64 - lane));
   int32_t* lds_wave = lds + wave * (64 * (TAPS > 0 ? TAPS : 1));
-  for (int it = 0; it < kTapRows / 256; ++it) {
-    const int64_t rw = row0 + it * 256 + wave * 64;
-    const int64_t r = rw + lane;
-    const bool in = r < t.rows;
-    int32_t v[kTapMax];
-    unsigned long long mk[kTapMax];
-    tap_load_rows<TAPS>(t.table, t.rows, rw, lds_wave, lane, v, taps);
+  const int64_t rw = row0 + wave * 64;
+  const int64_t r = rw + lane;
+  const bool in = r < t.rows;
+  int32_t v[kTapMax];
+  unsigned long long mk[kTapMax];
+  tap_load_rows<TAPS>(t.table, t.rows, rw, lds_wave, lane, v, taps);
+#pragma unroll
+  for (int k = 0; k < kTapMax; ++k)
+    if (k < taps) {
+      mk[k] = __ballot(v[k] >= 0);
+      if (lane == 0) wave_cnt[wave][k] = __popcll(mk[k]);
+    }
+  __syncthreads();
+  int32_t pos[kTapMax];
+#pragma unroll
+  for (int k = 0; k < kTapMax; ++k) {
+    if (k < taps) {
+      int32_t off = base[k];
+      for (int w = 0; w < wave; ++w) off += wave_cnt[w][k];
+      pos[k] = v[k] >= 0 ? off + __popcll(mk[k] & lt) : -1;
+      if (in && v[k] >= 0) t.src[pos[k]] = v[k];
+    }
+  }
+  if constexpr (TAPS == 8) {
+    if (in) {
+      reinterpret_cast<int4*>(t.slot)[r * 2] = make_int4(pos[0], pos[1], pos[2], pos[3]);
+      reinterpret_cast<int4*>(t.slot)[r * 2 + 1] = make_int4(pos[4], pos[5], pos[6], pos[7]);
+    }
+  } else if constexpr (TAPS > 0) {
+#pragma unroll
+    for (int k = 0; k < TAPS; ++k) lds_wave[lane * TAPS + k] = pos[k];
+    __builtin_amdgcn_fence(__ATOMIC_RELEASE, "wavefront");
+    __builtin_amdgcn_wave_barrier();
+    const int64_t w0 = rw * TAPS, wend = t.rows * TAPS;
+#pragma unroll
+    for (int j = 0; j < TAPS; ++j) {
+      const int64_t w = w0 + j * 64 + lane;
+      if (w < wend) t.slot[w] = lds_wave[j * 64 + lane];
+    }
+  } else {
 #pragma unroll
     for (int k = 0; k < kTapMax; ++k)
-      if (k < taps) mk[k] = __ballot(v[k] >= 0);
-    __syncthreads();
-    if (lane == 0)
-      for (int k = 0; k < taps; ++k) wave_cnt[wave][k] = __popcll(mk[k]);
-    __syncthreads();
-    int32_t pos[kTapMax];
-#pragma unroll
-    for (int k = 0; k < kTapMax; ++k) {
-      if (k < taps) {
-        int32_t off = base[k];
-        for (int w = 0; w < wave; ++w) off += wave_cnt[w][k];
-        pos[k] = v[k] >= 0 ? off + __popcll(mk[k] & lt) : -1;
-        if (in && v[k] >= 0) t.src[pos[k]] = v[k];
-      }
-    }
-    if constexpr (TAPS == 8) {
-      if (in) {
-        reinterpret_cast<int4*>(t.slot)[r * 2] = make_int4(pos[0], pos[1], pos[2], pos[3]);
-        reinterpret_cast<int4*>(t.slot)[r * 2 + 1] = make_int4(pos[4], pos[5], pos[6], pos[7]);
-      }
-    } else if constexpr (TAPS > 0) {
-#pragma unroll
-      for (int k = 0; k < TAPS; ++k) lds_wave[lane * TAPS + k] = pos[k];
-      __builtin_amdgcn_fence(__ATOMIC_RELEASE, "wavefront");
-      __builtin_amdgcn_wave_barrier();
-      const int64_t w0 = rw * TAPS, wend = t.rows * TAPS;
-#pragma unroll
-      for (int j = 0; j < TAPS; ++j) {
-        const int64_t w = w0 + j * 64 + lane;
-        if (w < wend) t.slot[w] = lds_wave[j * 64 + lane];
-      }
-      __builtin_amdgcn_wave_barrier();
-    } else {
-#pragma unroll
-      for (int k = 0; k < kTapMax; ++k)
-        if (k < taps && in) t.slot[r * taps + k] = pos[k];
-    }
-    __syncthreads();
-    if ((int)threadIdx.x < taps)
-      base[threadIdx.x] += wave_cnt[0][threadIdx.x] + wave_cnt[1][threadIdx.x] + wave_cnt[2][threadIdx.x] +
-                           wave_cnt[3][threadIdx.x];
+      if (k < taps && in) t.slot[r * taps + k] = pos[k];
   }
 }
 
diff --git a/hotformerloc_amd/csrc/window_misc.hip b/hotformerloc_amd/csrc/window_misc.hip
--- a/hotformerloc_amd/csrc/window_misc.hip
+++ b/hotformerloc_amd/csrc/window_misc.hip
@@ -1,4 +1,5 @@
 #include "hfl_common.h"
+#include "ln_row.h"
 
 namespace {
 
@@ -216,36 +217,6 @@
 }
 
 
-__device__ __forceinline__ uint16_t hfl_bf16_rne(float v) {
-  uint32_t u = __float_as_uint(v);
-  u += 0x7FFFu + ((u >> 16) & 1u);
-  return (uint16_t)(u >> 16);
-}
-__device__ __forceinline__ void hfl_split4(const float4 v, uint2& hi, uint2& lo) {
-  const uint16_t h0 = hfl_bf16_rne(v.x), h1 = hfl_bf16_rne(v.y), h2 = hfl_bf16_rne(v.z), h3 = hfl_bf16_rne(v.w);
-  const uint16_t l0 = hfl_bf16_rne(v.x - __uint_as_float((uint32_t)h0 << 16));
-  const uint16_t l1 = hfl_bf16_rne(v.y - __uint_as_float((uint32_t)h1 << 16));
-  const uint16_t l2 = hfl_bf16_rne(v.z - __uint_as_float((uint32_t)h2 << 16));
-  const uint16_t l3 = hfl_bf16_rne(v.w - __uint_as_float((uint32_t)h3 << 16));
-  hi = make_uint2((uint32_t)h0 | ((uint32_t)h1 << 16), (uint32_t)h2 | ((uint32_t)h3 << 16));
-  lo = make_uint2((uint32_t)l0 | ((uint32_t)l1 << 16), (uint32_t)l2 | ((uint32_t)l3 << 16));
-}
-__device__ __forceinline__ void hfl_store_split3(uint16_t* row, int C, int c4, const float4 v) {
-  uint2 hi, lo;
-  hfl_split4(v, hi, lo);
-  reinterpret_cast<uint2*>(row)[c4] = hi;
-  reinterpret_cast<uint2*>(row + C)[c4] = hi;
-  reinterpret_cast<uint2*>(row + 2 * C)[c4] = lo;
-}
-
-__device__ __forceinline__ void hfl_store_split2(uint16_t* row, int c4, const float4 v) {
-  uint2 hi, lo;
-  hfl_split4(v, hi, lo);
-  uint16_t* o = row + (c4 >> 3) * 64 + (c4 & 7) * 4;
-  *reinterpret_cast<uint2*>(o) = hi;
-  *reinterpret_cast<uint2*>(o + 32) = lo;
-}
-
 template <int TPR, int VPL, bool ADD, int SPLIT>
 __global__ void __launch_bounds__(256)
 layer_norm_kernel(float* __restrict__ h_out, float* x_out, const float* x, const float* __restrict__ y,
@@ -262,12 +233,10 @@
     bs[v] = make_float4(0.f, 0.f, 0.f, 0.f);
     if (ADD && bias != nullptr) bs[v] = reinterpret_cast<const float4*>(bias)[v * TPR + tx];
   }
-  const float inv_c = 1.0f / (float)C;
   for (int64_t base = (int64_t)blockIdx.x * RPB; base < n_rows; base += (int64_t)gridDim.x * RPB) {
     const int64_t r = base + ty;
     const bool live = r < n_rows;
     float4 a[VPL];
-    float sum = 0.f;
 #pragma unroll
     for (int v = 0; v < VPL; ++v) {
       a[v] = make_float4(0.f, 0.f, 0.f, 0.f);
@@ -280,35 +249,8 @@
           reinterpret_cast<float4*>(x_out + r * C)[v * TPR + tx] = a[v];
         }
       }
-      sum += (a[v].x + a[v].y) + (a[v].z + a[v].w);
-    }
-    const float mean = hfl_group_sum<TPR>(sum) * inv_c;
-    float sq = 0.f;
-#pragma unroll
-    for (int v = 0; v < VPL; ++v) {
-      a[v].x -= mean; a[v].y -= mean; a[v].z -= mean; a[v].w -= mean;
-      sq += (a[v].x * a[v].x + a[v].y * a[v].y) + (a[v].z * a[v].z + a[v].w * a[v].w);
-    }
-    const float rstd = 1.0f / sqrtf(hfl_group_sum<TPR>(sq) * inv_c + eps);
-    if (live) {
-#pragma unroll
-      for (int v = 0; v < VPL; ++v) {
-        float4 o;
-        o.x = fmaf(a[v].x * rstd, gm[v].x, bt[v].x);
-        o.y = fmaf(a[v].y * rstd, gm[v].y, bt[v].y);
-        o.z = fmaf(a[v].z * rstd, gm[v].z, bt[v].z);
-        o.w = fmaf(a[v].w * rstd, gm[v].w, bt[v].w);
-        if (relu) {
-          o.x = fmaxf(o.x, 0.f); o.y = fmaxf(o.y, 0.f); o.z = fmaxf(o.z, 0.f); o.w = fmaxf(o.w, 0.f);
-        }
-        if (SPLIT == 1)
-          hfl_store_split3(reinterpret_cast<uint16_t*>(h_out) + r * 3 * C, C, v * TPR + tx, o);
-        else if (SPLIT == 2)
-          hfl_store_split2(reinterpret_cast<uint16_t*>(h_out) + r * 2 * C, v * TPR + tx, o);
-        else
-          reinterpret_cast<float4*>(h_out + r * C)[v * TPR + tx] = o;
-      }
-    }
+    }
+    hfl_ln_row<TPR, VPL, SPLIT>(h_out, a, gm, bt, r, live, tx, eps, relu);
   }
 }
 
diff --git a/hotformerloc_amd/model.py b/hotformerloc_amd/model.py
--- a/hotformerloc_amd/model.py
+++ b/hotformerloc_amd/model.py
@@ -67,6 +67,7 @@
 _MERGED_ATTN = True
 _NATIVE_BLOCK = True
 _RELAY_FUSED = True
+_CONV_NORM_FUSED = True
 _Q_PRESCALE = 16 ** -0.5 * 1.4426950408889634
 
 
@@ -331,6 +332,13 @@
         return 'drop_prob={:.4f}'.format(self.drop_prob)
 
 
+class _NormTail:
+    __slots__ = ('norm', 'relu', 'split2', 'done')
+
+    def __init__(self, norm: nn.LayerNorm, relu: bool, split2: bool = False):
+        self.norm, self.relu, self.split2, self.done = norm, relu, split2, False
+
+
 class OctreeConv(nn.Module):
 
     def __init__(self, in_channels: int, out_channels: int, kernel_size: List[int] = [3],
@@ -351,14 +359,14 @@
                 and _GEMM_MODE == 'x3' and self.in_channels % 32 == 0
                 and (self.out_channels % 128 == 0 or self.out_channels == 64) and not _grad_path())
 
-    def forward(self, data: torch.Tensor, octree, depth: int):
+    def forward(self, data: torch.Tensor, octree, depth: int, tail: Optional[_NormTail] = None):
         if data.dtype == torch.bfloat16:
             assert self.takes_split2() and data.shape[1] == 2 * self.in_channels
-            return self._forward_live_taps(data, octree, depth)
+            return self._forward_live_taps(data, octree, depth, tail)
         if (_SPARSE_CONV and (self.kernel, self.stride) in (('333', 1), ('222', 2)) and self.in_channels >= 32
                 and data.is_cuda):
             if not _grad_path(data):
-                return self._forward_live_taps(data, octree, depth)
+                return self._forward_live_taps(data, octree, depth, tail)
             if self.in_channels % 64 == 0 and self.out_channels % 64 == 0:
                 out = ag.live_tap_conv(data, self.weights, octree, depth, self.kernel, self.stride)
                 return out if self.bias is None else out + self.bias
@@ -372,7 +380,7 @@
         return torch.mm(col, w)
 
 
-    def _forward_live_taps(self, data, octree, depth):
+    def _forward_live_taps(self, data, octree, depth, tail=None):
         src, slot, edges = octree.sparse_taps(depth, self.kernel, self.stride)
         if (_GEMM_MODE == 'x3' and self.in_channels % 32 == 0
                 and (self.out_channels % 128 == 0 or self.out_channels == 64) and edges[-1] > 0):
@@ -385,13 +393,13 @@
                 gs = ops.octree_gather(d2.view(torch.float32), src).view(torch.bfloat16)
                 part = ops.linear_x3_grouped(gs, ag._tap_blocks(self.weights, True, npad, ops.split2, 'taps2'),
                                              octree.tap_tiles(depth, self.kernel, self.stride, npad), self.out_channels)
-            return self._slot_sum(part, slot)
+            return self._slot_sum(part, slot, tail)
         if (_GEMM_MODE == 'x6' and not _grad_path() and data.dtype == torch.float32 and edges[-1] > 0
                 and self.in_channels % 32 == 0 and (self.out_channels % 128 == 0 or self.out_channels == 64)):
             npad = max(self.out_channels, 128)
             part = ops.linear_x6_grouped_gather(data, src, ag._tap_blocks(self.weights, True, npad),
                                                 octree.tap_tiles(depth, self.kernel, self.stride, npad), self.out_channels)
-            return self._slot_sum(part, slot)
+            return self._slot_sum(part, slot, tail)
         g = ops.octree_gather(data, src)
         part = torch.empty((g.shape[0], self.out_channels), dtype=torch.float32, device=data.device)
         w = self.weights
@@ -400,7 +408,12 @@
                 torch.mm(g[edges[k]:edges[k + 1]], w[k], out=part[edges[k]:edges[k + 1]])
         return self._slot_sum(part, slot)
 
-    def _slot_sum(self, part, slot):
+    def _slot_sum(self, part, slot, tail=None):
+        if (tail is not None and _CONV_NORM_FUSED and part.shape[1] in ops._SLOT_NORM_CHANNELS and slot.shape[1] <= 32
+                and slot.dtype == torch.int32 and slot.shape[0] > 0):
+            tail.done = True
+            return ops.slot_sum_norm(part, slot, self.bias, tail.norm.weight, tail.norm.bias, tail.norm.eps, relu=tail.relu,
+                                     split2=tail.split2)
         if part.shape[1] % 4 == 0 and part.shape[1] <= 1024 and slot.shape[1] <= 27 and slot.dtype == torch.int32:
             return ops.slot_sum(part, slot, self.bias)
         out = ops.dwconv_forward_backward(part, self._unit(part.device), slot)
@@ -431,7 +444,10 @@
         self.norm = nn.LayerNorm(out_channels)
 
     def forward(self, data, octree, depth, split2_out: bool = False):
-        y = self.conv(data, octree, depth)
+        tail = _NormTail(self.norm, True, split2_out)
+        y = self.conv(data, octree, depth, tail)
+        if tail.done:
+            return y
         if y.is_cuda and not _grad_path(y) and y.shape[-1] in ops._LN_CHANNELS:
             return ops.layer_norm_relu(y, self.norm.weight, self.norm.bias, self.norm.eps, split2=split2_out)
         y = F.relu_(_ln(y, self.norm))
@@ -480,7 +496,9 @@
         self.norm = nn.LayerNorm(out_channels)
 
     def forward(self, data, octree, depth):
-        return _ln(self.conv(data, octree, depth), self.norm)
+        tail = _NormTail(self.norm, False)
+        y = self.conv(data, octree, depth, tail)
+        return y if tail.done else _ln(y, self.norm)
 
 
 class MLP(nn.Module):
diff --git a/hotformerloc_amd/ops.py b/hotformerloc_amd/ops.py
--- a/hotformerloc_amd/ops.py
+++ b/hotformerloc_amd/ops.py
@@ -147,6 +147,27 @@
     out = torch.empty((n, c), dtype=torch.float32, device=part.device)
     check(_native.load().hfl_slot_sum(out.data_ptr(), part.data_ptr(), slot.data_ptr(),
                                       None if bias is None else _f32c(bias).data_ptr(), n, c, k, _stream()), 'hfl_slot_sum')
+    return out
+
+
+_SLOT_NORM_CHANNELS = (32, 64, 128, 256)
+
+
+def slot_sum_norm(part: torch.Tensor, slot: torch.Tensor, bias, weight, norm_bias, eps: float = 1e-5, relu: bool = False,
+                  split2: bool = False):
+    _dev(part, slot, bias, weight, norm_bias)
+    part = _f32c(part)
+    assert slot.dtype == torch.int32 and slot.is_contiguous() and slot.dim() == 2
+    n, k = slot.shape
+    c = part.shape[1]
+    if split2:
+        out = torch.empty((n, 2 * c), dtype=torch.bfloat16, device=part.device)
+    else:
+        out = torch.empty((n, c), dtype=torch.float32, device=part.device)
+    check(_native.load().hfl_slot_sum_norm(None if split2 else out.data_ptr(), out.data_ptr() if split2 else None,
+                                           part.data_ptr(), slot.data_ptr(), None if bias is None else _f32c(bias).data_ptr(),
+                                           _f32c(weight).data_ptr(), _f32c(norm_bias).data_ptr(), n, c, k, float(eps),
+                                           int(bool(relu)), _stream()), 'hfl_slot_sum_norm')
     return out
 
 
diff --git a/include/hotformerloc_hip.h b/include/hotformerloc_hip.h
--- a/include/hotformerloc_hip.h
+++ b/include/hotformerloc_hip.h
@@ -24,6 +24,10 @@
 
 int hfl_slot_sum(float* out, const float* part, const int32_t* slot, const float* bias, int64_t n_out, int64_t channels, int kngh,
                  hfl_stream_t stream);
+
+int hfl_slot_sum_norm(float* out_f32, uint16_t* out_split2, const float* part, const int32_t* slot, const float* bias,
+                      const float* gamma, const float* beta, int64_t n_out, int64_t channels, int kngh, float eps, int relu,
+                      hfl_stream_t stream);
 
 int64_t hfl_dwconv_weight_backward_workspace(int64_t n_rows, int64_t channels, int kngh);
 int hfl_dwconv_weight_backward(float* out, const float* grad, const float* data,
```
